# ChalmersPhotonicsLab/QAMpy

Measured on AMD Instinct MI355X. Metric: equalised MSym/s (2-pol, 2 SPS), higher is better.
Workload: dtype f32

## Files before the change

qampy_amd/csrc/api.hip:

```cpp
#include "common.h"
#include <stdlib.h>
#include <atomic>
#include <mutex>
#include <vector>
#include <unordered_map>
#include <string.h>

namespace qh {

thread_local hipStream_t g_stream = nullptr;
static thread_local hipStream_t g_streams[4] = {nullptr, nullptr, nullptr, nullptr};
int g_device = -1;
static thread_local std::string g_err;
static std::mutex g_mu;

void set_error(const std::string &s) { g_err = s; }

int hip_fail(hipError_t e, const char *what, const char *file, int line)
{
    g_err = std::string(hipGetErrorString(e)) + " in " + what + " (" + file + ":" + std::to_string(line) + ")";
    (void)hipGetLastError();
    return QH_ERR_HIP;
}

static std::atomic<int> g_reserved_cus{-1};
static std::atomic<double> g_gram_budget_gb{-1.0};
static std::atomic<int> g_default_tier{0};
static std::atomic<double> g_default_tol{1e-3};
static int reserved_cus()
{
    int v = g_reserved_cus.load();
    if (v < 0) { const char *e = getenv("QAMPY_HIP_RESERVED_CUS"); v = e ? atoi(e) : 32; if (v < 0) v = 0; g_reserved_cus.store(v); }
    return v;
}
double gram_budget_gb()
{
    double v = g_gram_budget_gb.load();
    if (v < 0) { const char *e = getenv("QAMPY_HIP_GRAM_BUDGET_GB"); v = e ? atof(e) : 160.0; if (!(v > 0)) v = 160.0; g_gram_budget_gb.store(v); }
    return v;
}
static std::atomic<int> g_pit_timing{-1};
int pit_timing_mode()
{
    int v = g_pit_timing.load();
    if (v < 0) { const char *e = getenv("QAMPY_HIP_PIT_TIMING"); v = !e ? 1 : (e[0] == 'a' ? 2 : (e[0] == 'n' ? 0 : 1)); g_pit_timing.store(v); }
    return v;
}
int default_tier() { return g_default_tier.load(); }
double default_tier_tol() { return g_default_tol.load(); }

static int init_device(int device)
{
    std::lock_guard<std::mutex> lk(g_mu);
    if (g_stream && device == g_device) return QH_OK;
    if (g_device >= 0 && device != g_device) {
        set_error("libqampy_hip is already initialised on device " + std::to_string(g_device) + ": one device per process");
        return QH_ERR_ARG;
    }
    int n = 0;
    if (hipGetDeviceCount(&n) != hipSuccess || n <= 0) {
        (void)hipGetLastError();
        set_error("no HIP device visible: libqampy_hip needs a gfx950 (MI355X) GPU, there is no CPU fallback");
        return QH_ERR_NODEVICE;
    }
    if (device < 0 || device >= n) { set_error("device index out of range"); return QH_ERR_ARG; }
    hipDeviceProp_t prop;
    QH_HIP(hipGetDeviceProperties(&prop, device));
    if (strncmp(prop.gcnArchName, "gfx950", 6) != 0) {
        set_error(std::string("device is ") + prop.gcnArchName + ", libqampy_hip is built for gfx950 only");
        return QH_ERR_NODEVICE;
    }
    QH_HIP(hipSetDevice(device));
    int prio_least = 0, prio_greatest = 0;
    QH_HIP(hipDeviceGetStreamPriorityRange(&prio_least, &prio_greatest));
    for (int i = 0; i < 4; i++) {
        if (g_streams[i]) { (void)hipStreamDestroy(g_streams[i]); g_streams[i] = nullptr; }
        if (i == 2) {
            const int reserved = reserved_cus();
            const int ncu = prop.multiProcessorCount;
            if (reserved > 0 && reserved < ncu) {
                std::vector<uint32_t> mask((ncu + 31) / 32, 0u);
                for (int c = reserved; c < ncu; c++) mask[c / 32] |= 1u << (c % 32);
                if (hipExtStreamCreateWithCUMask(&g_streams[i], (uint32_t)mask.size(), mask.data()) == hipSuccess) continue;
                (void)hipGetLastError();
                g_streams[i] = nullptr;
            }
        }
        QH_HIP(hipStreamCreateWithPriority(&g_streams[i], hipStreamNonBlocking, i == 2 ? prio_least : prio_greatest));
    }
    g_stream = g_streams[0];
    g_device = device;
    return QH_OK;
}

hipStream_t side_stream() { return g_stream == g_streams[0] ? g_streams[1] : g_streams[0]; }
hipStream_t helper_stream() { return g_streams[3]; }

int ensure_init()
{
    if (g_stream) return QH_OK;
    return init_device(g_device >= 0 ? g_device : 0);
}

thread_local void *g_scratch[16] = {nullptr};
thread_local size_t g_scratch_n[16] = {0};
thread_local unsigned g_scratch_epoch = 0;
static std::atomic<int> g_form[FORM_COUNT];
struct FormName { const char *key, *env; };
static const FormName FORM_NAMES[FORM_COUNT] = {
    {"trainer", "QAMPY_HIP_TRAINER"}, {"pit_form", "QAMPY_HIP_PIT_FORM"}, {"seg_lanes", "QAMPY_HIP_SEG_LANES"}, {"pit_probe", "QAMPY_HIP_PIT_PROBE"},
    {"bps", "QAMPY_HIP_BPS"}};
static int form_parse(int k, const char *v, int *out)
{
    if (!v || !v[0]) { *out = 0; return 0; }
    switch (k) {
    case FORM_TRAINER: *out = v[0] == 'd' ? 1 : (v[0] == 'l' ? 2 : (v[0] == 'i' ? 3 : (v[0] == 'a' || v[0] == '0' ? 0 : -1))); break;
    case FORM_PIT: *out = v[0] == 's' ? 1 : (v[0] == 'b' ? 2 : (v[0] == 'a' || v[0] == '0' ? 0 : -1)); break;
    case FORM_SEG_LANES: { const int n = atoi(v); *out = (n == 8 || n == 16 || n == 0) ? n : -1; break; }
    case FORM_BPS: *out = v[0] == 't' ? 1 : (v[0] == 'l' ? 2 : (v[0] == 'a' || v[0] == '0' ? 0 : -1)); break;
    default: *out = atoi(v) != 0 ? 1 : 0; break;
    }
    return *out < 0 ? -1 : 0;
}
static const int g_form_env_read = [] {
    for (int k = 0; k < FORM_COUNT; k++) {
        int v = 0;
        if (form_parse(k, getenv(FORM_NAMES[k].env), &v) == 0) g_form[k].store(v);
    }
    return 0;
}();
int form(FormKey k) { return g_form[k].load(std::memory_order_relaxed); }
const char *trainer_force()
{
    switch (form(FORM_TRAINER)) {
    case 1: return "direct";
    case 2: return "lookahead";
    case 3: return "iterative";
    default: return "";
    }
}
static constexpr int POOL_CLASSES = 48, POOL_KEEP = 8;
static constexpr size_t POOL_BYTES = (size_t)24 << 30;
static std::vector<void *> g_pool[POOL_CLASSES];
static size_t g_pool_bytes = 0;
static void pool_release();
static int pool_class(size_t bytes) { int k = 8; while (((size_t)1 << k) < bytes && k < POOL_CLASSES - 1) k++; return k; }
int pool_alloc(size_t bytes, void **p, size_t *cap)
{
    const int k = pool_class(bytes);
    *cap = (size_t)1 << k;
    {
        std::lock_guard<std::mutex> lk(g_mu);
        if (!g_pool[k].empty()) { *p = g_pool[k].back(); g_pool[k].pop_back(); g_pool_bytes -= *cap; return QH_OK; }
    }
    hipError_t e = hipMalloc(p, *cap);
    if (e == hipErrorOutOfMemory) {
        (void)hipGetLastError();
        (void)hipDeviceSynchronize();
        pool_release();
        e = hipMalloc(p, *cap);
    }
    QH_HIP(e);
    return QH_OK;
}
void pool_free(void *p, size_t cap)
{
    const int k = pool_class(cap);
    {
        std::lock_guard<std::mutex> lk(g_mu);
        if ((int)g_pool[k].size() < POOL_KEEP && g_pool_bytes + cap <= POOL_BYTES) { g_pool[k].push_back(p); g_pool_bytes += cap; return; }
    }
    (void)hipFree(p);
}
static std::unordered_map<void *, size_t> g_dlive;
static void pool_release()
{
    std::lock_guard<std::mutex> lk(g_mu);
    for (auto &v : g_pool) { for (void *p : v) (void)hipFree(p); v.clear(); }
    g_pool_bytes = 0;
}

static std::vector<void *> g_hpool[POOL_CLASSES];
static size_t g_hpool_bytes = 0;
static constexpr size_t HPOOL_BYTES = (size_t)8 << 30;
static std::vector<std::pair<void *, size_t>> g_hlive;
int pinned_alloc(size_t bytes, void **p)
{
    const int k = pool_class(bytes ? bytes : 1);
    const size_t cap = (size_t)1 << k;
    {
        std::lock_guard<std::mutex> lk(g_mu);
        if (!g_hpool[k].empty()) { *p = g_hpool[k].back(); g_hpool[k].pop_back(); g_hpool_bytes -= cap; g_hlive.emplace_back(*p, cap); return QH_OK; }
    }
    QH_HIP(hipHostMalloc(p, cap, hipHostMallocDefault));
    std::lock_guard<std::mutex> lk(g_mu);
    g_hlive.emplace_back(*p, cap);
    return QH_OK;
}
int pinned_free(void *p)
{
    size_t cap = 0;
    {
        std::lock_guard<std::mutex> lk(g_mu);
        for (size_t i = 0; i < g_hlive.size(); i++)
            if (g_hlive[i].first == p) { cap = g_hlive[i].second; g_hlive[i] = g_hlive.back(); g_hlive.pop_back(); break; }
        if (!cap) { set_error("qh_pinned_free: not a live buffer of qh_pinned_alloc"); return QH_ERR_ARG; }
        const int k = pool_class(cap);
        if ((int)g_hpool[k].size() < POOL_KEEP && g_hpool_bytes + cap <= HPOOL_BYTES) { g_hpool[k].push_back(p); g_hpool_bytes += cap; return QH_OK; }
    }
    (void)hipHostFree(p);
    return QH_OK;
}
static void hpool_release()
{
    std::lock_guard<std::mutex> lk(g_mu);
    for (auto &v : g_hpool) { for (void *p : v) (void)hipHostFree(p); v.clear(); }
    g_hpool_bytes = 0;
}

int scratch(int slot, size_t bytes, void **p)
{
    if (bytes > g_scratch_n[slot]) {
        if (g_scratch[slot]) QH_HIP(hipFree(g_scratch[slot]));
        g_scratch[slot] = nullptr; g_scratch_n[slot] = 0;
        QH_HIP(hipMalloc(&g_scratch[slot], bytes));
        g_scratch_n[slot] = bytes;
    }
    *p = g_scratch[slot];
    return QH_OK;
}
unsigned scratch_epoch() { return g_scratch_epoch; }

}

extern "C" {
int qh_set_trainer(int form)
{
    if (form < 0 || form > 3) { qh::set_error("qh_set_trainer: 0 automatic, 1 direct, 2 lookahead, 3 iterative"); return QH_ERR_ARG; }
    qh::g_form[qh::FORM_TRAINER].store(form);
    return QH_OK;
}
int qh_set_form(const char *key, const char *value)
{
    if (!key) { qh::set_error("qh_set_form: key"); return QH_ERR_ARG; }
    for (int k = 0; k < qh::FORM_COUNT; k++) {
        if (strcmp(key, qh::FORM_NAMES[k].key) != 0) continue;
        int v = 0;
        if (qh::form_parse(k, value, &v) != 0) { qh::set_error(std::string("qh_set_form: value '") + (value ? value : "") + "' is not one of key '" + key + "'"); return QH_ERR_ARG; }
        qh::g_form[k].store(v);
        return QH_OK;
    }
    qh::set_error(std::string("qh_set_form: unknown key '") + key + "'");
    return QH_ERR_ARG;
}
int qh_get_form(const char *key, int *value)
{
    if (!value) { qh::set_error("qh_get_form: value"); return QH_ERR_ARG; }
    for (int k = 0; key && k < qh::FORM_COUNT; k++)
        if (strcmp(key, qh::FORM_NAMES[k].key) == 0) { *value = qh::g_form[k].load(); return QH_OK; }
    qh::set_error("qh_get_form: unknown key");
    return QH_ERR_ARG;
}

int qh_set_reserved_cus(int n)
{
    if (n < 0) { qh::set_error("qh_set_reserved_cus: n >= 0"); return QH_ERR_ARG; }
    qh::g_reserved_cus.store(n);
    return QH_OK;
}
int qh_set_gram_budget_gb(double gb)
{
// ... 224 lines not shown
```

qampy_amd/csrc/common.h:

```cpp
#pragma once
#include <hip/hip_runtime.h>
#include <stdint.h>
#include <string>
#include "../../include/qampy_hip.h"

namespace qh {

extern thread_local hipStream_t g_stream;
extern int g_device;
void set_error(const std::string &s);
int hip_fail(hipError_t e, const char *what, const char *file, int line);

#define QH_HIP(call)                                                        \
    do {                                                                    \
        hipError_t _e = (call);                                             \
        if (_e != hipSuccess) return qh::hip_fail(_e, #call, __FILE__, __LINE__); \
    } while (0)

#define QH_REQUIRE(cond, msg)                                   \
    do {                                                        \
        if (!(cond)) { qh::set_error(msg); return QH_ERR_ARG; } \
    } while (0)

#define QH_WAVE_FIRST() __builtin_amdgcn_s_setprio(3)

int ensure_init();
hipStream_t side_stream();
hipStream_t helper_stream();
enum FormKey { FORM_TRAINER = 0, FORM_PIT, FORM_SEG_LANES, FORM_PIT_PROBE, FORM_BPS, FORM_COUNT };
int form(FormKey k);
const char *trainer_force();
double gram_budget_gb();
int pit_timing_mode();
int default_tier();
double default_tier_tol();
int scratch(int slot, size_t bytes, void **p);
unsigned scratch_epoch();

int pool_alloc(size_t bytes, void **p, size_t *cap);
void pool_free(void *p, size_t cap);

struct DevBuf {
    void *p = nullptr;
    size_t n = 0, cap = 0;
    ~DevBuf() { if (p) pool_free(p, cap); }
    int alloc(size_t bytes) {
        n = bytes;
        return pool_alloc(bytes ? bytes : 1, &p, &cap);
    }
    int from_host(const void *h, size_t bytes) {
        int rc = alloc(bytes);
        if (rc) return rc;
        if (bytes) QH_HIP(hipMemcpyAsync(p, h, bytes, hipMemcpyHostToDevice, g_stream));
        return QH_OK;
    }
    int to_host(void *h, size_t bytes) const {
        if (bytes) QH_HIP(hipMemcpyAsync(h, p, bytes, hipMemcpyDeviceToHost, g_stream));
        return QH_OK;
    }
};

template <typename R> struct Cx { R re, im; };

template <typename R> struct Cx2T;
template <> struct Cx2T<float> { using type = float2; };
template <> struct Cx2T<double> { using type = double2; };

template <typename R> __device__ __forceinline__ Cx<R> ldg(const Cx<R> *p)
{
    using V = typename Cx2T<R>::type;
    V v = *reinterpret_cast<const V *>(p);
    return Cx<R>{v.x, v.y};
}
template <typename R> __device__ __forceinline__ void stg(Cx<R> *p, Cx<R> v)
{
    using V = typename Cx2T<R>::type;
    V o; o.x = v.re; o.y = v.im;
    *reinterpret_cast<V *>(p) = o;
}

__device__ __forceinline__ float fma_(float a, float b, float c) { return __builtin_fmaf(a, b, c); }
__device__ __forceinline__ double fma_(double a, double b, double c) { return __builtin_fma(a, b, c); }
__device__ __forceinline__ float abs_(float a) { return __builtin_fabsf(a); }
__device__ __forceinline__ double abs_(double a) { return __builtin_fabs(a); }
__device__ __forceinline__ float min_(float a, float b) { return __builtin_fminf(a, b); }
__device__ __forceinline__ double min_(double a, double b) { return __builtin_fmin(a, b); }

constexpr int DPP_QUAD_1032 = 0xB1;
constexpr int DPP_QUAD_2301 = 0x4E;
constexpr int DPP_ROW_HALF_MIRROR = 0x141;
constexpr int DPP_ROW_MIRROR = 0x140;
constexpr int DPP_ROW_BCAST15 = 0x142;
constexpr int DPP_ROW_BCAST31 = 0x143;

template <int CTRL, int ROW_MASK = 0xF> __device__ __forceinline__ float dpp_mov(float v)
{
    return __builtin_bit_cast(float, __builtin_amdgcn_update_dpp(0, __builtin_bit_cast(int, v), CTRL, ROW_MASK, 0xF, false));
}
template <int CTRL, int ROW_MASK = 0xF> __device__ __forceinline__ double dpp_mov(double v)
{
    long long b = __builtin_bit_cast(long long, v);
    int lo = (int)b, hi = (int)(b >> 32);
    lo = __builtin_amdgcn_update_dpp(0, lo, CTRL, ROW_MASK, 0xF, false);
    hi = __builtin_amdgcn_update_dpp(0, hi, CTRL, ROW_MASK, 0xF, false);
    return __builtin_bit_cast(double, ((long long)hi << 32) | (unsigned)lo);
}

__device__ __forceinline__ float readlane(float v, int lane)
{
    return __builtin_bit_cast(float, __builtin_amdgcn_readlane(__builtin_bit_cast(int, v), lane));
}
__device__ __forceinline__ double readlane(double v, int lane)
{
    long long b = __builtin_bit_cast(long long, v);
    int lo = __builtin_amdgcn_readlane((int)b, lane), hi = __builtin_amdgcn_readlane((int)(b >> 32), lane);
    return __builtin_bit_cast(double, ((long long)hi << 32) | (unsigned)lo);
}
__device__ __forceinline__ int readlane(int v, int lane) { return __builtin_amdgcn_readlane(v, lane); }

template <typename R> __device__ __forceinline__ R wave_sum(R v)
{
    v += dpp_mov<DPP_QUAD_1032>(v);
    v += dpp_mov<DPP_QUAD_2301>(v);
    v += dpp_mov<DPP_ROW_HALF_MIRROR>(v);
    v += dpp_mov<DPP_ROW_MIRROR>(v);
    v += dpp_mov<DPP_ROW_BCAST15, 0xA>(v);
    v += dpp_mov<DPP_ROW_BCAST31, 0xC>(v);
    return readlane(v, 63);
}
template <typename R> __device__ __forceinline__ void wave_sum2(R &a, R &b)
{
    a += dpp_mov<DPP_QUAD_1032>(a);            b += dpp_mov<DPP_QUAD_1032>(b);
    a += dpp_mov<DPP_QUAD_2301>(a);            b += dpp_mov<DPP_QUAD_2301>(b);
    a += dpp_mov<DPP_ROW_HALF_MIRROR>(a);      b += dpp_mov<DPP_ROW_HALF_MIRROR>(b);
    a += dpp_mov<DPP_ROW_MIRROR>(a);           b += dpp_mov<DPP_ROW_MIRROR>(b);
    a += dpp_mov<DPP_ROW_BCAST15, 0xA>(a);     b += dpp_mov<DPP_ROW_BCAST15, 0xA>(b);
    a += dpp_mov<DPP_ROW_BCAST31, 0xC>(a);     b += dpp_mov<DPP_ROW_BCAST31, 0xC>(b);
    a = readlane(a, 63);
    b = readlane(b, 63);
}
template <typename R> __device__ __forceinline__ R wave_min(R v)
{
    v = min_(v, dpp_mov<DPP_QUAD_1032>(v));
    v = min_(v, dpp_mov<DPP_QUAD_2301>(v));
    v = min_(v, dpp_mov<DPP_ROW_HALF_MIRROR>(v));
    v = min_(v, dpp_mov<DPP_ROW_MIRROR>(v));
    R r0 = readlane(v, 0), r1 = readlane(v, 16), r2 = readlane(v, 32), r3 = readlane(v, 48);
    return min_(min_(r0, r1), min_(r2, r3));
}

}
```

qampy_amd/csrc/train_pit.h:

```cpp
#pragma once
#include <atomic>
#include <chrono>
#include <vector>
#include "train_impl.h"
#include "train_seg.h"

namespace qh {

typedef qh_pit_report PitCtrl;

constexpr double PIT_CONTRACT = 0.2;
constexpr int PIT_PROBE = 128;
constexpr int PIT_SEEDWIN = 512;
constexpr int PIT_MAXSEG = 65536;

__host__ __device__ inline int pit_symmetry(int method)
{
    switch (method) {
    case QH_M_CMA: case QH_M_SGNCMA: case QH_M_RDE: return 0;
    case QH_M_CMA2: return 2;
    default: return 4;
    }
}

// ... 56 lines not shown
    for (int k = 0; k < nmodes; k++)
        for (int64_t i = threadIdx.x; i < npow; i += 256) {
            const Cx<R> v = E[(size_t)k * L + i];
            acc += (double)v.re * v.re + (double)v.im * v.im;
        }
    red[threadIdx.x] = acc;
    __syncthreads();
    for (int s = 128; s > 0; s >>= 1) {
        if (threadIdx.x < s) red[threadIdx.x] += red[threadIdx.x + s];
        __syncthreads();
    }
    if (threadIdx.x == 0) {
        const double p = red[0] / ((double)nmodes * (double)npow);
        const double m = (double)*mu;
        double ma = gear * m;
        const double cap = bound / ((double)ntot * (p > 1e-30 ? p : 1e-30));
        if (ma > cap) ma = cap;
        if (!(ma > m)) ma = m;
        c->segments = sg.S; c->seg_len = sg.len; c->mu = m; c->mu_acq = ma; c->power = p; c->tol = tol;
        for (int q = 0; q < QH_PIT_MAXPASS; q++) { c->result_change[q] = -1; c->deviation[q] = -1; c->deviation_rms[q] = -1; c->deviation_taps[q] = -1; c->deviation_taps_worst[q] = -1; } c->passes = 0; c->converged = 0; c->acq_chunks = 0; c->acq_steps = 0; c->acq_done = 0; c->done = 0; c->diverged = 0; c->corr_on = 0; c->gain = 0; c->out_power = 0;
        for (int i = 0; i < QH_PIT_MAXPASS; i++) c->defect[i] = -1;
        for (int i = 0; i < QH_PIT_MAXCHUNK; i++) c->acq_err[i] = -1;
        *mu_acq = (R)ma;
    }
}

template <typename R>
__global__ void __launch_bounds__(256) pit_acq_monitor_kernel(const Cx<R> *err, int64_t err_pitch, int64_t step0, int64_t n, int nsel,
                                                              const int64_t *modes_dev, double plateau, PitCtrl *c, R *mu_acq, const R *mu, double floor_gear)
{
    QH_WAVE_FIRST();
    if (threadIdx.x == 0 && floor_gear >= 0) {
        const R lo = (R)((double)*mu * floor_gear), h = *mu_acq * (R)0.5;
        *mu_acq = h > lo ? h : (*mu_acq > lo ? lo : *mu_acq);
    }
    if (c->acq_done) return;
    __shared__ double red[256];
    double acc = 0;
    for (int j = 0; j < nsel; j++) {
        const Cx<R> *row = err + (size_t)modes_dev[j] * err_pitch + step0;
        for (int64_t i = threadIdx.x; i < n; i += 256) {
            const Cx<R> v = row[i];
            acc += (double)v.re * v.re + (double)v.im * v.im;
        }
    }
    red[threadIdx.x] = acc;
    __syncthreads();
    for (int s = 128; s > 0; s >>= 1) {
        if (threadIdx.x < s) red[threadIdx.x] += red[threadIdx.x + s];
        __syncthreads();
    }
    if (threadIdx.x == 0) {
        const double v = red[0] / ((double)n * nsel);
        const int k = c->acq_chunks;
        if (k < QH_PIT_MAXCHUNK) c->acq_err[k] = v;
        c->acq_chunks = k + 1;
        c->acq_steps = step0 + n;
        if (!(v == v) || v > 1e30) { c->diverged = 1; c->acq_done = 1; return; }
        if (k >= 1) {
            const double prev = c->acq_err[k - 1 < QH_PIT_MAXCHUNK ? k - 1 : QH_PIT_MAXCHUNK - 1];
            if (v > 100 * c->acq_err[0]) { c->diverged = 1; c->acq_done = 1; return; }
            if (v > plateau * prev) c->acq_done = 1;
        }
    }
}

template <typename R> __global__ void pit_acq_finish_kernel(Cx<R> *wx, const Cx<R> *w_start, int n, PitCtrl *c)
{
    QH_WAVE_FIRST();
    const int i = blockIdx.x * blockDim.x + threadIdx.x;
    if (c->diverged && i < n) wx[i] = w_start[i];
}

inline size_t pit_phase_pitch(int ntaps, int os, int nwin) { return (size_t)nwin + (size_t)(ntaps + os - 1) / os + 1; }
template <typename R>
__global__ void __launch_bounds__(256) pit_phase_kernel(const Cx<R> *E, int nmodes, int64_t L, int os, const Cx<R> *wx, int ntaps, PitSeg sg,
                                                        const int64_t *modes_dev, int nwin, double *z)
{
    QH_WAVE_FIRST();
    extern __shared__ __attribute__((aligned(16))) char pit_smem[];
    Cx<R> *w = reinterpret_cast<Cx<R> *>(pit_smem);
    const int ntot = nmodes * ntaps;
    const int pitch = nwin + (ntaps + os - 1) / os + 1;
    Cx<R> *xs = w + ntot;
    __shared__ double rr[256], ri[256];
    const int s = blockIdx.x, j = blockIdx.y;
    const int mode = (int)modes_dev[j];
    for (int f = threadIdx.x; f < ntot; f += 256) w[f] = wx[(size_t)mode * ntot + f];
    const int64_t st = sg.start(s);
    int64_t n = sg.steps(s);
    if (n > nwin) n = nwin;
    const int ns = n > 0 ? (int)(n - 1) * os + ntaps : 0;
    for (int k = 0; k < nmodes; k++) {
        const Cx<R> *x = E + (size_t)k * L + st * os;
        for (int g = threadIdx.x; g < ns; g += 256) xs[((size_t)k * os + g % os) * pitch + g / os] = x[g];
    }
    __syncthreads();
    double zr = 0, zi = 0;
    for (int i = threadIdx.x; i < n; i += 256) {
        R yr = 0, yi = 0;
        for (int k = 0; k < nmodes; k++) {
            const Cx<R> *wk = w + k * ntaps;
            for (int r = 0; r < os; r++) {
                const Cx<R> *xp = xs + ((size_t)k * os + r) * pitch + i;
                int u = 0;
                for (int t = r; t < ntaps; t += os, u++) {
                    const Cx<R> a = xp[u], b = wk[t];
                    yr = fma_(a.re, b.re, fma_(-a.im, b.im, yr));
                    yi = fma_(a.re, b.im, fma_(a.im, b.re, yi));
                }
            }
        }
        const double y2r = (double)yr * yr - (double)yi * yi, y2i = 2.0 * yr * yi;
        zr += y2r * y2r - y2i * y2i;
        zi += 2.0 * y2r * y2i;
    }
    rr[threadIdx.x] = zr; ri[threadIdx.x] = zi;
    __syncthreads();
    for (int q = 128; q > 0; q >>= 1) {
        if (threadIdx.x < q) { rr[threadIdx.x] += rr[threadIdx.x + q]; ri[threadIdx.x] += ri[threadIdx.x + q]; }
        __syncthreads();
    }
    if (threadIdx.x == 0) { z[2 * ((size_t)s * gridDim.y + j)] = rr[0]; z[2 * ((size_t)s * gridDim.y + j) + 1] = ri[0]; }
}

static __global__ void __launch_bounds__(256) pit_unwrap_kernel(const double *z, int S, int nsel, double *rot, double *phi, int *jump)
{
    QH_WAVE_FIRST();
    __shared__ int ptot[512];
    const double q = 1.5707963267948966;
    phi += (size_t)blockIdx.x * S; jump += (size_t)blockIdx.x * S;
    for (int j = blockIdx.x; j <= (int)blockIdx.x; j++) {
        for (int s = threadIdx.x; s < S; s += 256) {
            const double zr = z[2 * ((size_t)s * nsel + j)], zi = z[2 * ((size_t)s * nsel + j) + 1];
            phi[s] = (zr == 0 && zi == 0) ? 0.0 : (double)atan2f((float)-zi, (float)-zr) / 4;
        }
        __syncthreads();
        for (int s = threadIdx.x; s < S; s += 256) jump[s] = s == 0 ? 0 : (int)rint((phi[s - 1] - phi[s]) / q);
        __syncthreads();
        block_prefix_sum<int>(jump, S, ptot);
        for (int s = threadIdx.x; s < S; s += 256) {
            const double p = phi[s] + q * (jump[s] & 3);
            float sn, cs;
            sincosf((float)p, &sn, &cs);
            rot[2 * ((size_t)s * nsel + j)] = cs;
            rot[2 * ((size_t)s * nsel + j) + 1] = -sn;
        }
        __syncthreads();
    }
}

template <typename R>
__global__ void __launch_bounds__(256) pit_seed_kernel(const Cx<R> *wx, int nmodes, int ntot, const int64_t *modes_dev, int nsel, const double *rot, Cx<R> *X,
                                                       const Cx<R> *w0, Cx<R> *Y, PitCtrl *c)
{
    QH_WAVE_FIRST();
    const int s = blockIdx.x;
    const int n = nmodes * ntot;
    if (s == 0 && c) {
        if (threadIdx.x == 0) { c->done = 0; c->converged = 0; c->passes = 0; }
        for (int q = threadIdx.x; q < QH_PIT_MAXPASS; q += 256) {
            c->result_change[q] = -1; c->deviation[q] = -1; c->deviation_rms[q] = -1; c->deviation_taps[q] = -1; c->deviation_taps_worst[q] = -1; c->defect[q] = -1;
        }
    }
    const bool exact0 = s == 0 && w0 != nullptr;
    for (int e = threadIdx.x; e < n; e += 256) {
        const int row = e / ntot;
        Cx<R> v = exact0 ? w0[e] : wx[e];
        if (rot && !exact0) {
            for (int j = 0; j < nsel; j++)
                if ((int)modes_dev[j] == row) {
                    const double c = rot[2 * ((size_t)s * nsel + j)], d = rot[2 * ((size_t)s * nsel + j) + 1];
                    const double vr = (double)v.re * c - (double)v.im * d, vi = (double)v.re * d + (double)v.im * c;
                    v = Cx<R>{(R)vr, (R)vi};
                    break;
                }
        }
        X[(size_t)s * n + e] = v;
        Y[(size_t)s * n + e] = v;
    }
}

template <typename R>
__global__ void __launch_bounds__(PIT_PROBE) pit_defect_kernel(const Cx<R> *E, int nmodes, int64_t L, int os, int ntaps, PitSeg sg, int64_t TrSyms,
                                                                const int64_t *modes_dev, const Cx<R> *X, const Cx<R> *Y, int sym, const PitCtrl *c, double *dfc, double *pw, double *gph,
                                                                const Cx<R> *wx_prev)
{
    QH_WAVE_FIRST();
    if (c->done) return;
    extern __shared__ __attribute__((aligned(16))) char pit_smem[];
    Cx<R> *wa = reinterpret_cast<Cx<R> *>(pit_smem);
    const int ntot = nmodes * ntaps;
    Cx<R> *wb = wa + ntot;
    const int pitch = PIT_PROBE + (ntaps + os - 1) / os + 1;
    Cx<R> *xs = wb + ntot;
    __shared__ double red[4][PIT_PROBE];
    const int b = blockIdx.x + 1, j = blockIdx.y;
    const int mode = (int)modes_dev[j];
    const size_t wset = (size_t)nmodes * ntot;
    const bool result_probe = b == sg.S;
    for (int f = threadIdx.x; f < ntot; f += PIT_PROBE) {
        wa[f] = result_probe ? wx_prev[(size_t)mode * ntot + f] : X[(size_t)b * wset + (size_t)mode * ntot + f];
        wb[f] = Y[(size_t)(b - 1) * wset + (size_t)mode * ntot + f];
    }
    const int64_t st0 = result_probe ? (TrSyms > PIT_PROBE ? TrSyms - PIT_PROBE : 0) : sg.start(b);
    int64_t nout = TrSyms - st0;
    if (nout > PIT_PROBE) nout = PIT_PROBE;
    const int ns = nout > 0 ? (int)(nout - 1) * os + ntaps : 0;
    for (int k = 0; k < nmodes; k++) {
        const Cx<R> *x = E + (size_t)k * L + st0 * os;
        for (int g = threadIdx.x; g < ns; g += PIT_PROBE) xs[((size_t)k * os + g % os) * pitch + g / os] = x[g];
    }
    __syncthreads();
    double aa = 0, bb = 0, cr = 0, ci = 0;
    if (threadIdx.x < nout) {
        R ar = 0, ai = 0, br = 0, bi = 0;
        for (int k = 0; k < nmodes; k++)
            for (int r = 0; r < os; r++) {
                const Cx<R> *xp = xs + ((size_t)k * os + r) * pitch + threadIdx.x;
                int u = 0;
                for (int t = r; t < ntaps; t += os, u++) {
                    const Cx<R> v = xp[u], p = wa[k * ntaps + t], q = wb[k * ntaps + t];
                    ar = fma_(v.re, p.re, fma_(-v.im, p.im, ar)); ai = fma_(v.re, p.im, fma_(v.im, p.re, ai));
                    br = fma_(v.re, q.re, fma_(-v.im, q.im, br)); bi = fma_(v.re, q.im, fma_(v.im, q.re, bi));
                }
            }
        aa = (double)ar * ar + (double)ai * ai;
        bb = (double)br * br + (double)bi * bi;
        cr = (double)br * ar + (double)bi * ai;
        ci = (double)bi * ar - (double)br * ai;
    }
    red[0][threadIdx.x] = aa; red[1][threadIdx.x] = bb; red[2][threadIdx.x] = cr; red[3][threadIdx.x] = ci;
    __syncthreads();
    for (int q = PIT_PROBE / 2; q > 0; q >>= 1) {
        if (threadIdx.x < q)
            for (int u = 0; u < 4; u++) red[u][threadIdx.x] += red[u][threadIdx.x + q];
        __syncthreads();
    }
    if (threadIdx.x == 0) {
        const double A = red[0][0], B = red[1][0], Cr = red[2][0], Ci = red[3][0];
        double proj, gr = 1, gi = 0;
        if (sym == 0) {
            proj = sqrt(Cr * Cr + Ci * Ci);
            if (proj > 0) { gr = Cr / proj; gi = Ci / proj; }
        } else if (sym == 4 || sym == 2 || sym == 1) {
            if (sym == 4 && fabs(Ci) > fabs(Cr)) { gr = 0; gi = Ci >= 0 ? 1 : -1; proj = fabs(Ci); }
            else if (sym == 1) { gr = 1; proj = Cr; }
            else { gr = Cr >= 0 ? 1 : -1; proj = fabs(Cr); }
        } else {
            const double step = 6.283185307179586 / sym;
            const double k = rint(atan2(Ci, Cr) / step) * step;
            gr = cos(k); gi = sin(k);
            proj = Cr * gr + Ci * gi;
        }
        if (!result_probe) { gph[2 * ((size_t)blockIdx.x * gridDim.y + j)] = gr; gph[2 * ((size_t)blockIdx.x * gridDim.y + j) + 1] = gi; }
        double d2 = (A + B - 2 * proj) / (B > 1e-300 ? B : 1e-300);
        if (d2 < 0) d2 = 0;
        dfc[(size_t)blockIdx.x * gridDim.y + j] = (A == A && B == B) ? sqrt(d2) : 1e30;
        if (!result_probe) pw[(size_t)blockIdx.x * gridDim.y + j] = B / PIT_PROBE;
    }
}

template <typename R> __device__ inline double pit_gain(int method, double Py, Cx<R> c0)
{
    switch (method) {
    case QH_M_CMA: case QH_M_SGNCMA: return 2 * Py - (double)c0.re;
    case QH_M_MCMA: return 1.5 * Py - 0.5 * ((double)c0.re + (double)c0.im);
    case QH_M_RDE: case QH_M_MRDE: case QH_M_MDDMA: return Py;
    case QH_M_DD: return 1.0;
    case QH_M_SBD: return 0.866 * sqrt(Py / 2);
    default: return 0.0;
    }
}

constexpr double PIT_DEV_SAFETY = 1.0, PIT_DEV_WORST = 3.0, PIT_DEV_TAPS = 2.0, PIT_DEV_TAPS_WORST = 3.0;
template <typename R> struct PitDecideArgs {
    const double *dfc, *pw;
    int nb;
    const Cx<R> *Ylast;
    int n;
    Cx<R> *wx;
    PitCtrl *c;
    float *host_view;
    int nrow;
    const float *devmax;
    int ndev;
    double safety;
    const float2 *Ye;
    float2 *Yprev;
    int ne, ncol_e;
    const double *theta;
    const int64_t *modes_dev;
    int ntot_w, S, sym, corr_wanted;
    const float2 *Dfin;
    const float2 *Vfin;
    const double *lam_fin;
    int stall_from;
    const float *extra;
};
constexpr int PIT_FIN_MAX = 128;
template <typename R> __device__ __forceinline__ void pit_decide_body(const PitDecideArgs<R> &a)
{
    const double *dfc = a.dfc; const int nb = a.nb; const Cx<R> *Ylast = a.Ylast; const int n = a.n; Cx<R> *wx = a.wx; PitCtrl *c = a.c; float *host_view = a.host_view;
    const int nrow = a.nrow; const float *devmax = a.devmax; const int ndev = a.ndev; const double safety = a.safety; const float2 *Ye = a.Ye; float2 *Yprev = a.Yprev;
    const int ne = a.ne, ncol_e = a.ncol_e; const double *theta = a.theta; const int64_t *modes_dev = a.modes_dev; const int ntot_w = a.ntot_w, S = a.S, sym = a.sym, corr_wanted = a.corr_wanted;
    const int p = c->passes, corr_on0 = c->corr_on;
    const double c_out_power = c->out_power, c_gain = c->gain, c_power = c->power, c_mu = c->mu, c_tol = c->tol;
    const double c_seg_len = (double)c->seg_len;
    const int pl = p - 1 < QH_PIT_MAXPASS ? p - 1 : QH_PIT_MAXPASS - 1, pl2 = p - 2 < QH_PIT_MAXPASS ? p - 2 : QH_PIT_MAXPASS - 1;
    const double drms1 = p >= 1 ? c->deviation_rms[pl] : 0.0, drms2 = p >= 2 ? c->deviation_rms[pl2] : 0.0, dfc2 = p >= 2 ? c->defect[pl2] : 0.0;
    if (Yprev)
        for (int e = threadIdx.x; e < ne * nrow; e += 256) { const int k = e / nrow, j = e - k * nrow; Yprev[e] = Ye[(size_t)k * ncol_e + (ncol_e - nrow) + j]; }
    __shared__ double red[4], redd[4], reds[4], redt[4], redw[4], redm[4];
    __shared__ int s_flag[2];
    __shared__ float s_crit;
    double m = 0, dv = 0, ds = 0, dt = 0, wn = 0, dm = 0;
    for (int i0 = threadIdx.x; i0 < nb; i0 += 8 * 256) {
        double v[8];
#pragma unroll
        for (int q = 0; q < 8; q++) v[q] = i0 + 256 * q < nb ? dfc[i0 + 256 * q] : 0.0;
#pragma unroll
        for (int q = 0; q < 8; q++) m = (v[q] > m || !(v[q] == v[q])) ? (v[q] == v[q] ? v[q] : 1e30) : m;
    }
    if (devmax)
        for (int i = threadIdx.x; i < ndev; i += 256) {
            const double v = (double)devmax[4 * i];
            dv = (v > dv || !(v == v)) ? (v == v ? v : 1e30) : dv;
            ds += (double)devmax[4 * i + 1];
            dt += (double)devmax[4 * i + 2];
            const double vm = (double)devmax[4 * i + 3];
            dm = (vm > dm || !(vm == vm)) ? (vm == vm ? vm : 1e30) : dm;
        }
    double chg = 0;
    for (int r = 0; r < nrow; r++) { const double v = dfc[nb + r]; chg = (v > chg || !(v == v)) ? v : chg; }
    const bool extrap = a.Dfin != nullptr && p >= 1 && corr_on0 && c_gain > 0;
    for (int e = threadIdx.x; e < n; e += 256) {
        Cx<R> v = Ylast[e];
        wn += (double)v.re * v.re + (double)v.im * v.im;
        const int row = e / ntot_w;
        int jj = -1;
        for (int j = 0; j < nrow; j++) if ((int)modes_dev[j] == row) { jj = j; break; }
        if (jj >= 0 && theta) {
            const double tr = theta[2 * ((size_t)(S - 1) * nrow + jj)], ti = theta[2 * ((size_t)(S - 1) * nrow + jj) + 1];
            if (sym == 0) v = Cx<R>{(R)(tr * v.re - ti * v.im), (R)(tr * v.im + ti * v.re)};
        }
        wx[e] = v;
    }
    for (int o = 32; o > 0; o >>= 1) {
        const double m2 = __shfl_xor(m, o), dv2 = __shfl_xor(dv, o), dm2 = __shfl_xor(dm, o);
        m = m > m2 ? m : m2; dv = dv > dv2 ? dv : dv2; dm = dm > dm2 ? dm : dm2;
        ds += __shfl_xor(ds, o); dt += __shfl_xor(dt, o); wn += __shfl_xor(wn, o);
    }
    if ((threadIdx.x & 63) == 0) {
        const int w = threadIdx.x >> 6;
        red[w] = m; redd[w] = dv; reds[w] = ds; redt[w] = dt; redw[w] = wn; redm[w] = dm;
    }
    __syncthreads();
    if (threadIdx.x == 0)
        for (int w = 1; w < 4; w++) {
            red[0] = red[0] > red[w] ? red[0] : red[w]; redd[0] = redd[0] > redd[w] ? redd[0] : redd[w]; redm[0] = redm[0] > redm[w] ? redm[0] : redm[w];
            reds[0] += reds[w]; redt[0] += redt[w]; redw[0] += redw[w];
        }
    if (threadIdx.x == 0) {
        const bool have_dev = devmax != nullptr && corr_on0 && c_out_power > 0;
        const double dev = have_dev ? sqrt(redd[0] / c_out_power) : -1.0;
        const double dev_rms = have_dev ? sqrt(reds[0] / ((double)(nb + nrow) * c_out_power)) : -1.0;
        const double wnorm2 = redw[0] / (double)(nrow > 0 ? nrow : 1);
        const double dev_tap = (have_dev && wnorm2 > 0) ? sqrt(redt[0] / ((double)(nb + nrow) * wnorm2)) : -1.0;
        const double dev_tap_worst = (have_dev && wnorm2 > 0) ? sqrt(redm[0] / wnorm2) : -1.0;
        if (p < QH_PIT_MAXPASS) { c->defect[p] = red[0]; c->result_change[p] = chg; c->deviation[p] = dev; c->deviation_rms[p] = dev_rms; c->deviation_taps[p] = dev_tap; c->deviation_taps_worst[p] = dev_tap_worst; }
        c->passes = p + 1;
        double crit;
        if (have_dev) {
            crit = safety * dev_rms;
            if (safety * dev / PIT_DEV_WORST > crit) crit = safety * dev / PIT_DEV_WORST;
            double rho = 1.0;
            if (extrap && drms1 > 0) { rho = dev_rms / drms1; rho = rho < 0.25 ? 0.25 : (rho > 1.0 ? 1.0 : rho); }
            if (dev_tap >= 0 && safety * rho * dev_tap / PIT_DEV_TAPS > crit) crit = safety * rho * dev_tap / PIT_DEV_TAPS;
            if (dev_tap_worst >= 0 && safety * rho * dev_tap_worst / PIT_DEV_TAPS_WORST > crit) crit = safety * rho * dev_tap_worst / PIT_DEV_TAPS_WORST;
        }
        else {
            double amp = 1.0;
            if (c_gain > 0 && c_power > 0 && c_mu > 0) {
                const double gl = c_gain * 2.0 * c_power, a = c_mu * c_seg_len * gl;
                if (a > 0) amp = (1.0 - exp(-0.2 * gl)) / (1.0 - exp(-a));
                if (!(amp > 1.0)) amp = 1.0;
            }
            crit = red[0] * amp;
        }
        if (have_dev && p >= 2 && p < QH_PIT_MAXPASS && drms1 > 0 && drms2 > 0 && dev_rms > 1.5 * drms1 && drms1 > 1.5 * drms2) c->corr_on = 0;
        if (a.extra) { const double ex = (double)a.extra[0]; if (p < QH_PIT_MAXPASS) c->result_change[p] = ex; if (ex > crit || !(ex == ex)) crit = ex == ex ? ex : 1e30; }
        int done = 0, conv = 0;
        if (crit < c_tol && (have_dev || !corr_wanted)) { c->converged = 1; done = 1; conv = 1; }
        else if (p >= a.stall_from && p < QH_PIT_MAXPASS) {
            const bool use_dev = have_dev && drms2 > 0;
            const double prev2 = use_dev ? drms2 : dfc2, now = use_dev ? dev_rms : red[0];
            if (!(now < prev2)) done = 1;
        }
        if (done) c->done = 1;
        s_flag[0] = done; s_flag[1] = conv; s_crit = (float)crit;
    }
    __syncthreads();
    if (s_flag[1] && extrap) {
        __shared__ float2 s_cd[PIT_FIN_MAX];
        const float2 *VT = a.Vfin + (size_t)ntot_w * ntot_w;
        for (int jj = 0; jj < nrow; jj++) {
            const size_t col = (size_t)(S - 1) * nrow + jj;
            for (int k = threadIdx.x; k < ntot_w; k += 256) {
                const double ak = c_mu * c_gain * c_seg_len * a.lam_fin[k];
                const float ck = ak > 0 ? __expf(-(float)ak) : 1.f;
                const float2 dk = a.Dfin[(size_t)k * ncol_e + col];
                s_cd[k] = float2{ck * dk.x, ck * dk.y};
            }
            __syncthreads();
            const int row = (int)modes_dev[jj];
            const double tr = theta[2 * ((size_t)(S - 1) * nrow + jj)], ti = theta[2 * ((size_t)(S - 1) * nrow + jj) + 1];
            for (int f = threadIdx.x; f < ntot_w; f += 256) {
                float dr = 0.f, di = 0.f;
#pragma unroll 8
                for (int k = 0; k < ntot_w; k++) {
                    const float2 vk = VT[(size_t)k * ntot_w + f], cd = s_cd[k];
                    dr += vk.x * cd.x - vk.y * cd.y; di += vk.x * cd.y + vk.y * cd.x;
                }
                const int e = row * ntot_w + f;
                const Cx<R> v = wx[e];
                if (sym == 0) wx[e] = Cx<R>{(R)(v.re + dr), (R)(v.im + di)};
                else wx[e] = Cx<R>{(R)(v.re + tr * dr + ti * di), (R)(v.im + tr * di - ti * dr)};
            }
            __syncthreads();
        }
        __threadfence();
    }
    __syncthreads();
    if (threadIdx.x == 0) {
        host_view[1] = s_crit;
        __threadfence_system();
        __hip_atomic_store(&host_view[0], s_flag[0] ? (s_flag[1] ? 1.f : 2.f) : 0.f, __ATOMIC_RELEASE, __HIP_MEMORY_SCOPE_SYSTEM);
    }
}

template <typename R> __global__ void __launch_bounds__(256) pit_decide_kernel(PitDecideArgs<R> a)
{
    QH_WAVE_FIRST();
    if (a.c->done) return;
    pit_decide_body<R>(a);
}

template <typename R>
__global__ void __launch_bounds__(256) pit_rotate_err_kernel(Cx<R> *err, int64_t err_pitch, int64_t err_off, PitSeg sg, const int64_t *modes_dev, int nsel,
                                                             const double *theta, const PitCtrl *c, int p)
{
    QH_WAVE_FIRST();
    if (p >= 0 && (!c->done || c->passes != p + 1)) return;
    const int s = blockIdx.x, j = blockIdx.y;
    if (s == 0) return;
    const double tr = theta[2 * ((size_t)s * nsel + j)], ti = theta[2 * ((size_t)s * nsel + j) + 1];
    Cx<R> *row = err + (size_t)modes_dev[j] * err_pitch + err_off + sg.start(s);
    const int64_t n = sg.steps(s);
    for (int64_t i = threadIdx.x; i < n; i += 256) {
        const Cx<R> v = row[i];
        row[i] = Cx<R>{(R)(tr * v.re - ti * v.im), (R)(tr * v.im + ti * v.re)};
    }
}

typedef double2 Z;
__device__ __forceinline__ Z zmul(Z a, Z b) { return Z{a.x * b.x - a.y * b.y, a.x * b.y + a.y * b.x}; }

constexpr int PIT_COVW = 32, PIT_COVB = 256;
template <typename R, int EPT>
__global__ void __launch_bounds__(256) pit_cov_kernel(const Cx<R> *E, int nmodes, int64_t L, int os, int ntaps, int64_t TrSyms, int nwin, Z *part)
{
    QH_WAVE_FIRST();
    extern __shared__ __attribute__((aligned(16))) char pit_smem[];
    Cx<R> *x = reinterpret_cast<Cx<R> *>(pit_smem);
    const int ntot = nmodes * ntaps;
    const int nent = ntot * ntot;
    const int64_t stride = TrSyms / nwin > 0 ? TrSyms / nwin : 1;
    for (int e = threadIdx.x; e < PIT_COVW * ntot; e += 256) {
        const int w = e / ntot, f = e - w * ntot;
        const int k = f / ntaps, t = f - k * ntaps;
        const int64_t i = ((int64_t)blockIdx.x * PIT_COVW + w) * stride;
        x[e] = (i < TrSyms && (int64_t)blockIdx.x * PIT_COVW + w < nwin) ? E[(size_t)k * L + i * os + t] : Cx<R>{0, 0};
    }
    __syncthreads();
#pragma unroll 1
    for (int q = 0; q < EPT; q++) {
        const int e = threadIdx.x + 256 * q;
        if (e >= nent) break;
        const int fa = e / ntot, fb = e - fa * ntot;
        float ar = 0, ai = 0;
#pragma unroll 8
        for (int w = 0; w < PIT_COVW; w++) {
            const Cx<R> u = x[w * ntot + fa], v = x[w * ntot + fb];
            ar += (float)(u.re * v.re + u.im * v.im);
            ai += (float)(u.re * v.im - u.im * v.re);
        }
        part[(size_t)blockIdx.x * nent + e] = Z{(double)ar, (double)ai};
    }
}
static __global__ void __launch_bounds__(256) pit_cov_reduce_kernel(const Z *part, int nent, int nblk, Z *Rc)
{
    QH_WAVE_FIRST();
    __shared__ double sr[256], si[256];
    const int e = blockIdx.x * 64 + (threadIdx.x & 63), grp = threadIdx.x >> 6;
    double ar = 0, ai = 0;
    if (e < nent) {
#pragma unroll 16
        for (int b = grp; b < nblk; b += 4) { const Z v = part[(size_t)b * nent + e]; ar += v.x; ai += v.y; }
    }
    sr[threadIdx.x] = ar; si[threadIdx.x] = ai;
    __syncthreads();
    if (grp == 0 && e < nent) {
        const int t = threadIdx.x;
        Rc[e] = Z{(sr[t] + sr[t + 64]) + (sr[t + 128] + sr[t + 192]), (si[t] + si[t + 64]) + (si[t + 128] + si[t + 192])};
    }
}

typedef float2 Zf;
constexpr int PIT_EIGMAX = 128, PIT_EIGSWEEPS = 5;
static_assert(PIT_FIN_MAX >= PIT_EIGMAX, "final extrapolation stages one eigen-space column");
__device__ __forceinline__ Zf cmulf(Zf a, Zf b) { return Zf{a.x * b.x - a.y * b.y, a.x * b.y + a.y * b.x}; }
static __global__ void __launch_bounds__(1024) pit_jacobi_kernel(const Z *Rc, int n, double norm, double *lam, Zf *Vout, int nsweep, float4 *glog)
{
    QH_WAVE_FIRST();
    extern __shared__ __attribute__((aligned(16))) char pit_smem[];
    const int ld = n + 1;
    Zf *A = reinterpret_cast<Zf *>(pit_smem);
    Zf *V = A + (size_t)n * ld;
    const int tid = threadIdx.x;
    const int wave = tid >> 6, lane = tid & 63;
    for (int i = wave; i < n; i += 16)
        for (int j = lane; j < n; j += 64) {
            const Z v = Rc[(size_t)i * n + j];
            A[i * ld + j] = Zf{(float)(v.x * norm), (float)(v.y * norm)};
            if (!glog) V[i * ld + j] = Zf{i == j ? 1.f : 0.f, 0.f};
        }
    __syncthreads();
    const int m = (n + 1) & ~1;
    const int npair = m / 2;
    constexpr int NP = (PIT_EIGMAX / 2 + 15) / 16, NR = (PIT_EIGMAX + 63) / 64;
    for (int sweep = 0; sweep < nsweep; sweep++) {
        for (int r = 0; r < m - 1; r++) {
            int2 ixs[NP];
            float4 gs[NP];
            auto pair_of = [&](int i) -> int2 {
                int pa, pb;
                if (i == 0) { pa = m - 1; pb = r; }
                else {
                    pa = r + i; if (pa >= m - 1) pa -= m - 1;
                    pb = r - i; if (pb < 0) pb += m - 1;
                }
                const int p = pa < pb ? pa : pb, q = pa < pb ? pb : pa;
                return (i < npair && q < n) ? int2{p, q} : int2{0, n};
            };
            float4 gl = {1.f, 0.f, 1.f, 0.f};
            {
                const int2 ix = pair_of(wave + 16 * (lane < NP ? lane : 0));
                if (lane < NP && ix.y < n) {
                    const Zf apq = A[ix.x * ld + ix.y];
                    const float app = A[ix.x * ld + ix.x].x, aqq = A[ix.y * ld + ix.y].x;
                    const float m2 = apq.x * apq.x + apq.y * apq.y;
                    if (m2 > 1e-36f) {
                        const float rmag = __builtin_amdgcn_rsqf(m2);
                        const float tau = (aqq - app) * 0.5f * rmag;
                        const float t = (tau >= 0 ? 1.f : -1.f) * __builtin_amdgcn_rcpf(fabsf(tau) + __builtin_amdgcn_sqrtf(1.f + tau * tau));
                        const float c = __builtin_amdgcn_rsqf(1.f + t * t);
                        gl = float4{c, t * c, apq.x * rmag, apq.y * rmag};
                    }
                }
            }
#pragma unroll
            for (int a = 0; a < NP; a++) {
                ixs[a] = pair_of(wave + 16 * a);
                gs[a] = float4{__builtin_bit_cast(float, __builtin_amdgcn_readlane(__builtin_bit_cast(int, gl.x), a)),
                               __builtin_bit_cast(float, __builtin_amdgcn_readlane(__builtin_bit_cast(int, gl.y), a)),
                               __builtin_bit_cast(float, __builtin_amdgcn_readlane(__builtin_bit_cast(int, gl.z), a)),
                               __builtin_bit_cast(float, __builtin_amdgcn_readlane(__builtin_bit_cast(int, gl.w), a))};
            }
            if (glog && lane < NP) {
                const int pi = wave + 16 * lane;
                if (pi < npair) glog[((size_t)sweep * (m - 1) + r) * npair + pi] = gl;
            }
            {
                Zf xp[NP][NR][2], xq[NP][NR][2];
#pragma unroll
                for (int a = 0; a < NP; a++) {
                    const int2 ix = ixs[a];
                    if (ix.y >= n) continue;
#pragma unroll
                    for (int b = 0; b < NR; b++) {
                        if (64 * b >= n) continue;
                        const int row = lane + 64 * b < n ? lane + 64 * b : n - 1;
                        xp[a][b][0] = A[row * ld + ix.x]; xq[a][b][0] = A[row * ld + ix.y];
                        if (!glog) { xp[a][b][1] = V[row * ld + ix.x]; xq[a][b][1] = V[row * ld + ix.y]; }
                    }
                }
#pragma unroll
                for (int a = 0; a < NP; a++) {
// ... 327 lines not shown
    }
}
template <typename R, int PHASE>
__global__ void __launch_bounds__(256) pit_model_kernel(PitModelArgs<R> a)
{
    QH_WAVE_FIRST();
    const int lane = threadIdx.x & 63, wave = threadIdx.x >> 6, grp = lane >> 4, l16 = lane & 15;
    const int gg = (blockIdx.x * 4 + wave) * 4 + grp, ng = gridDim.x * 16;
    const int ntot = a.nmodes * a.ntaps;
    constexpr int TP = PIT_EIGMAX / 16;
    const int pw = 2 * PIT_EIGMAX + 8;
    const int tpl = (ntot + 15) / 16;
    for (int j = 0; j < a.nsel; j++) {
        const int mode = (int)a.modes[j];
        __shared__ Zf tab[PIT_MODTAB];
        const int nsy_l = a.nsy <= PIT_MODTAB ? (int)a.nsy : 1;
        const int tables_l = a.nsy <= PIT_MODTAB ? a.tables : 0;
        __syncthreads();
        for (int e = threadIdx.x; e < nsy_l; e += 256) { const Cx<R> v = a.symbols[(size_t)mode * a.sy_pitch + e]; tab[e] = Zf{(float)v.re, (float)v.im}; }
        __syncthreads();
        Zf wv[TP], uv[TP], pacc[TP];
        int64_t xoff[TP];
        float gacc = 0.f, k11 = 0.f, k12 = 0.f, k22 = 0.f, zz = 0.f, cnt = 0.f;
#pragma unroll
        for (int q = 0; q < TP; q++) {
            const int f = l16 * tpl + q;
            const bool ok = q < tpl && f < ntot;
            const int k = ok ? f / a.ntaps : 0;
            xoff[q] = ok ? (int64_t)k * a.L + (f - k * a.ntaps) : -1;
            wv[q] = Zf{0.f, 0.f}; uv[q] = Zf{0.f, 0.f}; pacc[q] = Zf{0.f, 0.f};
            if (ok) { const Cx<R> t = a.wx[(size_t)mode * ntot + f]; wv[q] = Zf{(float)t.re, (float)t.im}; if (PHASE == 1) { const Cx<R> v = a.u[(size_t)j * ntot + f]; uv[q] = Zf{(float)v.re, (float)v.im}; } }
        }
        int64_t st = ((int64_t)PIT_SEEDWIN * a.sg.S) / PIT_MODW;
        st = st < 1 ? 1 : (st > 37 ? 37 : st);
        for (int wi0 = gg - grp; wi0 < PIT_MODW; wi0 += ng) {
            const int wi = wi0 + grp;
            const int sgi = wi % a.sg.S;
            const int64_t off = (int64_t)(wi / a.sg.S) * st;
            const int64_t i = a.sg.start(sgi) + off;
            const bool valid = wi < PIT_MODW && off < PIT_SEEDWIN && off < a.sg.steps(sgi) && i < a.TrSyms;
            float rc = 1.f, rs = 0.f;
            if (a.rot && valid) { rc = (float)a.rot[2 * ((size_t)sgi * a.nsel + j)]; rs = (float)a.rot[2 * ((size_t)sgi * a.nsel + j) + 1]; }
            Zf xv[TP];
            float yr = 0.f, yi = 0.f, zr = 0.f, zi = 0.f;
#pragma unroll
            for (int q = 0; q < TP; q++) {
                xv[q] = Zf{0.f, 0.f};
                if (valid && xoff[q] >= 0) { const Cx<R> v = a.E[xoff[q] + i * a.os]; xv[q] = Zf{(float)v.re, (float)v.im}; }
            }
#pragma unroll
            for (int q = 0; q < TP; q++) {
                yr += xv[q].x * wv[q].x - xv[q].y * wv[q].y; yi += xv[q].x * wv[q].y + xv[q].y * wv[q].x;
                if (PHASE == 1) { zr += xv[q].x * uv[q].x - xv[q].y * uv[q].y; zi += xv[q].x * uv[q].y + xv[q].y * uv[q].x; }
            }
            for (int o = 8; o > 0; o >>= 1) { yr += __shfl_xor(yr, o); yi += __shfl_xor(yi, o); if (PHASE == 1) { zr += __shfl_xor(zr, o); zi += __shfl_xor(zi, o); } }
            const float yr0 = yr, yi0 = yi;
            { const float t = yr * rc - yi * rs; yi = yr * rs + yi * rc; yr = t; }
            if (PHASE == 1) { const float t = zr * rc - zi * rs; zi = zr * rs + zi * rc; zr = t; }
            float g11, g12, g22;
            pit_gain_matrix(a.method, yr, yi, tab, nsy_l, tables_l, g11, g12, g22);
            if (valid) {
                if (PHASE == 0) {
#pragma unroll
                    for (int q = 0; q < TP; q++) { pacc[q].x += xv[q].x * yr0 + xv[q].y * yi0; pacc[q].y += xv[q].x * yi0 - xv[q].y * yr0; }
                    gacc += 0.5f * (g11 + g22);
                } else {
                    k11 += zr * zr * g11 + 2 * zr * zi * g12 + zi * zi * g22;
                    k22 += zi * zi * g11 - 2 * zr * zi * g12 + zr * zr * g22;
                    k12 += -zr * zi * g11 + (zr * zr - zi * zi) * g12 + zr * zi * g22;
                    zz += zr * zr + zi * zi;
                }
                cnt += 1.f;
            }
        }
        __shared__ float blk[4][2 * PIT_EIGMAX + 8];
        for (int e = lane; e < 2 * PIT_EIGMAX + 8; e += 64) blk[wave][e] = 0.f;
        if (PHASE == 0) {
#pragma unroll
            for (int q = 0; q < TP; q++) {
                float pr = pacc[q].x, pi = pacc[q].y;
                pr += __shfl_xor(pr, 16); pi += __shfl_xor(pi, 16); pr += __shfl_xor(pr, 32); pi += __shfl_xor(pi, 32);
                const int f = l16 * tpl + q;
                if (grp == 0 && q < tpl && f < ntot) { blk[wave][2 * f] = pr; blk[wave][2 * f + 1] = pi; }
            }
            gacc += __shfl_xor(gacc, 16); gacc += __shfl_xor(gacc, 32); cnt += __shfl_xor(cnt, 16); cnt += __shfl_xor(cnt, 32);
            if (lane == 0) { blk[wave][2 * PIT_EIGMAX] = gacc; blk[wave][2 * PIT_EIGMAX + 1] = cnt; }
        } else {
            for (int o = 16; o <= 32; o <<= 1) { k11 += __shfl_xor(k11, o); k12 += __shfl_xor(k12, o); k22 += __shfl_xor(k22, o); zz += __shfl_xor(zz, o); cnt += __shfl_xor(cnt, o); }
            if (lane == 0) { blk[wave][0] = k11; blk[wave][1] = k12; blk[wave][2] = k22; blk[wave][3] = zz; blk[wave][4] = cnt; }
        }
        __syncthreads();
        float *dst = a.part + ((size_t)blockIdx.x * a.nsel + j) * pw;
        const int nval = PHASE == 0 ? 2 * PIT_EIGMAX + 2 : 5;
        for (int e = threadIdx.x; e < nval; e += 256) dst[e] = (blk[0][e] + blk[1][e]) + (blk[2][e] + blk[3][e]);
        __syncthreads();
    }
    __shared__ int last;
    __syncthreads();
    if (threadIdx.x == 0) { __threadfence(); const unsigned t = atomicAdd(a.ticket, 1u); last = t == gridDim.x - 1; if (last) { *a.ticket = 0; __threadfence(); } }
    __syncthreads();
    if (!last) return;
    __shared__ float red[256];
    const int nblk = gridDim.x;
    auto psum = [&](int j, int e) -> float {
        float acc = 0.f;
        for (int b0 = 0; b0 < nblk; b0 += 16) {
            float v[16];
#pragma unroll
            for (int q = 0; q < 16; q++) v[q] = b0 + q < nblk ? a.part[((size_t)(b0 + q) * a.nsel + j) * pw + e] : 0.f;
#pragma unroll
            for (int q = 0; q < 16; q++) acc += v[q];
        }
        return acc;
    };
    __shared__ float vals[2 * PIT_EIGMAX + 8];
    const int nval = PHASE == 0 ? 2 * PIT_EIGMAX + 2 : 5;
    for (int j = 0; j < a.nsel; j++) {
        for (int e = threadIdx.x; e < nval; e += 256) vals[e] = (PHASE == 1 || e >= 2 * PIT_EIGMAX || e < 2 * ntot) ? psum(j, e) : 0.f;
        __syncthreads();
        if (PHASE == 0) {
            float nrm = 0.f;
            for (int f = threadIdx.x; f < ntot; f += 256) nrm += vals[2 * f] * vals[2 * f] + vals[2 * f + 1] * vals[2 * f + 1];
            red[threadIdx.x] = nrm; __syncthreads();
            for (int o = 128; o > 0; o >>= 1) { if (threadIdx.x < o) red[threadIdx.x] += red[threadIdx.x + o]; __syncthreads(); }
            const float inv = red[0] > 0.f ? rsqrtf(red[0]) : 0.f;
            for (int f = threadIdx.x; f < ntot; f += 256) a.u[(size_t)j * ntot + f] = Cx<R>{(R)(vals[2 * f] * inv), (R)(vals[2 * f + 1] * inv)};
            if (threadIdx.x == 0) {
                const float gs = vals[2 * PIT_EIGMAX], cs = vals[2 * PIT_EIGMAX + 1];
                a.model[j].g = cs > 0.f ? gs / cs : 0.f;
                a.model[j].ok = 0;
            }
        } else if (threadIdx.x == 0) {
            float k11 = vals[0], k12 = vals[1], k22 = vals[2], zz = vals[3];
            const float cs = vals[4];
            const float n = cs > 0.f ? 1.f / cs : 0.f;
            k11 *= n; k12 *= n; k22 *= n; zz *= n;
            const float tr = 0.5f * (k11 + k22), df = 0.5f * (k11 - k22), rad = sqrtf(df * df + k12 * k12);
            float c = 1.f, sn = 0.f;
            if (rad > 1e-12f * (fabsf(tr) + 1e-30f)) { const float ang = 0.5f * atan2f(k12, df); c = cosf(ang); sn = sinf(ang); }
            PitModel m = a.model[j];
            m.k1 = tr + rad; m.k2 = tr - rad; m.q11 = c; m.q21 = sn; m.q12 = -sn; m.q22 = c; m.lam_u = zz;
            m.ok = (m.g > 0.f && m.g == m.g && m.k1 == m.k1 && m.k2 == m.k2) ? 1 : 0;
            a.model[j] = m;
        }
        __syncthreads();
    }
}

typedef float pit_f4 __attribute__((ext_vector_type(4)));
constexpr int PIT_MC = 16, PIT_MBP = PIT_MC + 1;
inline int pit_mfma_threads(int n) { return 64 * ((n + 15) / 16); }
inline size_t pit_mfma_lds(int n) { return ((size_t)(n + 4) * PIT_MBP + (size_t)PIT_MC * (PIT_EIGMAX + 1)) * sizeof(Zf); }
template <typename R, int MODE>
__global__ void __launch_bounds__(64 * (PIT_EIGMAX / 16)) pit_basis_mfma_kernel(const Zf *__restrict__ A2, const Cx<R> *__restrict__ T, const Zf *__restrict__ D, Zf *__restrict__ Out,
                                                                               int n, int ncol, const PitCtrl *c, PitFuse<R> fz)
{
    QH_WAVE_FIRST();
    if (c->done) return;
    extern __shared__ __attribute__((aligned(16))) char pit_smem[];
    const int np = (n + 3) & ~3;
    Zf *Bs = reinterpret_cast<Zf *>(pit_smem);
    Zf *Ct = Bs + (size_t)(n + 4) * PIT_MBP;
    const int tid = threadIdx.x, lane = tid & 63, wave = tid >> 6, nw = blockDim.x >> 6, nt = blockDim.x;
    const int nb1 = (ncol + PIT_MC - 1) / PIT_MC;
    const bool second = MODE == 0 && (int)blockIdx.x >= nb1;
    if (second) { T = fz.T2; Out = reinterpret_cast<Zf *>(fz.Out2); }
    const int col0 = ((int)blockIdx.x - (second ? nb1 : 0)) * PIT_MC;
    const size_t wset = (size_t)fz.nmodes * n;
    const int am = 16 * wave + (lane & 15), ak = lane >> 4;
    const Zf *ag = A2 + (size_t)ak * n + am;
    auto lda = [&](int k) -> Zf { return (am < n && k + ak < n) ? ag[(size_t)k * n] : Zf{0.f, 0.f}; };
    constexpr int PF = 8;
    Zf abuf[PF];
#pragma unroll
    for (int i = 0; i < PF; i++) abuf[i] = lda(4 * i);
    constexpr int NCW = 3;
    if (MODE == 0) {
        for (int cb = 0; cb < PIT_MC; cb += NCW * nw) {
            Zf tmp[NCW][2];
#pragma unroll
            for (int q = 0; q < NCW; q++) {
                const int cc = cb + wave + nw * q, col = col0 + cc;
                tmp[q][0] = Zf{0.f, 0.f}; tmp[q][1] = Zf{0.f, 0.f};
                if (cc < PIT_MC && col < ncol) {
                    const int s = col / fz.nsel, j = col - s * fz.nsel;
                    const Cx<R> *src = T + (size_t)s * wset + (size_t)fz.modes_dev[j] * n;
                    if (lane < n) { const Cx<R> t = src[lane]; tmp[q][0] = Zf{(float)t.re, (float)t.im}; }
                    if (lane + 64 < n) { const Cx<R> t = src[lane + 64]; tmp[q][1] = Zf{(float)t.re, (float)t.im}; }
                }
            }
#pragma unroll
            for (int q = 0; q < NCW; q++) {
                const int cc = cb + wave + nw * q;
                if (cc < PIT_MC) {
                    if (lane < np) Bs[lane * PIT_MBP + cc] = tmp[q][0];
                    if (lane + 64 < np) Bs[(lane + 64) * PIT_MBP + cc] = tmp[q][1];
                }
            }
        }
    } else {
        const int cc = tid & 15, k0 = tid >> 4, kstep = nt >> 4;
        const bool okc = col0 + cc < ncol;
        for (int kb = 0; kb < np; kb += 8 * kstep) {
            Zf tmp[8];
#pragma unroll
            for (int q = 0; q < 8; q++) {
                const int k = kb + k0 + kstep * q;
                tmp[q] = (okc && k < n) ? D[(size_t)k * ncol + col0 + cc] : Zf{0.f, 0.f};
            }
#pragma unroll
            for (int q = 0; q < 8; q++) {
                const int k = kb + k0 + kstep * q;
                if (k < np) Bs[k * PIT_MBP + cc] = tmp[q];
            }
        }
    }
    const bool pre = MODE == 1 && NCW * nw >= PIT_MC;
    Cx<R> xv[MODE == 1 ? NCW : 1][2];
    double th[MODE == 1 ? NCW : 1][2];
    if (pre) {
#pragma unroll
        for (int q = 0; q < NCW; q++) {
            const int cc = wave + nw * q, col = col0 + cc;
            xv[q][0] = Cx<R>{0, 0}; xv[q][1] = Cx<R>{0, 0}; th[q][0] = 1; th[q][1] = 0;
            if (cc < PIT_MC && col < ncol) {
                const int s = col / fz.nsel, j = col - s * fz.nsel;
                const size_t base = (size_t)s * wset + (size_t)fz.modes_dev[j] * n;
                th[q][0] = fz.theta[2 * (size_t)col]; th[q][1] = fz.theta[2 * (size_t)col + 1];
                if (lane < n) xv[q][0] = fz.X[base + lane];
                if (lane + 64 < n) xv[q][1] = fz.X[base + lane + 64];
            }
        }
    }
    __syncthreads();
    pit_f4 rr = {0.f, 0.f, 0.f, 0.f}, ii = rr, im = rr;
    const Zf *bp = Bs + (lane >> 4) * PIT_MBP + (lane & 15);
    for (int k0 = 0; k0 < np; k0 += 4 * PF) {
#pragma unroll
        for (int i = 0; i < PF; i++) {
            const int k = k0 + 4 * i;
            if (k < np) {
                Zf a = abuf[i];
                abuf[i] = lda(k + 4 * PF);
                if (MODE == 0) a.y = -a.y;
                const Zf b = bp[(size_t)k * PIT_MBP];
                rr = __builtin_amdgcn_mfma_f32_16x16x4f32(a.x, b.x, rr, 0, 0, 0);
                ii = __builtin_amdgcn_mfma_f32_16x16x4f32(a.y, b.y, ii, 0, 0, 0);
                im = __builtin_amdgcn_mfma_f32_16x16x4f32(a.x, b.y, im, 0, 0, 0);
                im = __builtin_amdgcn_mfma_f32_16x16x4f32(a.y, b.x, im, 0, 0, 0);
            }
        }
    }
    const int cl = lane & 15;
    if (MODE == 0) {
        const int col = col0 + cl;
#pragma unroll
        for (int q = 0; q < 4; q++) {
            const int m = 16 * wave + 4 * (lane >> 4) + q;
            if (m < n && col < ncol) Out[(size_t)m * ncol + col] = Zf{rr[q] - ii[q], im[q]};
        }
    } else {
#pragma unroll
        for (int q = 0; q < 4; q++) {
            const int m = 16 * wave + 4 * (lane >> 4) + q;
            Ct[cl * (PIT_EIGMAX + 1) + m] = Zf{rr[q] - ii[q], im[q]};
        }
        __syncthreads();
        for (int cb = 0; cb < PIT_MC; cb += NCW * nw) {
#pragma unroll
            for (int q = 0; q < NCW; q++) {
                const int cc = cb + wave + nw * q, col = col0 + cc;
                if (cc < PIT_MC && col < ncol) {
                    const int s = col / fz.nsel, j = col - s * fz.nsel;
                    const size_t base = (size_t)s * wset + (size_t)fz.modes_dev[j] * n;
                    const double qr = pre ? th[q][0] : fz.theta[2 * (size_t)col], qi = pre ? th[q][1] : fz.theta[2 * (size_t)col + 1];
#pragma unroll
                    for (int h = 0; h < 2; h++) {
                        const int m = lane + 64 * h;
                        if (m < n) {
                            const Cx<R> x = pre ? xv[q][h] : fz.X[base + m];
                            const Zf d = Ct[cc * (PIT_EIGMAX + 1) + m];
                            const Cx<R> w{(R)(qr * x.re - qi * x.im + fz.damp * d.x), (R)(qr * x.im + qi * x.re + fz.damp * d.y)};
                            fz.X[base + m] = w;
                            fz.Y[base + m] = w;
                        }
                    }
                }
            }
        }
    }
}

static __global__ void __launch_bounds__(256) pit_bound_kernel(const Zf *Xe, const Zf *Ye, const Zf *Yprev, const double *lam, int n, int S, int nsel, int sym,
                                                              const PitCtrl *c, double *dfc, double *pw, double *gph, float4 *ualpha = nullptr)
{
    QH_WAVE_FIRST();
    if (c->done) return;
    const int lane = threadIdx.x & 63, bi = blockIdx.x * 4 + (threadIdx.x >> 6);
    const int nb = (S - 1) * nsel, ncol = S * nsel;
    if (bi >= nb + nsel) return;
    const bool result_probe = bi >= nb;
    const int j = result_probe ? bi - nb : bi % nsel;
    const int sb = result_probe ? S - 1 : bi / nsel;
    const Zf *pa = result_probe ? (c->passes == 0 ? Xe + (size_t)(S - 1) * nsel + j : Yprev + j) : Xe + (size_t)(sb + 1) * nsel + j;
    const size_t sa = (result_probe && c->passes != 0) ? (size_t)nsel : (size_t)ncol;
    const Zf *pb = Ye + (size_t)sb * nsel + j;
    Zf av[(PIT_EIGMAX + 63) / 64], bv[(PIT_EIGMAX + 63) / 64];
    float lv[(PIT_EIGMAX + 63) / 64];
    double A = 0, B = 0, Cr = 0, Ci = 0;
#pragma unroll
    for (int q = 0; q < (PIT_EIGMAX + 63) / 64; q++) {
        const int k = lane + 64 * q;
        av[q] = Zf{0.f, 0.f}; bv[q] = Zf{0.f, 0.f}; lv[q] = 0.f;
        if (k < n) {
            av[q] = pa[(size_t)k * sa]; bv[q] = pb[(size_t)k * ncol];
            const float l = (float)lam[k];
            lv[q] = l > 0.f ? l : 0.f;
        }
        A += (double)lv[q] * ((double)av[q].x * av[q].x + (double)av[q].y * av[q].y);
        B += (double)lv[q] * ((double)bv[q].x * bv[q].x + (double)bv[q].y * bv[q].y);
        Cr += (double)lv[q] * ((double)bv[q].x * av[q].x + (double)bv[q].y * av[q].y);
        Ci += (double)lv[q] * ((double)bv[q].y * av[q].x - (double)bv[q].x * av[q].y);
    }
    for (int o = 32; o > 0; o >>= 1) { A += __shfl_xor(A, o); B += __shfl_xor(B, o); Cr += __shfl_xor(Cr, o); Ci += __shfl_xor(Ci, o); }
    double gr = 1, gi = 0;
    if (sym == 0) {
        const double pr = sqrt(Cr * Cr + Ci * Ci);
        if (pr > 0) { gr = Cr / pr; gi = Ci / pr; }
    } else if (sym == 4 || sym == 2 || sym == 1) {
        if (sym == 4 && fabs(Ci) > fabs(Cr)) { gr = 0; gi = Ci >= 0 ? 1 : -1; }
        else if (sym == 1) gr = 1;
        else gr = Cr >= 0 ? 1 : -1;
    } else {
        const double step = 6.283185307179586 / sym;
        const double kk = rint(atan2(Ci, Cr) / step) * step;
        gr = cos(kk); gi = sin(kk);
    }
    double d2 = 0;
    const float grf = (float)gr, gif = (float)gi;
#pragma unroll
    for (int q = 0; q < (PIT_EIGMAX + 63) / 64; q++) {
        const float dr = bv[q].x - (grf * av[q].x - gif * av[q].y), di = bv[q].y - (grf * av[q].y + gif * av[q].x);
        d2 += (double)lv[q] * ((double)dr * dr + (double)di * di);
    }
    for (int o = 32; o > 0; o >>= 1) d2 += __shfl_xor(d2, o);
    if (ualpha && !result_probe) {
        float nn = 0.f, ar = 0.f, ai = 0.f;
#pragma unroll
        for (int q = 0; q < (PIT_EIGMAX + 63) / 64; q++) {
            const float dr = bv[q].x - (grf * av[q].x - gif * av[q].y), di = bv[q].y - (grf * av[q].y + gif * av[q].x);
            const float ur = lv[q] * bv[q].x, ui = lv[q] * bv[q].y;
            nn += ur * ur + ui * ui;
            ar += ur * dr + ui * di;
            ai += ur * di - ui * dr;
        }
        for (int o = 32; o > 0; o >>= 1) { nn += __shfl_xor(nn, o); ar += __shfl_xor(ar, o); ai += __shfl_xor(ai, o); }
        const float inv = nn > 0.f ? rsqrtf(nn) : 0.f;
        if (lane == 0) ualpha[bi] = float4{ar * inv, ai * inv, inv, 0.f};
    }
    if (lane == 0) {
        if (!result_probe) { gph[2 * (size_t)bi] = gr; gph[2 * (size_t)bi + 1] = gi; pw[bi] = B; }
        dfc[bi] = (A == A && B == B) ? sqrt(d2 / (B > 1e-300 ? B : 1e-300)) : 1e30;
    }
}

constexpr int PIT_RT = 1024;
template <typename R>
__global__ void __launch_bounds__(PIT_RT) pit_recur_eig_kernel(Zf *Xe, const Zf *Ye, Zf *D, const double *theta, const double *lam, int nsel, int S, int64_t T, const R *mu,
                                                               double beta, const PitCtrl *c, const float *Msum = nullptr, float damp = 1.f,
                                                               const float4 *ualpha = nullptr, const float2 *uq = nullptr)
{
    QH_WAVE_FIRST();
    if (c->done) return;
    __shared__ float4 aff[2 * PIT_RT];
    const int k = blockIdx.x, j = blockIdx.y;
    const int ncol = S * nsel;
    Zf *row = D + (size_t)k * ncol + j, *xr = Xe + (size_t)k * ncol + j;
    const Zf *yr = Ye + (size_t)k * ncol + j;
    double a = (double)*mu * c->gain * (double)T * lam[k];
    if (a < 0) a = 0;
    const float coef = c->corr_on ? (float)exp(-a * (1 + beta * a)) : 0.f;
    const float gl = (float)(c->gain * lam[k] > 0 ? c->gain * lam[k] : 0.0), betaf = (float)beta;
    const bool corr = c->corr_on != 0;
    auto cf = [&](int s) -> float {
        if (!Msum) return coef;
        const float as = gl * Msum[(size_t)s * nsel + j];
        return corr ? __expf(-as * (1.f + betaf * as)) : 0.f;
    };
    const int len = (S + PIT_RT - 1) / PIT_RT;
    const int s0 = threadIdx.x * len, s1 = s0 + len < S ? s0 + len : S;
    auto th = [&](int s) { return Zf{(float)theta[2 * ((size_t)s * nsel + j)], (float)theta[2 * ((size_t)s * nsel + j) + 1]}; };
    auto scan_op = [](float4 e, float4 l) { return float4{l.x * e.x, l.x * e.y + l.y, l.x * e.z + l.z, 0.f}; };
    if (len <= 4) {
        Zf y[4], x[4], t[5], r[4];
        t[0] = s0 > 0 && s0 < S ? th(s0 - 1) : Zf{1.f, 0.f};
#pragma unroll
        for (int q = 0; q < 4; q++) {
            const int s = s0 + q;
            const bool ok = s < s1;
            y[q] = (ok && s > 0) ? yr[(size_t)(s - 1) * nsel] : Zf{0.f, 0.f};
            x[q] = ok ? xr[(size_t)s * nsel] : Zf{0.f, 0.f};
            t[q + 1] = ok ? th(s) : Zf{1.f, 0.f};
        }
        Zf run{0.f, 0.f};
        float cq[4], clen = 1.f;
        float4 ua[4];
        float2 qq[4];
        const float lk = (float)(lam[k] > 0 ? lam[k] : 0.0);
#pragma unroll
        for (int q = 0; q < 4; q++) {
            const int s = s0 + q;
            cq[q] = (s < s1 && s > 0) ? cf(s - 1) : (s < s1 ? 0.f : 1.f);
            ua[q] = (ualpha && s < s1 && s > 0) ? ualpha[(size_t)(s - 1) * nsel + j] : float4{0.f, 0.f, 0.f, 0.f};
            qq[q] = (uq && s < s1 && s > 0) ? uq[(size_t)s * nsel + j] : float2{0.f, 0.f};
        }
        Zf uk[4];
#pragma unroll
        for (int q = 0; q < 4; q++) {
            const int s = s0 + q;
            uk[q] = Zf{0.f, 0.f};
            if (s < s1) {
                x[q] = cmulf(t[q + 1], x[q]);
                Zf d{0.f, 0.f};
                if (s > 0) {
                    const Zf aa = cmulf(t[q], y[q]);
                    d = Zf{aa.x - x[q].x, aa.y - x[q].y};
                    uk[q] = Zf{aa.x * lk * ua[q].z, aa.y * lk * ua[q].z};
                    const Zf ual = cmulf(uk[q], Zf{ua[q].x, ua[q].y});
                    d = Zf{d.x - ual.x, d.y - ual.y};
                }
                run = Zf{d.x + cq[q] * run.x, d.y + cq[q] * run.y};
                r[q] = run;
                clen *= cq[q];
            }
        }
        const float4 comp = block_scan_excl<float4, decltype(scan_op), PIT_RT>(float4{clen, run.x, run.y, 0.f}, scan_op, float4{1.f, 0.f, 0.f, 0.f}, aff);
        float pw = 1.f;
#pragma unroll
        for (int q = 0; q < 4; q++) {
            const int s = s0 + q;
            if (s < s1) {
                pw *= cq[q];
                const Zf uqv = cmulf(uk[q], Zf{qq[q].x, qq[q].y});
                const Zf v{r[q].x + pw * comp.y + uqv.x, r[q].y + pw * comp.z + uqv.y};
                row[(size_t)s * nsel] = v;
                xr[(size_t)s * nsel] = Zf{x[q].x + damp * v.x, x[q].y + damp * v.y};
            }
        }
        return;
    }
    Zf run{0.f, 0.f};
    float clen = 1.f;
    for (int sb = s0; sb < s1; sb += 4) {
        Zf y[4], x[4], t[5];
        t[0] = sb > 0 ? th(sb - 1) : Zf{1.f, 0.f};
#pragma unroll
        for (int q = 0; q < 4; q++) {
            const int s = sb + q;
            const bool ok = s < s1;
            y[q] = (ok && s > 0) ? yr[(size_t)(s - 1) * nsel] : Zf{0.f, 0.f};
            x[q] = ok ? xr[(size_t)s * nsel] : Zf{0.f, 0.f};
            t[q + 1] = ok ? th(s) : Zf{1.f, 0.f};
        }
#pragma unroll
        for (int q = 0; q < 4; q++) {
            const int s = sb + q;
            if (s < s1) {
                Zf d{0.f, 0.f};
                if (s > 0) {
                    const Zf aa = cmulf(t[q], y[q]), bb = cmulf(t[q + 1], x[q]);
                    d = Zf{aa.x - bb.x, aa.y - bb.y};
                    if (ualpha) {
                        const float4 al = ualpha[(size_t)(s - 1) * nsel + j];
                        const float lk2 = (float)(lam[k] > 0 ? lam[k] : 0.0);
                        const Zf ual = cmulf(Zf{aa.x * lk2 * al.z, aa.y * lk2 * al.z}, Zf{al.x, al.y});
                        d = Zf{d.x - ual.x, d.y - ual.y};
                    }
                }
                const float cs = s > 0 ? cf(s - 1) : 0.f;
                run = Zf{d.x + cs * run.x, d.y + cs * run.y};
                clen *= cs;
                row[(size_t)s * nsel] = run;
            }
        }
    }
    const float4 comp = block_scan_excl<float4, decltype(scan_op), PIT_RT>(float4{clen, run.x, run.y, 0.f}, scan_op, float4{1.f, 0.f, 0.f, 0.f}, aff);
    const Zf cin{comp.y, comp.z};
    float pw = 1.f;
    for (int sb = s0; sb < s1; sb += 4) {
        Zf v[4], x[4], t[4];
#pragma unroll
        for (int q = 0; q < 4; q++) {
            const int s = sb + q;
            const bool ok = s < s1;
            v[q] = ok ? row[(size_t)s * nsel] : Zf{0.f, 0.f};
            x[q] = ok ? xr[(size_t)s * nsel] : Zf{0.f, 0.f};
            t[q] = ok ? th(s) : Zf{1.f, 0.f};
        }
#pragma unroll
        for (int q = 0; q < 4; q++) {
            const int s = sb + q;
            if (s < s1) {
                pw *= s > 0 ? cf(s - 1) : 0.f;
                v[q].x += pw * cin.x; v[q].y += pw * cin.y;
                if (uq && s > 0) {
                    const float4 al = ualpha[(size_t)(s - 1) * nsel + j];
                    const float2 qv = uq[(size_t)s * nsel + j];
                    const float lk2 = (float)(lam[k] > 0 ? lam[k] : 0.0);
                    const Zf ts = s > 0 ? th(s - 1) : Zf{1.f, 0.f};
                    const Zf aa = cmulf(ts, yr[(size_t)(s - 1) * nsel]);
                    const Zf uqv = cmulf(Zf{aa.x * lk2 * al.z, aa.y * lk2 * al.z}, Zf{qv.x, qv.y});
                    v[q].x += uqv.x; v[q].y += uqv.y;
                }
                row[(size_t)s * nsel] = v[q];
                const Zf xx = cmulf(t[q], x[q]);
                xr[(size_t)s * nsel] = Zf{xx.x + damp * v[q].x, xx.y + damp * v[q].y};
            }
        }
    }
}

template <typename R>
__global__ void __launch_bounds__(256) pit_recur_kernel(Zf *D, const double *lam, int nsel, int S, int64_t T, const R *mu, double beta, const PitCtrl *c)
{
    QH_WAVE_FIRST();
    if (c->done) return;
    __shared__ float4 aff[512];
    const int k = blockIdx.x, j = blockIdx.y;
    const int ncol = S * nsel;
    Zf *row = D + (size_t)k * ncol + j;
    double a = (double)*mu * c->gain * (double)T * lam[k];
    if (a < 0) a = 0;
    const float coef = c->corr_on ? (float)exp(-a * (1 + beta * a)) : 0.f;
    const int len = (S + 255) / 256;
    const int s0 = threadIdx.x * len, s1 = s0 + len < S ? s0 + len : S;
    Zf run{0.f, 0.f};
    for (int s = s0; s < s1; s++) {
        const Zf d = row[(size_t)s * nsel];
        run = Zf{d.x + coef * run.x, d.y + coef * run.y};
        row[(size_t)s * nsel] = run;
    }
    const float clen = powf(coef, (float)len);
    const float4 comp = block_scan_excl<float4>(float4{clen, run.x, run.y, 0.f},
                                                [](float4 e, float4 l) { return float4{l.x * e.x, l.x * e.y + l.y, l.x * e.z + l.z, 0.f}; },
                                                float4{1.f, 0.f, 0.f, 0.f}, aff);
    const Zf cin{comp.y, comp.z};
    float pw = coef;
    for (int s = s0; s < s1; s++) {
        Zf v = row[(size_t)s * nsel];
        v.x += pw * cin.x; v.y += pw * cin.y;
        row[(size_t)s * nsel] = v;
        pw *= coef;
    }
}

template <typename R>
__global__ void __launch_bounds__(256) pit_adapt_init_kernel(const R *mu, const Cx<R> *e_last, int n, R *rS, Cx<R> *eS)
{
    QH_WAVE_FIRST();
    const R r0 = (R)1 / *mu;
    for (int s = blockIdx.x * 256 + threadIdx.x; s < n; s += gridDim.x * 256) { rS[s] = r0; eS[s] = s == 0 ? *e_last : Cx<R>{0, 0}; }
}
template <typename R>
__global__ void __launch_bounds__(1024) pit_adapt_scan_kernel(R *rS, const R *rE, Cx<R> *eS, const Cx<R> *eE, int n, float *chg, const PitCtrl *c, float relax,
                                                              float *rPrev, float *dPrev, int newton)
{
    QH_WAVE_FIRST();
    if (c->done) return;
    __shared__ double2 buf[16];
    __shared__ float red[16];
    const int pass = c->passes;
    const int len = (n + 1023) / 1024;
    const int s0 = threadIdx.x * len, s1 = s0 + len < n ? s0 + len : n;
    auto seg_map = [&](int s, double &A, double &B) {
        const double rho = (double)rS[s], d = (double)rE[s] - rho;
        double kappa = 0;
        if (newton && pass >= 2) {
            const double rp = (double)rPrev[s], dp = (double)dPrev[s];
            if (fabs(rho - rp) > 1e-6 * rho && fabs(d) > 1e-30) kappa = -((d - dp) / d) / ((rho - rp) / rho);
            kappa = kappa == kappa ? (kappa < 0 ? 0 : (kappa > 4 ? 4 : kappa)) : 0;
        }
        A = 1.0 - kappa * d / rho;
        B = d * (1.0 + kappa);
    };
    double Ac = 1, Bc = 0;
    for (int s = s0; s < s1; s++) { double A, B; seg_map(s, A, B); Bc = A * Bc + B; Ac = A * Ac; }
    auto comp = [](double2 e, double2 l) { return double2{l.x * e.x, l.x * e.y + l.y}; };
    const double2 pre = block_scan_excl<double2, decltype(comp), 1024>(double2{Ac, Bc}, comp, double2{1.0, 0.0}, buf);
    double run = pre.x * (double)rS[0] + pre.y;
    float worst = 0.f;
    for (int s = s0; s < s1; s++) {
        double A, B;
        seg_map(s, A, B);
        const float old = (float)rS[s];
        rPrev[s] = old; dPrev[s] = (float)((double)rE[s] - (double)old);
        if (s > 0) {
            const float nw = pass == 0 ? (float)run : old + relax * ((float)run - old);
            const float rel = fabsf(nw - old) / (fabsf(old) > 1e-30f ? fabsf(old) : 1e-30f);
            worst = (rel > worst || !(rel == rel)) ? (rel == rel ? rel : 3.0e38f) : worst;
            rS[s] = (R)nw;
            eS[s] = eE[s - 1];
        }
        run = A * run + B;
    }
    for (int o = 32; o > 0; o >>= 1) { const float w2 = __shfl_xor(worst, o); worst = worst > w2 ? worst : w2; }
    if ((threadIdx.x & 63) == 0) red[threadIdx.x >> 6] = worst;
    __syncthreads();
    if (threadIdx.x == 0) { float m = 0.f; for (int w = 0; w < 16; w++) m = m > red[w] ? m : red[w]; chg[0] = m; }
}
template <typename R> __global__ void pit_adapt_finish_kernel(R *mu, const R *rE, int n) { *mu = (R)1 / rE[n - 1]; }

struct PitInit { void *z[3]; unsigned zn[3]; void *cd[2]; const void *cs[2]; unsigned cn[2]; int64_t *modes_dev; int64_t modes[16]; int nsel; };
static __global__ void __launch_bounds__(256) pit_init_kernel(PitInit a)
{
    QH_WAVE_FIRST();
    const unsigned t = blockIdx.x * 256 + threadIdx.x, nt = gridDim.x * 256;
#pragma unroll
    for (int r = 0; r < 3; r++)
        if (a.z[r]) for (unsigned i = t; i < a.zn[r] / 4; i += nt) reinterpret_cast<uint32_t *>(a.z[r])[i] = 0u;
#pragma unroll
    for (int r = 0; r < 2; r++)
        if (a.cd[r]) for (unsigned i = t; i < a.cn[r] / 8; i += nt) reinterpret_cast<uint64_t *>(a.cd[r])[i] = reinterpret_cast<const uint64_t *>(a.cs[r])[i];
    if ((int)t < a.nsel) a.modes_dev[t] = a.modes[t];
}
constexpr int PIT_GT_THREADS = 1024;
template <typename R>
__global__ void __launch_bounds__(PIT_GT_THREADS) pit_gauge_kernel(const double *gph, int S, int nsel, PitCtrl *c, double *theta, const double *pw, int nb, int method, const Cx<R> *sy0,
                                                                   int want_corr, const PitModel *model = nullptr, const float4 *ualpha = nullptr, float2 *uq = nullptr,
                                                                   const R *mu = nullptr, int64_t T = 0, const float *Msum = nullptr)
{
    QH_WAVE_FIRST();
    if (c->done) return;
    constexpr int NT = PIT_GT_THREADS;
    __shared__ double redp[NT / 64];
    __shared__ double2 gbuf[NT / 64];
    __shared__ float4 abuf[NT / 64];
    if (gridDim.x > 1 && blockIdx.x == 1 && !(model && uq)) return;
    if (model && uq && (gridDim.x == 1 || blockIdx.x == 1)) {
        const bool corr = c->passes == 0 ? true : c->corr_on != 0;
        const int len = (S + NT - 1) / NT;
        const int s0 = threadIdx.x * len, s1 = s0 + len < S ? s0 + len : S;
        const float muT = mu ? (float)((double)*mu * (double)T) : 0.f;
        auto op = [](float4 e, float4 l) { return float4{l.x * e.x, l.x * e.y + l.y, l.z * e.z, l.z * e.w + l.w}; };
        for (int j = 0; j < nsel; j++) {
            const PitModel m = model[j];
            const bool on = corr && m.ok;
            auto cf = [&](int s, float &c1, float &c2) {
                const float t = Msum ? Msum[(size_t)s * nsel + j] : muT;
                c1 = on ? __expf(-fmaxf(m.k1, 0.f) * t) : 0.f; c2 = on ? __expf(-fmaxf(m.k2, 0.f) * t) : 0.f;
            };
            float4 loc{1.f, 0.f, 1.f, 0.f};
            for (int s = s0; s < s1; s++) {
                float b1 = 0.f, b2 = 0.f, c1 = 0.f, c2 = 0.f;
                if (s > 0) { const float4 al = ualpha[(size_t)(s - 1) * nsel + j]; b1 = m.q11 * al.x + m.q21 * al.y; b2 = m.q12 * al.x + m.q22 * al.y; cf(s - 1, c1, c2); }
                loc = op(loc, float4{c1, b1, c2, b2});
            }
            const float4 pre = block_scan_excl<float4, decltype(op), NT>(loc, op, float4{1.f, 0.f, 1.f, 0.f}, abuf);
            float r1 = pre.y, r2 = pre.w;
            for (int s = s0; s < s1; s++) {
                float b1 = 0.f, b2 = 0.f, c1 = 0.f, c2 = 0.f;
                if (s > 0) { const float4 al = ualpha[(size_t)(s - 1) * nsel + j]; b1 = m.q11 * al.x + m.q21 * al.y; b2 = m.q12 * al.x + m.q22 * al.y; cf(s - 1, c1, c2); }
                r1 = c1 * r1 + b1; r2 = c2 * r2 + b2;
                uq[(size_t)s * nsel + j] = float2{m.q11 * r1 + m.q12 * r2, m.q21 * r1 + m.q22 * r2};
            }
        }
        if (gridDim.x > 1) return;
    }
    if (c->passes == 0) {
        double ps = 0;
        for (int i = threadIdx.x; i < nb; i += NT) ps += pw[i];
        for (int o = 32; o > 0; o >>= 1) ps += __shfl_xor(ps, o);
        if ((threadIdx.x & 63) == 0) redp[threadIdx.x >> 6] = ps;
        __syncthreads();
        if (threadIdx.x == 0) {
            double tot = 0;
            for (int w = 0; w < NT / 64; w++) tot += redp[w];
            const double Py = tot / (nb > 0 ? nb : 1);
            double g = pit_gain<R>(method, Py, sy0[0]);
            if (model) {
                double gs = 0; int ng = 0;
                for (int j = 0; j < nsel; j++) if (model[j].ok) { gs += (double)model[j].g; ng++; }
                if (ng == nsel && gs > 0) g = gs / ng;
            }
            c->out_power = Py; c->gain = g;
            c->corr_on = (want_corr && g > 0 && g == g) ? 1 : 0;
        }
        __syncthreads();
    }
    const int len = (S + NT - 1) / NT;
    const int s0 = threadIdx.x * len, s1 = s0 + len < S ? s0 + len : S;
    auto cm = [](double2 x, double2 y) { return double2{x.x * y.x - x.y * y.y, x.x * y.y + x.y * y.x}; };
    const double2 *g2 = reinterpret_cast<const double2 *>(gph);
    double2 *th2 = reinterpret_cast<double2 *>(theta);
    if (len <= 4 && nsel <= 2) {
        double2 g[2][4];
#pragma unroll
        for (int j = 0; j < 2; j++)
#pragma unroll
            for (int q = 0; q < 4; q++) {
                const int s = s0 + q;
                g[j][q] = (j < nsel && s < s1 && s > 0) ? g2[(size_t)(s - 1) * nsel + j] : double2{1.0, 0.0};
            }
#pragma unroll
        for (int j = 0; j < 2; j++) {
            if (j >= nsel) break;
            const double2 prod = cm(cm(g[j][0], g[j][1]), cm(g[j][2], g[j][3]));
            double2 run = block_scan_excl<double2, decltype(cm), NT>(prod, cm, double2{1.0, 0.0}, gbuf);
#pragma unroll
            for (int q = 0; q < 4; q++) {
                const int s = s0 + q;
                run = cm(run, g[j][q]);
                if (s < s1) {
                    const double r = rsqrt(run.x * run.x + run.y * run.y);
                    th2[(size_t)s * nsel + j] = double2{run.x * r, run.y * r};
                }
            }
        }
        return;
    }
    for (int j = 0; j < nsel; j++) {
        double2 prod{1.0, 0.0};
        for (int s = s0; s < s1; s++)
            if (s > 0) prod = cm(prod, g2[(size_t)(s - 1) * nsel + j]);
        double2 run = block_scan_excl<double2, decltype(cm), NT>(prod, cm, double2{1.0, 0.0}, gbuf);
        for (int s = s0; s < s1; s++) {
            if (s > 0) run = cm(run, g2[(size_t)(s - 1) * nsel + j]);
            const double r = rsqrt(run.x * run.x + run.y * run.y);
            th2[(size_t)s * nsel + j] = double2{run.x * r, run.y * r};
        }
    }
}
template <typename R>
__global__ void __launch_bounds__(256) pit_devest_kernel(const Zf *D, const double *lam, int n, int ncol, const PitCtrl *c, float *devmax, unsigned *ticket, PitDecideArgs<R> da)
{
    QH_WAVE_FIRST();
    if (c->done) return;
    __shared__ float part[2][4][64], red[64], reds[64], redt[64], redm[64];
    const int cl = threadIdx.x & 63, kg = threadIdx.x >> 6;
    const int col = blockIdx.x * 64 + cl;
    float acc = 0.f, tap = 0.f;
    if (col < ncol) {
#pragma unroll 8
        for (int k = kg; k < n; k += 4) {
            const Zf v = D[(size_t)k * ncol + col];
            const float l = (float)lam[k], m2 = v.x * v.x + v.y * v.y;
            acc += (l > 0.f ? l : 0.f) * m2;
            tap += m2;
        }
    }
    part[0][kg][cl] = acc; part[1][kg][cl] = tap;
    __syncthreads();
    if (kg == 0) {
        acc = (part[0][0][cl] + part[0][1][cl]) + (part[0][2][cl] + part[0][3][cl]);
        tap = (part[1][0][cl] + part[1][1][cl]) + (part[1][2][cl] + part[1][3][cl]);
        red[cl] = (acc == acc) ? acc : 3.0e38f;
        reds[cl] = (acc == acc) ? acc : 3.0e38f;
        redt[cl] = (tap == tap) ? tap : 3.0e38f;
        redm[cl] = (tap == tap) ? tap : 3.0e38f;
    }
    __syncthreads();
    for (int s = 32; s > 0; s >>= 1) {
        if (threadIdx.x < s) {
            red[threadIdx.x] = red[threadIdx.x] > red[threadIdx.x + s] ? red[threadIdx.x] : red[threadIdx.x + s];
            reds[threadIdx.x] += reds[threadIdx.x + s];
            redt[threadIdx.x] += redt[threadIdx.x + s];
            redm[threadIdx.x] = redm[threadIdx.x] > redm[threadIdx.x + s] ? redm[threadIdx.x] : redm[threadIdx.x + s];
        }
        __syncthreads();
    }
    if (threadIdx.x == 0) {
        devmax[4 * blockIdx.x] = red[0]; devmax[4 * blockIdx.x + 1] = reds[0]; devmax[4 * blockIdx.x + 2] = redt[0]; devmax[4 * blockIdx.x + 3] = redm[0];
    }
    __shared__ int last;
    if (threadIdx.x == 0) {
        __threadfence();
        const unsigned t = atomicAdd(ticket, 1u);
        last = t == gridDim.x - 1;
        if (last) { *ticket = 0; __threadfence(); }
    }
    __syncthreads();
    if (!last) return;
    pit_decide_body<R>(da);
}
static __global__ void __launch_bounds__(256) pit_front_kernel(const Zf *D, const double *lam, int n, int ncol, double thr, int *front, int *bad)
{
    QH_WAVE_FIRST();
    const int col = blockIdx.x * 256 + threadIdx.x;
    if (col >= ncol) return;
    float acc = 0.f;
    for (int k = 0; k < n; k++) { const Zf v = D[(size_t)k * ncol + col]; const float l = (float)lam[k]; acc += (l > 0.f ? l : 0.f) * (v.x * v.x + v.y * v.y); }
    if (!(acc == acc) || acc > 1e30f) { atomicMax(bad, 1); return; }
    if ((double)acc > thr) atomicMax(front, col);
}
struct PitTiming { int npass; float pass_ms[QH_PIT_MAXPASS]; float acq_ms; };
inline PitTiming &pit_timing() { static thread_local PitTiming t; return t; }
constexpr int PIT_NEV = (QH_PIT_MAXPASS > QH_PIT_MAXCHUNK ? QH_PIT_MAXPASS : QH_PIT_MAXCHUNK) + 1;
struct PitEvents { hipEvent_t t0[PIT_NEV], t1[PIT_NEV], flag[PIT_NEV]; int32_t *hflag; float *hview; bool ok; };
inline PitEvents &pit_events()
{
    static thread_local PitEvents e = {{nullptr}, {nullptr}, {nullptr}, nullptr, nullptr, false};
    if (!e.ok) {
        for (int i = 0; i < PIT_NEV; i++) { (void)hipEventCreate(&e.t0[i]); (void)hipEventCreate(&e.t1[i]); (void)hipEventCreateWithFlags(&e.flag[i], hipEventDisableTiming); }
        (void)hipHostMalloc((void **)&e.hflag, PIT_NEV * sizeof(int32_t), hipHostMallocDefault);
        (void)hipHostMalloc((void **)&e.hview, 2 * PIT_NEV * sizeof(float), hipHostMallocCoherent);
        e.ok = e.hflag != nullptr && e.hview != nullptr;
    }
    return e;
}

inline int pit_auto_segments(int64_t TrSyms, double mu, int nsel, int cold)
{
    double target = (cold ? 0.45 : 0.4) / (mu > 1e-12 ? mu : 1e-12);
    if (target < 256) target = 256;
    if (target > 1048576) target = 1048576;
    const int64_t seg = ((int64_t)target + 63) / 64 * 64;
    int64_t St = TrSyms / seg;
    if (St > PIT_MAXSEG) St = PIT_MAXSEG;
    if (St < 4) return 1;
    if (nsel < 1) nsel = 1;
    const int64_t cap = cold ? 896 : 1024;
    auto cost = [&](int64_t S) {
        const int64_t chains = S * nsel;
        const bool l16 = chains <= 4096;
        const int64_t waves = (chains + (l16 ? 3 : 7)) / (l16 ? 4 : 8);
        return (double)((waves + cap - 1) / cap) * (double)(TrSyms / S) * (l16 ? 303.0 : 428.0);
    };
    int64_t best = St;
    double cbest = cost(St);
    auto consider = [&](int64_t S) {
        if (S < 4 || S > PIT_MAXSEG || S > St) return;
        const double c = cost(S);
        if (c < cbest * 0.999 || (c < cbest * 1.001 && S > best)) { best = S; cbest = c; }
    };
    const int64_t S16 = cap * 4 / nsel, S8 = cap * 8 / nsel;
    if (S16 * nsel <= 4096) consider(S16 < St ? S16 : St);
    for (int64_t r = 1; r * S8 <= St && r <= 64; r++) consider(r * S8);
    return (int)best;
}

inline size_t pit_basis_bytes(int ntot) { return (size_t)ntot * sizeof(double) + 2 * (size_t)ntot * ntot * sizeof(Zf); }
inline bool pit_basis_ok(int ntot, size_t elem) { return ntot <= PIT_EIGMAX && (size_t)PIT_COVW * ntot * elem <= 64 * 1024; }
struct PitBasisSync { hipEvent_t in = nullptr, out = nullptr; bool pending = false; };
inline PitBasisSync &pit_basis_sync() { static thread_local PitBasisSync b; return b; }
template <typename R>
int pit_basis(const void *E, int nmodes, int64_t L, int os, int ntaps, int64_t TrSyms, void *basis, int overlap = 0)
{
    int rc = ensure_init();
    if (rc) return rc;
    hipStream_t st = g_stream;
    PitBasisSync &bs = pit_basis_sync();
    if (overlap) {
        if (!bs.in) { QH_HIP(hipEventCreateWithFlags(&bs.in, hipEventDisableTiming)); QH_HIP(hipEventCreateWithFlags(&bs.out, hipEventDisableTiming)); }
        st = side_stream();
        QH_HIP(hipEventRecord(bs.in, g_stream));
        QH_HIP(hipStreamWaitEvent(st, bs.in, 0));
    }
    const int ntot = nmodes * ntaps;
    QH_REQUIRE(pit_basis_ok(ntot, sizeof(Cx<R>)), "pit basis: nmodes*ntaps too large for the eigen-solver");
    QH_REQUIRE(TrSyms >= 1 && (TrSyms - 1) * os + ntaps <= L, "pit basis: field shorter than TrSyms*os + ntaps");
    const size_t msz = (size_t)ntot * ntot;
    void *cb = nullptr;
    if ((rc = scratch(9, (1 + (size_t)PIT_COVB) * msz * sizeof(Z), &cb))) return rc;
    Z *Rc = (Z *)cb, *part = Rc + msz;
    const int ncov = (int)(TrSyms < PIT_COVW * PIT_COVB ? TrSyms : PIT_COVW * PIT_COVB);
    const int ept = (int)((msz + 255) / 256);
    const size_t lds = (size_t)PIT_COVW * ntot * sizeof(Cx<R>);
    if (ept <= 8) hipLaunchKernelGGL((pit_cov_kernel<R, 8>), dim3(PIT_COVB), dim3(256), lds, st, (const Cx<R> *)E, nmodes, L, os, ntaps, TrSyms, ncov, part);
    else if (ept <= 32) hipLaunchKernelGGL((pit_cov_kernel<R, 32>), dim3(PIT_COVB), dim3(256), lds, st, (const Cx<R> *)E, nmodes, L, os, ntaps, TrSyms, ncov, part);
    else hipLaunchKernelGGL((pit_cov_kernel<R, 64>), dim3(PIT_COVB), dim3(256), lds, st, (const Cx<R> *)E, nmodes, L, os, ntaps, TrSyms, ncov, part);
    hipLaunchKernelGGL(pit_cov_reduce_kernel, dim3((unsigned)((msz + 63) / 64)), dim3(256), 0, st, (const Z *)part, (int)msz, PIT_COVB, Rc);
    static std::atomic<bool> attr_set{false};
    if (!attr_set.load(std::memory_order_acquire)) { QH_HIP(hipFuncSetAttribute((const void *)pit_jacobi_kernel, hipFuncAttributeMaxDynamicSharedMemorySize, 160 * 1024 - 256)); attr_set.store(true, std::memory_order_release); }
    const int nsweep = PIT_EIGSWEEPS;
    float4 *glog = nullptr;
    const bool logged = true;
    const size_t jlds = (size_t)ntot * (ntot + 1) * sizeof(Zf) + 256;
    {
        void *gl = nullptr;
        const int mm = (ntot + 1) & ~1;
        if ((rc = scratch(11, (size_t)nsweep * (mm - 1) * (mm / 2) * sizeof(float4) + 64, &gl))) return rc;
        glog = (float4 *)gl;
    }
    const size_t blds = 2 * (size_t)ntot * (ntot + 1) * sizeof(Zf) + 256;
    if (logged && blds <= 160 * 1024 - 2048) {
        static std::atomic<bool> battr{false};
        if (!battr.load(std::memory_order_acquire)) { QH_HIP(hipFuncSetAttribute((const void *)pit_jacobi_blk_kernel, hipFuncAttributeMaxDynamicSharedMemorySize, 160 * 1024 - 2048)); battr.store(true, std::memory_order_release); }
        hipLaunchKernelGGL(pit_jacobi_blk_kernel, dim3(1), dim3(1024), blds, st, (const Z *)Rc, ntot, 1.0 / (double)ncov, (double *)basis, nsweep, glog);
    } else
    hipLaunchKernelGGL(pit_jacobi_kernel, dim3(1), dim3(1024), jlds, st, (const Z *)Rc, ntot, 1.0 / (double)ncov, (double *)basis,
                       (Zf *)((char *)basis + (size_t)ntot * sizeof(double)), nsweep, glog);
    if (glog) hipLaunchKernelGGL(pit_jacobi_v_kernel, dim3(ntot), dim3(64), 0, st, (const float4 *)glog, ntot, nsweep, (Zf *)((char *)basis + (size_t)ntot * sizeof(double)));
    QH_HIP(hipGetLastError());
    if (overlap) { QH_HIP(hipEventRecord(bs.out, st)); bs.pending = true; }
    return QH_OK;
}

inline qh_pit_opts pit_opts_default()
{
    qh_pit_opts o;
    memset(&o, 0, sizeof(o));
    o.phase_seed = -1; o.corr_beta = -1;
    return o;
}

template <typename R> inline int64_t pit_acq_chunk(R mu_acq)
{
    const double m = (double)mu_acq > 1e-12 ? (double)mu_acq : 1e-12;
    const int64_t c = (int64_t)1 << (int)floor(log2(2.0 / m) + 0.5);
    return c < 256 ? 256 : (c > 4096 ? 4096 : c);
}

struct PitPlan {
    PitSeg sg;
    double gear, bound, plateau, anneal;
    int64_t acq_ch = 0, amax = 0;
    int64_t CH = 0, ngram = 0;
    int nchunks = 0;
    void acquisition(const qh_pit_opts &o, int64_t TrSyms, int64_t chunk)
    {
        acq_ch = (chunk + LA_B - 1) / LA_B * LA_B;
        amax = o.acq_max > 0 ? o.acq_max : 2 * acq_ch;
        if (amax > TrSyms / 2 && o.acq_max <= 0) amax = TrSyms / 2;
        if (amax > TrSyms) amax = TrSyms;
        ngram = (amax / LA_B + 1) * LA_B < TrSyms ? (amax / LA_B + 1) * LA_B : TrSyms;
        CH = acq_ch;
        if (CH * QH_PIT_MAXCHUNK < amax) CH = (amax + QH_PIT_MAXCHUNK - 1) / QH_PIT_MAXCHUNK;
        CH = (CH + LA_B - 1) / LA_B * LA_B;
        if (CH < 4 * LA_B) CH = 4 * LA_B;
        nchunks = (int)(amax / CH);
    }
};
inline PitPlan pit_plan(const qh_pit_opts &o, int64_t TrSyms, int64_t head, int S, bool adaptive, int64_t chunk)
{
    PitPlan p;
    const int64_t nblk_all = (TrSyms - head) / LA_B;
// ... 11 lines not shown
    if (chunk > 0) p.acquisition(o, TrSyms, chunk);
    return p;
}

template <typename R>
int pit_acq_enqueue(const PitPlan &pl, const LaArgs<R> *la, bool use_bi, const TrainArgs<R> *ta, Cx<R> *wx, Cx<R> *err, int64_t err_pitch,
                    PitCtrl *ctrl, R *mu_acq, const R *mu_dev, const int64_t *modes_dev, int nsel)
{
    for (int c = 0; c < pl.nchunks; c++) {
        const int64_t step0 = (int64_t)c * pl.CH;
        int rc;
        if (la) {
            LaArgs<R> lp = *la;
            lp.E = la->E + step0 * la->os; lp.L = la->L - step0 * la->os; lp.TrSyms = pl.CH; lp.nch = 1; lp.wx = wx; lp.wx_cs = 0;
            lp.G = la->G + step0 * (la->gpair ? LA_B : GRAM_TRI / 2 / LA_B); lp.err = err; lp.err_pitch = err_pitch; lp.err_off = step0;
            lp.mu = mu_acq; lp.skip = &ctrl->acq_done;
            rc = use_bi ? launch_bi<R>(lp) : launch_la<R>(lp);
        } else {
            TrainArgs<R> tp = *ta;
            tp.wx = wx; tp.err = err; tp.mu = mu_acq; tp.nseg = 1; tp.seg_begin = step0; tp.seg_len = pl.CH; tp.seg_iter = 0; tp.skip = &ctrl->acq_done;
            rc = launch_any<R>(tp);
        }
        if (rc) return rc;
        hipLaunchKernelGGL((pit_acq_monitor_kernel<R>), dim3(1), dim3(256), 0, g_stream, (const Cx<R> *)err, err_pitch, step0, pl.CH, nsel, modes_dev,
                           pl.plateau, ctrl, mu_acq, mu_dev, pl.anneal);
    }
    return QH_OK;
}

struct PitPrepLayout { size_t ctrl, mu_acq, modes, wx, w0, err, gram, total; int64_t err_pitch; };
template <typename R> inline PitPrepLayout pit_prep_layout(int nmodes, int ntaps, int64_t acq_steps)
{
    PitPrepLayout l;
    auto up = [](size_t x) { return (x + 255) / 256 * 256; };
    const size_t wset = (size_t)nmodes * nmodes * ntaps * sizeof(Cx<R>);
    l.err_pitch = (acq_steps + LA_B + 63) / 64 * 64;
    l.ctrl = 0; l.mu_acq = up(sizeof(PitCtrl)); l.modes = l.mu_acq + 64; l.wx = up(l.modes + 128); l.w0 = up(l.wx + wset);
    l.err = up(l.w0 + wset); l.gram = up(l.err + (size_t)nmodes * l.err_pitch * sizeof(Cx<R>));
    l.total = up(l.gram + gram_bytes<R>(l.err_pitch));
    return l;
}
template <typename R> __global__ void __launch_bounds__(256) pit_adopt_kernel(Cx<R> *wx, const Cx<R> *wx_prep, int n, const PitCtrl *p, PitCtrl *c, R *mu_acq, const R *mu_acq_prep)
{
    QH_WAVE_FIRST();
    const int i = blockIdx.x * blockDim.x + threadIdx.x;
    if (!p->diverged && i < n) wx[i] = wx_prep[i];
    if (i == 0) {
        c->acq_chunks = p->acq_chunks; c->acq_steps = p->acq_steps; c->acq_done = 1; c->diverged = p->diverged; c->mu_acq = p->mu_acq;
        for (int q = 0; q < QH_PIT_MAXCHUNK; q++) c->acq_err[q] = p->acq_err[q];
        *mu_acq = *mu_acq_prep;
    }
}
template <typename R>
int pit_prepare(const void *E, int nmodes, int64_t L, int64_t TrSyms, int os, const R *mu_dev, const void *wx0, int ntaps, const int64_t *modes, int nsel,
                const void *symbols, int64_t nsy, int method, const qh_pit_opts *opts, void *prep, size_t prep_bytes)
{
    int rc = ensure_init();
    if (rc) return rc;
    if ((rc = train_args_ok("pit prepare", method, nmodes, ntaps, os, TrSyms, 1, nsel, nsy, modes))) return rc;
    QH_REQUIRE(opts && prep, "pit prepare: options and a preparation buffer are needed");
    QH_REQUIRE(TrSyms >= 1, "pit prepare: bad sizes");
    QH_REQUIRE((TrSyms - 1) * os + ntaps <= L, "pit prepare: field shorter than TrSyms*os + ntaps");
    const qh_pit_opts &o = *opts;
    QH_REQUIRE(o.acquire != 0 && o.adaptive == 0 && o.segments > 1 && o.mu_hint > 0 && o.acq_chunk > 0 && o.head_steps == 0 && !o.exchange,
               "pit prepare: not preparable (a cold fixed-step sweep with segments, mu_hint and acq_chunk given)");
    const int ntot = nmodes * ntaps;
    const PitPlan pl = pit_plan(o, TrSyms, 0, o.segments, false, o.acq_chunk);
    const PitSeg &sg = pl.sg;
    QH_REQUIRE(sg.S >= 2, "pit prepare: not preparable (nothing to parallelise)");
    const char *not_prep = "pit prepare: not preparable (throughput-form passes, block-form acquisition, blind error function)";
    QH_REQUIRE(!(method == QH_M_SBD || method == QH_M_MDDMA || method == QH_M_DD || method == QH_M_SBD_DATA), not_prep);
    TrainerForm f;
    if ((rc = trainer_form<R>(f, FORM_PASSES, method, 0, nmodes, ntaps, os, sg.len, (int64_t)sg.S * nsel, symbols, nsy, modes, nsel))) return rc;
    QH_REQUIRE(f.seg && f.block && la_shape_ok(nmodes, ntaps, os), not_prep);
    const PitPrepLayout lay = pit_prep_layout<R>(nmodes, ntaps, pl.amax);
    QH_REQUIRE(prep_bytes >= lay.total, "pit prepare: preparation buffer too small (qh_pit_prepare_bytes)");
    char *pb = (char *)prep;
    PitCtrl *ctrl = (PitCtrl *)(pb + lay.ctrl);
    R *mu_acq = (R *)(pb + lay.mu_acq);
    int64_t *modes_dev = (int64_t *)(pb + lay.modes);
    Cx<R> *wxp = (Cx<R> *)(pb + lay.wx), *w0 = (Cx<R> *)(pb + lay.w0), *errp = (Cx<R> *)(pb + lay.err);
    const size_t wset = (size_t)nmodes * ntot, wbytes = wset * sizeof(Cx<R>);
    const int64_t npow = L < 4096 ? L : 4096;
    hipLaunchKernelGGL((pit_setup_kernel<R>), dim3(1), dim3(256), 0, g_stream, (const Cx<R> *)E, nmodes, L, npow, ntot, mu_dev, pl.gear, pl.bound, o.tol > 0 ? o.tol : 1e-3, sg, ctrl, mu_acq);
    PitInit init{};
    init.cd[0] = wxp; init.cs[0] = wx0; init.cn[0] = (unsigned)wbytes;
    init.cd[1] = w0; init.cs[1] = wx0; init.cn[1] = (unsigned)wbytes;
    init.modes_dev = modes_dev; init.nsel = nsel;
    for (int j = 0; j < 16; j++) init.modes[j] = j < nsel ? modes[j] : 0;
    hipLaunchKernelGGL(pit_init_kernel, dim3(32), dim3(256), 0, g_stream, init);
    QH_REQUIRE(pl.ngram <= lay.err_pitch, "pit prepare: acquisition range exceeds the preparation buffer");
    void *G = nullptr;
    rc = f.pair_tab ? gram_build<R>(E, nmodes, L, os, ntaps, pl.ngram, &G, 1, 0, 0, pb + lay.gram) : QH_ERR_ARG;
    if (rc) return rc;
    LaArgs<R> la = la_args<R>(E, L, nmodes, ntaps, os, modes, nsel, method, symbols, nsy, mu_acq, errp, lay.err_pitch);
    la.G = (const GramPair<R> *)G; la.gpair = 1;
    if ((rc = pit_acq_enqueue<R>(pl, &la, f.use_bi, nullptr, wxp, errp, lay.err_pitch, ctrl, mu_acq, mu_dev, modes_dev, nsel))) return rc;
    hipLaunchKernelGGL((pit_acq_finish_kernel<R>), dim3((unsigned)((wset + 255) / 256)), dim3(256), 0, g_stream, wxp, (const Cx<R> *)w0, (int)wset, ctrl);
    QH_HIP(hipGetLastError());
    return QH_OK;
}

template <typename R>
int train_pit_dev(const void *E, int nmodes, int64_t L, int64_t TrSyms, int Niter, int os, R *mu_dev, void *wx, int ntaps,
                  const int64_t *modes, int nsel, const void *symbols, int64_t nsy, int method, void *err, int zero_err,
                  const void *gram, const qh_pit_opts *opts, void *report_dev, int depth = 0)
{
    int rc = ensure_init();
    if (rc) return rc;
    if ((rc = train_args_ok("train_equaliser", method, nmodes, ntaps, os, TrSyms, Niter, nsel, nsy, modes))) return rc;
    QH_REQUIRE(TrSyms == 0 || (TrSyms - 1) * os + ntaps <= L, "train_equaliser: field shorter than TrSyms*os + ntaps");
    qh_pit_opts o = opts ? *opts : pit_opts_default();
    auto exact_form = [&](PitCtrl *c, int ad, int zero, const void *g, int passes) -> int {
        int r = train_dev<R>(E, nmodes, L, TrSyms, Niter, os, mu_dev, wx, ntaps, modes, nsel, ad, symbols, nsy, method, err, zero, g);
        if (r) return r;
        const int32_t hdr[3] = {1, passes, 2};
        if (passes < 0) QH_HIP(hipMemcpyAsync(&c->converged, &hdr[2], sizeof(int32_t), hipMemcpyHostToDevice, g_stream));
        else QH_HIP(hipMemcpyAsync(&c->segments, hdr, sizeof(hdr), hipMemcpyHostToDevice, g_stream));
        QH_HIP(hipStreamSynchronize(g_stream));
        return QH_OK;
    };
    QH_REQUIRE(o.segments >= 0 && o.segments <= PIT_MAXSEG && o.max_passes >= 0 && o.max_passes <= QH_PIT_MAXPASS, "train_equaliser: bad segment / pass count");
    QH_REQUIRE(o.adaptive >= 0 && o.adaptive <= 2, "train_equaliser: adaptive must be 0, 1 or 2");
    bool adaptive = o.adaptive != 0;
    {
        bool exact_only = method == QH_M_SBD_DATA;
        if (adaptive && (o.adaptive == 2 || sizeof(R) != 4 || nsel != 1 || Niter != 1 || !seg_adaptive_supported(method))) exact_only = true;
        QH_REQUIRE(!(adaptive && o.exchange), "train_equaliser: a capture split over processes is trained with a fixed step");
        if (exact_only) {
            QH_REQUIRE(!o.exchange, "train_equaliser: a capture split over processes needs the parallel-in-time solver (blind / decision-directed method, fixed step)");
            void *cb0 = nullptr;
            if ((rc = scratch(8, sizeof(PitCtrl) + 64, &cb0))) return rc;
            PitCtrl *c0 = report_dev ? (PitCtrl *)report_dev : (PitCtrl *)cb0;
            PitSeg s1; s1.S = 1; s1.len = TrSyms; s1.extra = 0; s1.tail = 0;
            hipLaunchKernelGGL((pit_setup_kernel<R>), dim3(1), dim3(256), 0, g_stream, (const Cx<R> *)E, nmodes, L, (int64_t)(L < 4096 ? L : 4096), nmodes * ntaps, (const R *)mu_dev, 1.0, 1.0,
                               o.tol > 0 ? o.tol : 1e-3, s1, c0, (R *)((char *)cb0 + sizeof(PitCtrl)));
            return exact_form(c0, o.adaptive, zero_err, adaptive ? nullptr : gram, 0);
        }
    }
    if (adaptive) o.acquire = 0;
    const int ntot = nmodes * ntaps;
    const int npass = o.max_passes > 0 ? o.max_passes : (adaptive ? QH_PIT_MAXPASS : 16);
    const double tol = (o.tol > 0 ? o.tol : 1e-3) * (adaptive ? 1.0 / 3.0 : 1.0);
    const double safety = o.dev_safety > 0 ? o.dev_safety : PIT_DEV_SAFETY;
    const int sym = pit_symmetry(method);
    const bool seed_phase = o.phase_seed < 0 ? sym == 4 : o.phase_seed != 0;
    const bool want_corr = o.correction != 0 && pit_basis_ok(ntot, sizeof(Cx<R>));
    double beta = o.corr_beta >= 0 ? o.corr_beta : (sym == 0 ? 1.5 : 0.0);

    void *cbuf = nullptr;
    if ((rc = scratch(8, sizeof(PitCtrl) + 64, &cbuf))) return rc;
    PitCtrl *ctrl = report_dev ? (PitCtrl *)report_dev : (PitCtrl *)cbuf;
    R *mu_acq = (R *)((char *)cbuf + sizeof(PitCtrl));

    int S = o.segments;
    const float ad_relax = 1.0f, ad_damp = 0.7f;
    const int ad_newton = 1;
    const int64_t head_want = 16384;
    int64_t head = adaptive ? ((TrSyms / 4 < head_want ? TrSyms / 4 : head_want) / LA_B * LA_B) : 0;
    if (!adaptive && o.head_steps > 0) {
        QH_REQUIRE(!o.exchange, "train_equaliser: a capture split over processes takes no exact head");
        head = (int64_t)o.head_steps / LA_B * LA_B;
        if (head > TrSyms) head = TrSyms / LA_B * LA_B;
        o.acquire = 0;
    }
    int64_t seg_want = 2048;
    if (adaptive && !(method == QH_M_SBD || method == QH_M_MDDMA || method == QH_M_DD)) {
        const int64_t t = ((TrSyms - head) / 512 + LA_B - 1) / LA_B * LA_B;
        if (t > seg_want) seg_want = t;
    }
    if (S == 0 && adaptive) S = (int)((TrSyms - head) / seg_want < PIT_MAXSEG ? (TrSyms - head) / seg_want : PIT_MAXSEG);
    if (S == 0) {
        R mu_h = (R)o.mu_hint;
        if (!(o.mu_hint > 0)) {
            QH_HIP(hipMemcpyAsync(&mu_h, mu_dev, sizeof(R), hipMemcpyDeviceToHost, g_stream));
            QH_HIP(hipStreamSynchronize(g_stream));
        }
        S = pit_auto_segments(TrSyms, (double)mu_h, nsel, o.acquire);
    }
    PitPlan pl = pit_plan(o, TrSyms, head, S, adaptive, o.acquire ? o.acq_chunk : 0);
    const PitSeg &sg = pl.sg;
    if (zero_err) QH_HIP(hipMemsetAsync(err, 0, (size_t)nmodes * TrSyms * Niter * sizeof(Cx<R>), g_stream));
    const int64_t npow = L < 4096 ? L : 4096;
    hipLaunchKernelGGL((pit_setup_kernel<R>), dim3(1), dim3(256), 0, g_stream, (const Cx<R> *)E, nmodes, L, npow, ntot, (const R *)mu_dev, pl.gear, pl.bound, tol, sg, ctrl, mu_acq);
    QH_HIP(hipGetLastError());
    if (TrSyms == 0 || Niter == 0) return QH_OK;
    if (sg.S < 2) {
        const double zero = 0;
        QH_HIP(hipMemcpyAsync(&ctrl->defect[0], &zero, sizeof(double), hipMemcpyHostToDevice, g_stream));
        return exact_form(ctrl, adaptive ? 1 : 0, 0, gram, 1);
    }

    TrainerForm f;
    if ((rc = trainer_form<R>(f, FORM_PASSES, method, adaptive, nmodes, ntaps, os, sg.len, (int64_t)sg.S * nsel, symbols, nsy, modes, nsel))) return rc;
    if (adaptive && !f.seg) return exact_form(ctrl, 1, 0, nullptr, 0);
    const bool decision = method == QH_M_SBD || method == QH_M_MDDMA || method == QH_M_DD;
    const bool seg_form = f.seg, use_bi = f.use_bi, block_form = f.block, pair_tab = f.pair_tab;
    const bool split = o.exchange != nullptr;
    const int own_first = split ? o.seg_first : 0, own_count = split ? o.seg_count : sg.S;
    const bool xchg_async = split && o.exchange_on_stream != 0;
    if (split) {
        QH_REQUIRE(seg_form, "train_equaliser: a capture split over processes needs the throughput form of the passes (>= 512 chains, supported tap layout)");
        QH_REQUIRE(own_first >= 0 && own_count >= 0 && own_first + own_count <= sg.S, "train_equaliser: owned segments outside the segment grid");
        QH_REQUIRE(Niter == 1, "train_equaliser: a capture split over processes is trained in one sweep");
    }

    const size_t wset = (size_t)nmodes * ntot;
    const size_t wbytes = wset * sizeof(Cx<R>);
    void *wbuf = nullptr;
    const size_t nsj = (size_t)sg.S * nsel;
    const size_t bytes_w = ((2 * (size_t)sg.S + 2) * wbytes + 63) / 64 * 64;
    if ((rc = scratch(2, bytes_w + 10 * nsj * sizeof(double) + (size_t)nsel * sizeof(int64_t) + 320 + nsj * 16 + 4 * ((nsj + 63) / 64) * sizeof(float) + 64, &wbuf))) return rc;
    Cx<R> *X = (Cx<R> *)wbuf, *Y = X + (size_t)sg.S * wset, *w_start = Y + (size_t)sg.S * wset, *w_call = w_start + wset;
    double *z = (double *)((char *)wbuf + bytes_w), *rot = z + 2 * nsj, *dfc = rot + 2 * nsj, *pw = dfc + nsj, *gph = pw + nsj, *theta = gph + 2 * nsj;
    int64_t *modes_dev = (int64_t *)(theta + 2 * nsj);
    double *uw_phi = (double *)(modes_dev + ((nsel + 7) / 8 * 8));
    int *uw_jump = (int *)(uw_phi + (size_t)sg.S * nsel);
    float *devmax = (float *)(uw_jump + (size_t)sg.S * nsel);
    const int ndev = (int)((nsj + 63) / 64);
    unsigned *ticket = (unsigned *)(devmax + 4 * (size_t)ndev);
    PitInit init{};
    init.z[0] = ticket; init.zn[0] = sizeof(unsigned);
    R *ad_rS = nullptr, *ad_rE = nullptr;
    Cx<R> *ad_eS = nullptr, *ad_eE = nullptr, *ad_errh = nullptr;
    float *ad_M = nullptr, *ad_chg = nullptr, *ad_rP = nullptr, *ad_dP = nullptr;
    if (!adaptive && head > 0) {
        void *ab = nullptr;
        if ((rc = scratch(13, (size_t)nmodes * head * sizeof(Cx<R>) + 64, &ab))) return rc;
        ad_errh = (Cx<R> *)ab;
    }
    if (adaptive) {
        void *ab = nullptr;
        const size_t nS = ((size_t)sg.S + 15) / 16 * 16;
        if ((rc = scratch(13, nS * (2 * sizeof(R) + 2 * sizeof(Cx<R>) + 3 * sizeof(float)) + 64 + (size_t)nmodes * head * sizeof(Cx<R>), &ab))) return rc;
        ad_eS = (Cx<R> *)ab; ad_eE = ad_eS + nS; ad_errh = ad_eE + nS;
        ad_rS = (R *)(ad_errh + (size_t)nmodes * head); ad_rE = ad_rS + nS;
        ad_M = (float *)(ad_rE + nS); ad_rP = ad_M + nS; ad_dP = ad_rP + nS; ad_chg = ad_dP + nS;
    }
    init.modes_dev = modes_dev; init.nsel = nsel;
    for (int j = 0; j < 16; j++) init.modes[j] = j < nsel ? modes[j] : 0;
    const bool prepared = o.prepared != nullptr && o.acquire && !adaptive && head == 0 && Niter >= 1;
    const bool need_mu = adaptive || !(o.mu_hint > 0), need_acq = o.acquire && !(o.acq_chunk > 0) && !prepared;
    R mu_acq_h = 0;
    if (need_acq) QH_HIP(hipMemcpyAsync(&mu_acq_h, mu_acq, sizeof(R), hipMemcpyDeviceToHost, g_stream));
    R mu_host = need_mu ? (R)1 : (R)o.mu_hint;
    if (need_mu) QH_HIP(hipMemcpyAsync(&mu_host, mu_dev, sizeof(R), hipMemcpyDeviceToHost, g_stream));
    if (need_mu || need_acq) QH_HIP(hipStreamSynchronize(g_stream));
    if (!adaptive && !(mu_host != 0))
        return exact_form(ctrl, 0, 0, gram, 0);
    if (o.acquire && !(o.acq_chunk > 0)) pl.acquisition(o, TrSyms, pit_acq_chunk(mu_acq_h));

    const int64_t amax = pl.amax;
    void *G = const_cast<void *>(gram);
    if (prepared) QH_REQUIRE(seg_form && o.acq_chunk > 0, "train_equaliser: a prepared acquisition belongs to throughput-form passes with acq_chunk given (qh_pit_prepare_*_dev said so)");
    if (block_form && !G && (!seg_form || amax > 0) && !prepared) {
        const int64_t n = seg_form ? pl.ngram : TrSyms;
        rc = pair_tab ? gram_build<R>(E, nmodes, L, os, ntaps, n, &G) : gram_cur_build<R>(E, nmodes, L, os, ntaps, n, &G);
        if (rc) return rc;
    }
    const int64_t g_per_step = pair_tab ? LA_B : GRAM_TRI / 2 / LA_B;

    const int ncol = sg.S * nsel;
    const double *lam = nullptr;
    const Zf *Vb = nullptr;
    Zf *Dz[2] = {nullptr, nullptr};
    Zf *Xe = nullptr, *Ye = nullptr, *Yprev = nullptr;
    if (want_corr) {
        void *cb = nullptr;
        if ((rc = scratch(10, pit_basis_bytes(ntot) + 4 * (size_t)ntot * ncol * sizeof(Zf) + (size_t)ntot * nsel * sizeof(Zf) + 256, &cb))) return rc;
        void *basis = o.basis ? o.basis : cb;
        if (!o.basis && (rc = pit_basis<R>(E, nmodes, L, os, ntaps, TrSyms, basis))) return rc;
        lam = (const double *)basis; Vb = (const Zf *)((const char *)basis + (size_t)ntot * sizeof(double));
        Dz[0] = (Zf *)((char *)cb + (pit_basis_bytes(ntot) + 63) / 64 * 64); Dz[1] = Dz[0] + (size_t)ntot * ncol;
        Xe = Dz[1] + (size_t)ntot * ncol; Ye = Xe + (size_t)ntot * ncol; Yprev = Ye + (size_t)ntot * ncol;
    }
    const bool eig = want_corr && sizeof(R) == 4 && form(FORM_PIT_PROBE) == 0;
    const bool tables_ok = method == QH_M_CMA || method == QH_M_SGNCMA || method == QH_M_MCMA || method == QH_M_RDE || method == QH_M_MRDE ||
                           (decision && (use_bi || seg_form));
    const bool ssb = eig && tables_ok && method != QH_M_CMA2;
    PitModel *model = nullptr;
    float4 *ualpha = nullptr;
    float2 *uqv = nullptr;
    PitModelArgs<R> ma;
    hipEvent_t model_event = nullptr;
    if (ssb) {
        void *mb = nullptr;
        const size_t pw_ = 2 * PIT_EIGMAX + 8;
        const size_t b_part = (size_t)PIT_MODB * 4 * nsel * pw_ * sizeof(float), b_u = ((size_t)nsel * ntot * sizeof(Cx<R>) + 63) / 64 * 64;
        const size_t b_ua = ((size_t)ncol * sizeof(float4) + 63) / 64 * 64, b_uq = ((size_t)ncol * sizeof(float2) + 63) / 64 * 64;
        if ((rc = scratch(14, b_part + b_u + b_ua + b_uq + 16 * sizeof(PitModel) + 128, &mb))) return rc;
        ma.part = (float *)mb; ma.u = (Cx<R> *)((char *)mb + b_part);
        ualpha = (float4 *)((char *)mb + b_part + b_u); uqv = (float2 *)((char *)ualpha + b_ua);
        model = (PitModel *)((char *)uqv + b_uq); ma.model = model; ma.ticket = (unsigned *)(model + 16);
        init.z[1] = ma.ticket; init.zn[1] = sizeof(unsigned);
        init.z[2] = ualpha; init.zn[2] = (unsigned)(b_ua + b_uq);
        ma.E = (const Cx<R> *)E; ma.wx = (const Cx<R> *)wx; ma.L = L; ma.TrSyms = TrSyms; ma.nmodes = nmodes; ma.ntaps = ntaps; ma.os = os; ma.nsel = nsel; ma.method = method;
        if (decision) { ma.symbols = (const Cx<R> *)f.dd_table; ma.nsy = 2 * f.dd_npart + 1; ma.sy_pitch = 2 * BI_DD_MAXLEV; ma.tables = 1; }
        else { ma.symbols = (const Cx<R> *)symbols; ma.nsy = nsy; ma.sy_pitch = nsy; ma.tables = (method == QH_M_RDE || method == QH_M_MRDE) ? 1 : 0; }
        for (int j = 0; j < 16; j++) ma.modes[j] = j < nsel ? modes[j] : 0;
        if (o.corr_beta < 0) beta = 0.0;
    }
    const size_t glds = ((size_t)PIT_EIGMAX * PIT_EIGMAX + (size_t)PIT_EIGMAX * PIT_GT) * sizeof(Zf);
    static std::atomic<bool> gemm_attr{false};
    if (want_corr && !gemm_attr.load(std::memory_order_acquire)) {
        QH_HIP(hipFuncSetAttribute((const void *)pit_cgemm_kernel<R, true>, hipFuncAttributeMaxDynamicSharedMemorySize, 160 * 1024 - 256));
        QH_HIP(hipFuncSetAttribute((const void *)pit_cgemm_kernel<R, false>, hipFuncAttributeMaxDynamicSharedMemorySize, 160 * 1024 - 256));
        QH_HIP(hipFuncSetAttribute((const void *)pit_basis_mfma_kernel<R, 0>, hipFuncAttributeMaxDynamicSharedMemorySize, 128 * 1024));
        QH_HIP(hipFuncSetAttribute((const void *)pit_basis_mfma_kernel<R, 1>, hipFuncAttributeMaxDynamicSharedMemorySize, 128 * 1024));
        gemm_attr.store(true, std::memory_order_release);
    }

    LaArgs<R> la = la_args<R>(E, L, nmodes, ntaps, os, modes, nsel, method, symbols, nsy, mu_dev, err, TrSyms * Niter);
    la.G = (const GramPair<R> *)G; la.gpair = pair_tab ? 1 : 0; la.wx_cs = (int64_t)wset;
    la.dd_general = f.dd_general;
    f.alphabet(la);
    const TrainArgs<R> ta = train_args<R>(E, L, nmodes, ntaps, os, TrSyms, Niter, modes, nsel, method, symbols, nsy, mu_dev, err);

    PitTiming &tm = pit_timing();
    tm.npass = 0; tm.acq_ms = 0;
    bool acq_timed = false;
    PitEvents &ev = pit_events();
    QH_REQUIRE(ev.ok, "train_equaliser: no pinned memory for the pass flags");
    const bool redo_ok = o.exact_redo_off == 0;
    bool fell_back = false;
    if (redo_ok && !adaptive) { init.cd[0] = w_call; init.cs[0] = wx; init.cn[0] = (unsigned)wbytes; }
    if (o.acquire && Niter > 0) { init.cd[1] = w_start; init.cs[1] = wx; init.cn[1] = (unsigned)wbytes; }
    hipLaunchKernelGGL(pit_init_kernel, dim3(32), dim3(256), 0, g_stream, init);
    QH_HIP(hipGetLastError());
    for (int it = 0; it < Niter; it++) {
        if (it == 0 && prepared) {
            const PitPrepLayout lay = pit_prep_layout<R>(nmodes, ntaps, amax);
            const char *pb = (const char *)o.prepared;
            hipLaunchKernelGGL((pit_adopt_kernel<R>), dim3((unsigned)((wset + 255) / 256)), dim3(256), 0, g_stream, (Cx<R> *)wx, (const Cx<R> *)(pb + lay.wx), (int)wset,
                               (const PitCtrl *)(pb + lay.ctrl), ctrl, mu_acq, (const R *)(pb + lay.mu_acq));
            QH_HIP(hipGetLastError());
        } else if (it == 0 && o.acquire) {
            if (pl.nchunks > 0) { QH_HIP(hipEventRecord(ev.t0[PIT_NEV - 1], g_stream)); acq_timed = true; }
            if ((rc = pit_acq_enqueue<R>(pl, block_form ? &la : nullptr, use_bi, &ta, (Cx<R> *)wx, (Cx<R> *)err, TrSyms * Niter, ctrl, mu_acq, mu_dev,
                                         modes_dev, nsel))) return rc;
            if (pl.nchunks > 0) QH_HIP(hipEventRecord(ev.t1[PIT_NEV - 1], g_stream));
            hipLaunchKernelGGL((pit_acq_finish_kernel<R>), dim3((unsigned)((wset + 255) / 256)), dim3(256), 0, g_stream, (Cx<R> *)wx, (const Cx<R> *)w_start, (int)wset, ctrl);
            QH_HIP(hipGetLastError());
        }
        if (adaptive) {
            QH_HIP(hipMemcpyAsync(w_start, wx, wbytes, hipMemcpyDeviceToDevice, g_stream));
            QH_HIP(hipMemcpyAsync(ad_chg + 1, mu_dev, sizeof(R), hipMemcpyDeviceToDevice, g_stream));
            if ((rc = train_dev<R>(E, nmodes, L, head, 1, os, mu_dev, wx, ntaps, modes, 1, 1, symbols, nsy, method, ad_errh, 0, nullptr))) return rc;
            QH_HIP(hipMemcpyAsync((Cx<R> *)err + (size_t)modes[0] * TrSyms, ad_errh + (size_t)modes[0] * head, (size_t)head * sizeof(Cx<R>), hipMemcpyDeviceToDevice, g_stream));
            hipLaunchKernelGGL((pit_adapt_init_kernel<R>), dim3((sg.S + 255) / 256), dim3(256), 0, g_stream, (const R *)mu_dev, (const Cx<R> *)(ad_errh + (size_t)modes[0] * head + head - 1),
                               sg.S, ad_rS, ad_eS);
            QH_HIP(hipGetLastError());
        }
        if (!adaptive && head > 0) {
            if ((rc = train_dev<R>(E, nmodes, L, head, 1, os, mu_dev, wx, ntaps, modes, nsel, 0, symbols, nsy, method, ad_errh, 0, nullptr))) return rc;
            for (int j = 0; j < nsel; j++)
                QH_HIP(hipMemcpyAsync((Cx<R> *)err + (size_t)modes[j] * TrSyms * Niter + (size_t)it * TrSyms, ad_errh + (size_t)modes[j] * head, (size_t)head * sizeof(Cx<R>),
                                      hipMemcpyDeviceToDevice, g_stream));
        }
        const double *rot_use = nullptr;
        if (seed_phase) {
            int nwin = PIT_SEEDWIN;
            auto phase_lds = [&](int nw) { return ((size_t)ntot + (size_t)nmodes * os * pit_phase_pitch(ntaps, os, nw)) * sizeof(Cx<R>); };
            while (nwin > 32 && phase_lds(nwin) > 60 * 1024) nwin /= 2;
            QH_REQUIRE(phase_lds(nwin) <= 60 * 1024, "train_equaliser: phase seeding does not fit the LDS for this filter shape (pass phase_seed = 0)");
            hipLaunchKernelGGL((pit_phase_kernel<R>), dim3(sg.S, nsel), dim3(256), phase_lds(nwin), g_stream, (const Cx<R> *)E, nmodes, L, os,
                               (const Cx<R> *)wx, ntaps, sg, (const int64_t *)modes_dev, nwin, z);
            hipLaunchKernelGGL(pit_unwrap_kernel, dim3(nsel), dim3(256), 0, g_stream, (const double *)z, sg.S, nsel, rot, uw_phi, uw_jump);
            rot_use = rot;
        }
        const Cx<R> *w_exact = o.start == 1 ? nullptr : ((it == 0 && o.acquire) ? (const Cx<R> *)w_start : (const Cx<R> *)wx);
        hipLaunchKernelGGL((pit_seed_kernel<R>), dim3(sg.S), dim3(256), 0, g_stream, (const Cx<R> *)wx, nmodes, ntot, (const int64_t *)modes_dev, nsel, rot_use, X, w_exact, Y, ctrl);
        if (ssb) {
            ma.sg = sg; ma.rot = rot_use;
            static thread_local hipEvent_t ev_seed = nullptr, ev_model = nullptr;
            if (!ev_seed) { QH_HIP(hipEventCreateWithFlags(&ev_seed, hipEventDisableTiming)); QH_HIP(hipEventCreateWithFlags(&ev_model, hipEventDisableTiming)); }
            hipStream_t ss = helper_stream();
            QH_HIP(hipEventRecord(ev_seed, g_stream));
            QH_HIP(hipStreamWaitEvent(ss, ev_seed, 0));
            hipLaunchKernelGGL((pit_model_kernel<R, 0>), dim3(PIT_MODB), dim3(256), 0, ss, ma);
            hipLaunchKernelGGL((pit_model_kernel<R, 1>), dim3(PIT_MODB), dim3(256), 0, ss, ma);
            QH_HIP(hipEventRecord(ev_model, ss));
            model_event = ev_model;
        }
        QH_HIP(hipGetLastError());
        const int timing_mode = pit_timing_mode();
        auto decide_args = [&](int p, const float *dm, const float2 *ye, float2 *yprev, int ne, int ncol_e, int corr_wanted) {
            PitDecideArgs<R> d;
            d.dfc = dfc; d.pw = pw; d.nb = (int)((sg.S - 1) * nsel); d.Ylast = (const Cx<R> *)(Y + (size_t)(sg.S - 1) * wset); d.n = (int)wset; d.wx = (Cx<R> *)wx; d.c = ctrl;
            d.host_view = &ev.hview[2 * p]; d.nrow = nsel; d.devmax = dm; d.ndev = ndev; d.safety = safety; d.Ye = ye; d.Yprev = yprev; d.ne = ne; d.ncol_e = ncol_e;
            d.theta = theta; d.modes_dev = (const int64_t *)modes_dev; d.ntot_w = ntot; d.S = (int)sg.S; d.sym = sym; d.corr_wanted = corr_wanted;
            d.extra = adaptive ? (const float *)ad_chg : nullptr;
            d.Dfin = (ye && !adaptive) ? (const float2 *)Dz[1] : nullptr; d.Vfin = (const float2 *)Vb; d.lam_fin = lam;
            d.stall_from = adaptive ? 5 : 2;
            return d;
        };
        auto timed = [&](int p) { return timing_mode == 2 || (timing_mode == 1 && p == 1); };
        auto enqueue_pass = [&](int p) -> int {
            ((volatile float *)ev.hview)[2 * p] = -1.f;
            PitFuse<R> fz;
            fz.X = X; fz.Y = Y; fz.theta = theta; fz.modes_dev = (const int64_t *)modes_dev; fz.nmodes = nmodes; fz.nsel = nsel;
            fz.damp = (adaptive && p > 1) ? ad_damp : 1.f;
            if (p > 0 && want_corr) {
                if (eig)
                    hipLaunchKernelGGL((pit_basis_mfma_kernel<R, 1>), dim3((ncol + PIT_MC - 1) / PIT_MC), dim3(pit_mfma_threads(ntot)), pit_mfma_lds(ntot), g_stream, Vb + (size_t)ntot * ntot,
                                       (const Cx<R> *)nullptr, (const Zf *)Dz[1], (Zf *)nullptr, ntot, ncol, (const PitCtrl *)ctrl, fz);
                else
                    hipLaunchKernelGGL((pit_cgemm_kernel<R, false>), dim3((ncol + PIT_GT - 1) / PIT_GT), dim3(256), glds, g_stream, Vb + (size_t)ntot * ntot, (const Zf *)Dz[1], (Zf *)nullptr, ntot, ncol, (const PitCtrl *)ctrl, fz);
                QH_HIP(hipGetLastError());
            } else if (p > 0) {
                QH_HIP(hipMemcpyAsync(X + wset, Y, (size_t)(sg.S - 1) * wbytes, hipMemcpyDeviceToDevice, g_stream));
                QH_HIP(hipMemcpyAsync(Y, X, (size_t)sg.S * wbytes, hipMemcpyDeviceToDevice, g_stream));
            }
            if (o.on_pass) {
                hipStream_t keep = g_stream;
                o.on_pass(o.on_pass_user, it, p);
                g_stream = keep;
            }
            if (timed(p)) QH_HIP(hipEventRecord(ev.t0[p], g_stream));
            if (seg_form) {
                SegArgs<R> sa{};
                sa.E = (const Cx<R> *)E; sa.wx = Y; sa.symbols = la.symbols; sa.err = (Cx<R> *)err; sa.mu = mu_dev;
                sa.L = L; sa.TrSyms = TrSyms; sa.nsy = la.nsy; sa.sy_pitch = la.sy_pitch; sa.err_pitch = TrSyms * Niter; sa.err_off = (int64_t)it * TrSyms;
                sa.nmodes = nmodes; sa.ntaps = ntaps; sa.os = os; sa.nsel = nsel; sa.S = sg.S;
                sa.seg_len = sg.len; sa.seg_extra = sg.extra; sa.seg_tail = sg.tail; sa.seg_begin = sg.begin;
                sa.r_in = ad_rS; sa.r_out = ad_rE; sa.e_in = ad_eS; sa.e_out = ad_eE; sa.mu_sum = (R *)ad_M; sa.adapt_first = sg.begin > 0 ? 1 : 0;
                for (int j = 0; j < 16; j++) sa.modes[j] = j < nsel ? modes[j] : 0;
                sa.skip = &ctrl->done;
                sa.q_first = own_first * nsel; sa.q_count = split ? own_count * nsel : 0;
                if (!split || own_count > 0) { int r = launch_seg<R>(sa, method, adaptive); if (r) return r; }
                if (adaptive) hipLaunchKernelGGL((pit_adapt_scan_kernel<R>), dim3(1), dim3(1024), 0, g_stream, ad_rS, (const R *)ad_rE, ad_eS, (const Cx<R> *)ad_eE, sg.S, ad_chg, (const PitCtrl *)ctrl, ad_relax, ad_rP, ad_dP, ad_newton);
            } else if (block_form) {
                LaArgs<R> ls = la;
                ls.TrSyms = sg.len; ls.nch = sg.S; ls.wx = Y; ls.err_off = (int64_t)it * TrSyms; ls.seg = 1; ls.seg_extra = sg.extra; ls.seg_tail = sg.tail;
                ls.skip = &ctrl->done;
                if (sg.begin > 0) {
                    ls.E = (const Cx<R> *)E + sg.begin * os; ls.L = L - sg.begin * os; ls.err_off += sg.begin;
                    ls.G = (const GramPair<R> *)G + sg.begin * g_per_step;
                }
                { int r = use_bi ? launch_bi<R>(ls) : launch_la<R>(ls); if (r) return r; }
            } else {
                TrainArgs<R> ts = ta;
                ts.wx = Y; ts.nseg = sg.S; ts.seg_begin = sg.begin; ts.seg_len = sg.len; ts.seg_extra = sg.extra; ts.seg_tail = sg.tail; ts.seg_iter = it; ts.skip = &ctrl->done;
                { int r = launch_any<R>(ts); if (r) return r; }
            }
            if (timed(p)) QH_HIP(hipEventRecord(ev.t1[p], g_stream));
            if (split) {
                if (own_first > 0) QH_HIP(hipMemsetAsync(Y, 0, (size_t)own_first * wbytes, g_stream));
                if (own_first + own_count < sg.S)
                    QH_HIP(hipMemsetAsync(Y + (size_t)(own_first + own_count) * wset, 0, (size_t)(sg.S - own_first - own_count) * wbytes, g_stream));
                if (!xchg_async) QH_HIP(hipStreamSynchronize(g_stream));
                if (o.exchange(o.exchange_user, Y, (size_t)sg.S * wbytes) != 0) { set_error("train_equaliser: the exchange callback failed"); return QH_ERR_ARG; }
            }
            const int nbnd = (int)((sg.S - 1) * nsel);
            if (eig) {
                if (o.basis && pit_basis_sync().pending) {
                    QH_HIP(hipStreamWaitEvent(g_stream, pit_basis_sync().out, 0));
                    pit_basis_sync().pending = false;
                }
                auto forward2 = [&](const Cx<R> *src, Zf *dst, const Cx<R> *src2, Zf *dst2) {
                    PitFuse<R> f2 = fz;
                    f2.T2 = src2; f2.Out2 = reinterpret_cast<float2 *>(dst2);
                    hipLaunchKernelGGL((pit_basis_mfma_kernel<R, 0>), dim3(2 * ((ncol + PIT_MC - 1) / PIT_MC)), dim3(pit_mfma_threads(ntot)), pit_mfma_lds(ntot), g_stream, Vb, src, (const Zf *)nullptr, dst, ntot, ncol, (const PitCtrl *)ctrl, f2);
                };
                if (p == 0 && model_event) QH_HIP(hipStreamWaitEvent(g_stream, model_event, 0));
                forward2((const Cx<R> *)X, Xe, (const Cx<R> *)Y, Ye);
                hipLaunchKernelGGL(pit_bound_kernel, dim3((nbnd + nsel + 3) / 4), dim3(256), 0, g_stream, (const Zf *)Xe, (const Zf *)Ye, (const Zf *)Yprev, lam, ntot, sg.S, nsel, sym,
                                   (const PitCtrl *)ctrl, dfc, pw, gph, ualpha);
                hipLaunchKernelGGL((pit_gauge_kernel<R>), dim3(ssb ? 2 : 1), dim3(PIT_GT_THREADS), 0, g_stream, (const double *)gph, sg.S, nsel, ctrl, theta, (const double *)pw,
                                   nbnd, method, (const Cx<R> *)symbols + (size_t)modes[0] * nsy, 1, (const PitModel *)model, (const float4 *)ualpha, uqv,
                                   (const R *)mu_dev, sg.len, (const float *)ad_M);
                hipLaunchKernelGGL((pit_recur_eig_kernel<R>), dim3(ntot, nsel), dim3(PIT_RT), 0, g_stream, Xe, (const Zf *)Ye, Dz[1], (const double *)theta, lam, nsel, sg.S, sg.len,
                                   (const R *)mu_dev, beta, (const PitCtrl *)ctrl, (const float *)ad_M, (adaptive && p >= 1) ? ad_damp : 1.f,
                                   (const float4 *)ualpha, (const float2 *)uqv);
                hipLaunchKernelGGL((pit_devest_kernel<R>), dim3(ndev), dim3(256), 0, g_stream, (const Zf *)Dz[1], lam, ntot, ncol, (const PitCtrl *)ctrl, devmax, ticket,
                                   decide_args(p, (const float *)devmax, (const float2 *)Ye, (float2 *)Yprev, ntot, ncol, 1));
            } else {
            const size_t dlds = (2 * (size_t)ntot + (size_t)nmodes * os * pit_phase_pitch(ntaps, os, PIT_PROBE)) * sizeof(Cx<R>);
            QH_REQUIRE(dlds <= 60 * 1024, "train_equaliser: boundary probe does not fit the LDS for this filter shape");
            hipLaunchKernelGGL((pit_defect_kernel<R>), dim3(sg.S, nsel), dim3(PIT_PROBE), dlds, g_stream, (const Cx<R> *)E, nmodes, L, os,
                               ntaps, sg, TrSyms, (const int64_t *)modes_dev, (const Cx<R> *)X, (const Cx<R> *)Y, sym, (const PitCtrl *)ctrl, dfc, pw, gph, (const Cx<R> *)wx);
            hipLaunchKernelGGL((pit_gauge_kernel<R>), dim3(1), dim3(PIT_GT_THREADS), 0, g_stream, (const double *)gph, sg.S, nsel, ctrl, theta, (const double *)pw,
                               nbnd, method, (const Cx<R> *)symbols + (size_t)modes[0] * nsy, want_corr ? 1 : 0);
            if (want_corr) {
                if (o.basis && pit_basis_sync().pending) {
                    QH_HIP(hipStreamWaitEvent(g_stream, pit_basis_sync().out, 0));
                    pit_basis_sync().pending = false;
                }
                hipLaunchKernelGGL((pit_cgemm_kernel<R, true>), dim3((ncol + PIT_GT - 1) / PIT_GT), dim3(256), glds, g_stream, Vb, (const Zf *)nullptr, Dz[1], ntot, ncol, (const PitCtrl *)ctrl, fz);
                hipLaunchKernelGGL((pit_recur_kernel<R>), dim3(ntot, nsel), dim3(256), 0, g_stream, Dz[1], lam, nsel, sg.S, sg.len, (const R *)mu_dev, beta, (const PitCtrl *)ctrl);
                hipLaunchKernelGGL((pit_devest_kernel<R>), dim3(ndev), dim3(256), 0, g_stream, (const Zf *)Dz[1], lam, ntot, ncol, (const PitCtrl *)ctrl, devmax, ticket,
                                   decide_args(p, (const float *)devmax, (const float2 *)nullptr, (float2 *)nullptr, 0, 0, 1));
            } else
                hipLaunchKernelGGL((pit_decide_kernel<R>), dim3(1), dim3(256), 0, g_stream, decide_args(p, (const float *)nullptr, (const float2 *)nullptr, (float2 *)nullptr, 0, 0, 0));
            }
            QH_HIP(hipGetLastError());
            return QH_OK;
        };
        if ((rc = enqueue_pass(0))) return rc;
        if (it == 0 && o.on_pass0) {
            hipStream_t keep = g_stream;
            o.on_pass0(o.on_pass0_user);
            g_stream = keep;
        }
        bool ahead = false;
        bool certified = false;
        for (int p = 0; p < npass; p++) {
            double contr = PIT_CONTRACT;
            if (p >= 2 && ev.hview[2 * (p - 2) + 1] > 0) {
                contr = (double)ev.hview[2 * (p - 1) + 1] / (double)ev.hview[2 * (p - 2) + 1];
                contr = contr < 0.1 ? 0.1 : (contr > 0.9 ? 0.9 : contr);
            }
            const bool expect_last = p > 0 && contr * (double)ev.hview[2 * (p - 1) + 1] < tol;
            ahead = false;
            if (p + 1 < npass && !expect_last && (!split || xchg_async)) { if ((rc = enqueue_pass(p + 1))) return rc; ahead = true; }
            {
                volatile float *hv = (volatile float *)ev.hview;
                unsigned spins = 0;
                auto t_last = std::chrono::steady_clock::now();
                while (hv[2 * p] < 0.f) {
                    if ((++spins & 255u) != 0) continue;
                    const auto now = std::chrono::steady_clock::now();
                    if (now - t_last < std::chrono::milliseconds(20)) continue;
                    t_last = now;
                    const hipError_t q = hipStreamQuery(g_stream);
                    if (q == hipSuccess) { if (hv[2 * p] < 0.f) hv[2 * p] = 2.f; break; }
                    if (q != hipErrorNotReady) QH_HIP(q);
                }
                std::atomic_thread_fence(std::memory_order_acquire);
            }
            if (timed(p) && tm.npass < QH_PIT_MAXPASS) {
                float ms = 0;
                QH_HIP(hipEventSynchronize(ev.t1[p]));
                QH_HIP(hipEventElapsedTime(&ms, ev.t0[p], ev.t1[p]));
                tm.pass_ms[tm.npass++] = ms;
            }
            if (ev.hview[2 * p] != 0.f) { certified = ev.hview[2 * p] == 1.f; break; }
            if (p + 1 < npass && !ahead && (rc = enqueue_pass(p + 1))) return rc;
        }
        if (acq_timed) {
            float ms = 0;
            QH_HIP(hipEventSynchronize(ev.t1[PIT_NEV - 1]));
            QH_HIP(hipEventElapsedTime(&ms, ev.t0[PIT_NEV - 1], ev.t1[PIT_NEV - 1]));
            tm.acq_ms = ms; acq_timed = false;
        }
        if (!adaptive && !certified && redo_ok && !split && depth < 3 && o.head_auto_off == 0) {
            double hp = 0;
            int hfront[2] = {-1, 0};
            bool finite = false;
            if (eig) {
                int *fr = (int *)(ticket + 4);
                QH_HIP(hipMemcpyAsync(&hp, &ctrl->out_power, sizeof(double), hipMemcpyDeviceToHost, g_stream));
                QH_HIP(hipStreamSynchronize(g_stream));
                QH_HIP(hipMemcpyAsync(fr, hfront, sizeof(hfront), hipMemcpyHostToDevice, g_stream));
                hipLaunchKernelGGL(pit_front_kernel, dim3((ncol + 255) / 256), dim3(256), 0, g_stream, (const Zf *)Dz[1], lam, ntot, ncol, tol * tol * (hp > 0 ? hp : 1.0), fr, fr + 1);
                QH_HIP(hipMemcpyAsync(hfront, fr, sizeof(hfront), hipMemcpyDeviceToHost, g_stream));
                QH_HIP(hipStreamSynchronize(g_stream));
                finite = hp > 0 && hfront[1] == 0;
            }
            const int front = hfront[0];
            const int64_t front_seg = front < 0 ? -1 : front / nsel + 1;
            if (eig && finite && front >= 0 && front_seg <= sg.S / 4) {
                int64_t hs = front_seg + 8 + (front_seg + 1) / 2;
                if (hs > sg.S - 4) hs = sg.S - 4;
                const int64_t new_head = sg.start(hs);
                if (new_head > head && new_head < TrSyms && new_head <= 0x7fffffff) {
                    QH_HIP(hipMemcpyAsync(wx, w_call, wbytes, hipMemcpyDeviceToDevice, g_stream));
                    qh_pit_opts o2 = opts ? *opts : pit_opts_default();
                    o2.head_steps = (int32_t)new_head; o2.acquire = 0; o2.segments = 0;
                    return train_pit_dev<R>(E, nmodes, L, TrSyms, Niter, os, mu_dev, wx, ntaps, modes, nsel, symbols, nsy, method, err, 0, gram, &o2, report_dev, depth + 1);
                }
            }
        }
        if (!adaptive && !certified && redo_ok) {
            QH_HIP(hipMemcpyAsync(wx, w_call, wbytes, hipMemcpyDeviceToDevice, g_stream));
            if ((rc = exact_form(ctrl, 0, 0, gram, -1))) return rc;
            fell_back = true;
            break;
        }
        if (adaptive) {
            hipLaunchKernelGGL((pit_adapt_finish_kernel<R>), dim3(1), dim3(1), 0, g_stream, mu_dev, (const R *)ad_rE, sg.S);
            int32_t conv = 0;
            QH_HIP(hipMemcpyAsync(&conv, &ctrl->converged, sizeof(conv), hipMemcpyDeviceToHost, g_stream));
            QH_HIP(hipStreamSynchronize(g_stream));
            if (!conv && redo_ok) {
                fell_back = true;
                QH_HIP(hipMemcpyAsync(wx, w_start, wbytes, hipMemcpyDeviceToDevice, g_stream));
                QH_HIP(hipMemcpyAsync(mu_dev, ad_chg + 1, sizeof(R), hipMemcpyDeviceToDevice, g_stream));
                if ((rc = exact_form(ctrl, 1, 0, nullptr, -1))) return rc;
            }
        }
        if (sym == 0 && !fell_back)
            hipLaunchKernelGGL((pit_rotate_err_kernel<R>), dim3(sg.S, nsel), dim3(256), 0, g_stream, (Cx<R> *)err, (int64_t)(TrSyms * Niter), (int64_t)it * TrSyms, sg,
                               (const int64_t *)modes_dev, nsel, (const double *)theta, (const PitCtrl *)ctrl, -1);
        QH_HIP(hipGetLastError());
    }
    return QH_OK;
}

inline qh_pit_report &last_host_report() { static thread_local qh_pit_report r; return r; }
template <typename R>
int train_host_tier_b(const void *E, int nmodes, int64_t L, int64_t TrSyms, int Niter, int os, R *mu, void *wx, int ntaps,
                      const int64_t *modes, int nsel, int adaptive, const void *symbols, int64_t nsy, int method, void *err, double tol)
{
    int rc = ensure_init();
    if (rc) return rc;
    if ((rc = train_args_ok("train_equaliser", method, nmodes, ntaps, os, TrSyms, Niter, nsel, nsy, modes))) return rc;
    QH_REQUIRE(L >= 1, "train_equaliser: bad sizes");
    const size_t cs = sizeof(Cx<R>);
    bool cold = true;
    {
        const Cx<R> *w = (const Cx<R> *)wx;
        const size_t ntot = (size_t)nmodes * ntaps;
        for (int j = 0; j < nsel && cold; j++) {
            int nz = 0;
            for (size_t f = 0; f < ntot; f++) {
                const Cx<R> v = w[(size_t)modes[j] * ntot + f];
                if (v.re != 0 || v.im != 0) { nz++; if (!(v.re == 1 && v.im == 0)) nz = 2; }
                if (nz > 1) break;
            }
            cold = nz == 1;
        }
    }
    DevBuf dE, dw, ds, de, dmu, drep;
    if ((rc = dE.from_host(E, (size_t)nmodes * L * cs))) return rc;
    if ((rc = dw.from_host(wx, (size_t)nmodes * nmodes * ntaps * cs))) return rc;
    if ((rc = ds.from_host(symbols, (size_t)nmodes * nsy * cs))) return rc;
    if ((rc = dmu.from_host(mu, sizeof(R)))) return rc;
    if ((rc = de.alloc((size_t)nmodes * TrSyms * Niter * cs))) return rc;
    if ((rc = drep.alloc(sizeof(qh_pit_report)))) return rc;
    QH_HIP(hipMemsetAsync(drep.p, 0, sizeof(qh_pit_report), g_stream));
    qh_pit_opts o = pit_opts_default();
    o.correction = -1;
    o.tol = tol;
    o.adaptive = adaptive;
    if (adaptive == 1) {
        for (int j = 0; j < nsel; j++)
            if ((rc = train_pit_dev<R>(dE.p, nmodes, L, TrSyms, Niter, os, (R *)dmu.p, dw.p, ntaps, modes + j, 1, ds.p, nsy, method, de.p, j == 0 ? 1 : 0, nullptr, &o, drep.p))) return rc;
    } else {
        o.acquire = cold ? 1 : 0;
        if (!adaptive && *mu > 0) o.mu_hint = (double)*mu;
        if (!adaptive && *mu > 0) o.segments = pit_auto_segments(TrSyms, (double)*mu, nsel, o.acquire);
        if ((rc = train_pit_dev<R>(dE.p, nmodes, L, TrSyms, Niter, os, (R *)dmu.p, dw.p, ntaps, modes, nsel, ds.p, nsy, method, de.p, 1, nullptr, &o, drep.p))) return rc;
    }
    if ((rc = dw.to_host(wx, dw.n))) return rc;
    if ((rc = de.to_host(err, de.n))) return rc;
    if ((rc = dmu.to_host(mu, sizeof(R)))) return rc;
    if ((rc = drep.to_host(&last_host_report(), sizeof(qh_pit_report)))) return rc;
    QH_HIP(hipStreamSynchronize(g_stream));
    return QH_OK;
}

}
```

Baseline: 1207.

## Fuse PIT analysis pass into a single persistent kernel with grid barriers

Refactors the bound, gauge, recurrence, deviation-estimate, decide and basis kernels into device bodies. They are then run inside one resident pit_analysis_kernel that steps through the stages using software grid barriers in a sync word. This targets the per-pass kernel launch overhead and inter-kernel gaps in the eigen-path PIT analysis. It adds an abandon flag and polling limits, and carries deadlock and occupancy risk if not all blocks are co-resident.

```diff
diff --git a/qampy_amd/csrc/api.hip b/qampy_amd/csrc/api.hip
--- a/qampy_amd/csrc/api.hip
+++ b/qampy_amd/csrc/api.hip
@@ -109,7 +109,7 @@
 struct FormName { const char *key, *env; };
 static const FormName FORM_NAMES[FORM_COUNT] = {
     {"trainer", "QAMPY_HIP_TRAINER"}, {"pit_form", "QAMPY_HIP_PIT_FORM"}, {"seg_lanes", "QAMPY_HIP_SEG_LANES"}, {"pit_probe", "QAMPY_HIP_PIT_PROBE"},
-    {"bps", "QAMPY_HIP_BPS"}};
+    {"bps", "QAMPY_HIP_BPS"}, {"pit_analysis", "QAMPY_HIP_PIT_ANALYSIS"}};
 static int form_parse(int k, const char *v, int *out)
 {
     if (!v || !v[0]) { *out = 0; return 0; }
@@ -117,6 +117,7 @@
     case FORM_TRAINER: *out = v[0] == 'd' ? 1 : (v[0] == 'l' ? 2 : (v[0] == 'i' ? 3 : (v[0] == 'a' || v[0] == '0' ? 0 : -1))); break;
     case FORM_PIT: *out = v[0] == 's' ? 1 : (v[0] == 'b' ? 2 : (v[0] == 'a' || v[0] == '0' ? 0 : -1)); break;
     case FORM_SEG_LANES: { const int n = atoi(v); *out = (n == 8 || n == 16 || n == 0) ? n : -1; break; }
+    case FORM_PIT_ANALYSIS: *out = v[0] == 'l' ? 1 : (v[0] == 'e' ? 2 : (v[0] == 'a' || v[0] == '0' ? 0 : -1)); break;
     case FORM_BPS: *out = v[0] == 't' ? 1 : (v[0] == 'l' ? 2 : (v[0] == 'a' || v[0] == '0' ? 0 : -1)); break;
     default: *out = atoi(v) != 0 ? 1 : 0; break;
     }
diff --git a/qampy_amd/csrc/common.h b/qampy_amd/csrc/common.h
--- a/qampy_amd/csrc/common.h
+++ b/qampy_amd/csrc/common.h
@@ -27,7 +27,7 @@
 int ensure_init();
 hipStream_t side_stream();
 hipStream_t helper_stream();
-enum FormKey { FORM_TRAINER = 0, FORM_PIT, FORM_SEG_LANES, FORM_PIT_PROBE, FORM_BPS, FORM_COUNT };
+enum FormKey { FORM_TRAINER = 0, FORM_PIT, FORM_SEG_LANES, FORM_PIT_PROBE, FORM_BPS, FORM_PIT_ANALYSIS, FORM_COUNT };
 int form(FormKey k);
 const char *trainer_force();
 double gram_budget_gb();
diff --git a/qampy_amd/csrc/train_pit.h b/qampy_amd/csrc/train_pit.h
--- a/qampy_amd/csrc/train_pit.h
+++ b/qampy_amd/csrc/train_pit.h
@@ -232,13 +232,14 @@
 
 template <typename R>
 __global__ void __launch_bounds__(256) pit_seed_kernel(const Cx<R> *wx, int nmodes, int ntot, const int64_t *modes_dev, int nsel, const double *rot, Cx<R> *X,
-                                                       const Cx<R> *w0, Cx<R> *Y, PitCtrl *c)
+                                                       const Cx<R> *w0, Cx<R> *Y, PitCtrl *c, unsigned *sync_words = nullptr)
 {
     QH_WAVE_FIRST();
     const int s = blockIdx.x;
     const int n = nmodes * ntot;
     if (s == 0 && c) {
         if (threadIdx.x == 0) { c->done = 0; c->converged = 0; c->passes = 0; }
+        if (threadIdx.x == 0 && sync_words) { sync_words[0] = 0u; sync_words[1] = 0u; }
         for (int q = threadIdx.x; q < QH_PIT_MAXPASS; q += 256) {
             c->result_change[q] = -1; c->deviation[q] = -1; c->deviation_rms[q] = -1; c->deviation_taps[q] = -1; c->deviation_taps_worst[q] = -1; c->defect[q] = -1;
         }
@@ -379,7 +380,7 @@
     const float *extra;
 };
 constexpr int PIT_FIN_MAX = 128;
-template <typename R> __device__ __forceinline__ void pit_decide_body(const PitDecideArgs<R> &a)
+template <typename R> __device__ __forceinline__ void pit_decide_body(const PitDecideArgs<R> &a, const int tid, const bool act)
 {
     const double *dfc = a.dfc; const int nb = a.nb; const Cx<R> *Ylast = a.Ylast; const int n = a.n; Cx<R> *wx = a.wx; PitCtrl *c = a.c; float *host_view = a.host_view;
     const int nrow = a.nrow; const float *devmax = a.devmax; const int ndev = a.ndev; const double safety = a.safety; const float2 *Ye = a.Ye; float2 *Yprev = a.Yprev;
@@ -389,21 +390,21 @@
     const double c_seg_len = (double)c->seg_len;
     const int pl = p - 1 < QH_PIT_MAXPASS ? p - 1 : QH_PIT_MAXPASS - 1, pl2 = p - 2 < QH_PIT_MAXPASS ? p - 2 : QH_PIT_MAXPASS - 1;
     const double drms1 = p >= 1 ? c->deviation_rms[pl] : 0.0, drms2 = p >= 2 ? c->deviation_rms[pl2] : 0.0, dfc2 = p >= 2 ? c->defect[pl2] : 0.0;
-    if (Yprev)
-        for (int e = threadIdx.x; e < ne * nrow; e += 256) { const int k = e / nrow, j = e - k * nrow; Yprev[e] = Ye[(size_t)k * ncol_e + (ncol_e - nrow) + j]; }
+    if (Yprev && act)
+        for (int e = tid; e < ne * nrow; e += 256) { const int k = e / nrow, j = e - k * nrow; Yprev[e] = Ye[(size_t)k * ncol_e + (ncol_e - nrow) + j]; }
     __shared__ double red[4], redd[4], reds[4], redt[4], redw[4], redm[4];
     __shared__ int s_flag[2];
     __shared__ float s_crit;
     double m = 0, dv = 0, ds = 0, dt = 0, wn = 0, dm = 0;
-    for (int i0 = threadIdx.x; i0 < nb; i0 += 8 * 256) {
+    for (int i0 = act ? tid : nb; i0 < nb; i0 += 8 * 256) {
         double v[8];
 #pragma unroll
         for (int q = 0; q < 8; q++) v[q] = i0 + 256 * q < nb ? dfc[i0 + 256 * q] : 0.0;
 #pragma unroll
         for (int q = 0; q < 8; q++) m = (v[q] > m || !(v[q] == v[q])) ? (v[q] == v[q] ? v[q] : 1e30) : m;
     }
-    if (devmax)
-        for (int i = threadIdx.x; i < ndev; i += 256) {
+    if (devmax && act)
+        for (int i = tid; i < ndev; i += 256) {
             const double v = (double)devmax[4 * i];
             dv = (v > dv || !(v == v)) ? (v == v ? v : 1e30) : dv;
             ds += (double)devmax[4 * i + 1];
@@ -414,7 +415,7 @@
     double chg = 0;
     for (int r = 0; r < nrow; r++) { const double v = dfc[nb + r]; chg = (v > chg || !(v == v)) ? v : chg; }
     const bool extrap = a.Dfin != nullptr && p >= 1 && corr_on0 && c_gain > 0;
-    for (int e = threadIdx.x; e < n; e += 256) {
+    for (int e = act ? tid : n; e < n; e += 256) {
         Cx<R> v = Ylast[e];
         wn += (double)v.re * v.re + (double)v.im * v.im;
         const int row = e / ntot_w;
@@ -431,17 +432,17 @@
         m = m > m2 ? m : m2; dv = dv > dv2 ? dv : dv2; dm = dm > dm2 ? dm : dm2;
         ds += __shfl_xor(ds, o); dt += __shfl_xor(dt, o); wn += __shfl_xor(wn, o);
     }
-    if ((threadIdx.x & 63) == 0) {
-        const int w = threadIdx.x >> 6;
+    if (act && (tid & 63) == 0) {
+        const int w = tid >> 6;
         red[w] = m; redd[w] = dv; reds[w] = ds; redt[w] = dt; redw[w] = wn; redm[w] = dm;
     }
     __syncthreads();
-    if (threadIdx.x == 0)
+    if (tid == 0)
         for (int w = 1; w < 4; w++) {
             red[0] = red[0] > red[w] ? red[0] : red[w]; redd[0] = redd[0] > redd[w] ? redd[0] : redd[w]; redm[0] = redm[0] > redm[w] ? redm[0] : redm[w];
             reds[0] += reds[w]; redt[0] += redt[w]; redw[0] += redw[w];
         }
-    if (threadIdx.x == 0) {
+    if (tid == 0) {
         const bool have_dev = devmax != nullptr && corr_on0 && c_out_power > 0;
         const double dev = have_dev ? sqrt(redd[0] / c_out_power) : -1.0;
         const double dev_rms = have_dev ? sqrt(reds[0] / ((double)(nb + nrow) * c_out_power)) : -1.0;
@@ -486,7 +487,7 @@
         const float2 *VT = a.Vfin + (size_t)ntot_w * ntot_w;
         for (int jj = 0; jj < nrow; jj++) {
             const size_t col = (size_t)(S - 1) * nrow + jj;
-            for (int k = threadIdx.x; k < ntot_w; k += 256) {
+            for (int k = act ? tid : ntot_w; k < ntot_w; k += 256) {
                 const double ak = c_mu * c_gain * c_seg_len * a.lam_fin[k];
                 const float ck = ak > 0 ? __expf(-(float)ak) : 1.f;
                 const float2 dk = a.Dfin[(size_t)k * ncol_e + col];
@@ -495,7 +496,7 @@
             __syncthreads();
             const int row = (int)modes_dev[jj];
             const double tr = theta[2 * ((size_t)(S - 1) * nrow + jj)], ti = theta[2 * ((size_t)(S - 1) * nrow + jj) + 1];
-            for (int f = threadIdx.x; f < ntot_w; f += 256) {
+            for (int f = act ? tid : ntot_w; f < ntot_w; f += 256) {
                 float dr = 0.f, di = 0.f;
 #pragma unroll 8
                 for (int k = 0; k < ntot_w; k++) {
@@ -512,7 +513,7 @@
         __threadfence();
     }
     __syncthreads();
-    if (threadIdx.x == 0) {
+    if (tid == 0) {
         host_view[1] = s_crit;
         __threadfence_system();
         __hip_atomic_store(&host_view[0], s_flag[0] ? (s_flag[1] ? 1.f : 2.f) : 0.f, __ATOMIC_RELEASE, __HIP_MEMORY_SCOPE_SYSTEM);
@@ -523,7 +524,7 @@
 {
     QH_WAVE_FIRST();
     if (a.c->done) return;
-    pit_decide_body<R>(a);
+    pit_decide_body<R>(a, (int)threadIdx.x, true);
 }
 
 template <typename R>
@@ -1157,24 +1158,21 @@
 inline int pit_mfma_threads(int n) { return 64 * ((n + 15) / 16); }
 inline size_t pit_mfma_lds(int n) { return ((size_t)(n + 4) * PIT_MBP + (size_t)PIT_MC * (PIT_EIGMAX + 1)) * sizeof(Zf); }
 template <typename R, int MODE>
-__global__ void __launch_bounds__(64 * (PIT_EIGMAX / 16)) pit_basis_mfma_kernel(const Zf *__restrict__ A2, const Cx<R> *__restrict__ T, const Zf *__restrict__ D, Zf *__restrict__ Out,
-                                                                               int n, int ncol, const PitCtrl *c, PitFuse<R> fz)
-{
-    QH_WAVE_FIRST();
-    if (c->done) return;
-    extern __shared__ __attribute__((aligned(16))) char pit_smem[];
+__device__ __forceinline__ void pit_basis_mfma_body(const int vb, const int tid, const int nt, const bool act, char *pit_smem, const Zf *A2, const Cx<R> *T, const Zf *D, Zf *Out,
+                                                    int n, int ncol, PitFuse<R> fz)
+{
     const int np = (n + 3) & ~3;
     Zf *Bs = reinterpret_cast<Zf *>(pit_smem);
     Zf *Ct = Bs + (size_t)(n + 4) * PIT_MBP;
-    const int tid = threadIdx.x, lane = tid & 63, wave = tid >> 6, nw = blockDim.x >> 6, nt = blockDim.x;
+    const int lane = tid & 63, wave = tid >> 6, nw = nt >> 6;
     const int nb1 = (ncol + PIT_MC - 1) / PIT_MC;
-    const bool second = MODE == 0 && (int)blockIdx.x >= nb1;
+    const bool second = MODE == 0 && vb >= nb1;
     if (second) { T = fz.T2; Out = reinterpret_cast<Zf *>(fz.Out2); }
-    const int col0 = ((int)blockIdx.x - (second ? nb1 : 0)) * PIT_MC;
+    const int col0 = (vb - (second ? nb1 : 0)) * PIT_MC;
     const size_t wset = (size_t)fz.nmodes * n;
     const int am = 16 * wave + (lane & 15), ak = lane >> 4;
     const Zf *ag = A2 + (size_t)ak * n + am;
-    auto lda = [&](int k) -> Zf { return (am < n && k + ak < n) ? ag[(size_t)k * n] : Zf{0.f, 0.f}; };
+    auto lda = [&](int k) -> Zf { return (act && am < n && k + ak < n) ? ag[(size_t)k * n] : Zf{0.f, 0.f}; };
     constexpr int PF = 8;
     Zf abuf[PF];
 #pragma unroll
@@ -1187,7 +1185,7 @@
             for (int q = 0; q < NCW; q++) {
                 const int cc = cb + wave + nw * q, col = col0 + cc;
                 tmp[q][0] = Zf{0.f, 0.f}; tmp[q][1] = Zf{0.f, 0.f};
-                if (cc < PIT_MC && col < ncol) {
+                if (act && cc < PIT_MC && col < ncol) {
                     const int s = col / fz.nsel, j = col - s * fz.nsel;
                     const Cx<R> *src = T + (size_t)s * wset + (size_t)fz.modes_dev[j] * n;
                     if (lane < n) { const Cx<R> t = src[lane]; tmp[q][0] = Zf{(float)t.re, (float)t.im}; }
@@ -1197,7 +1195,7 @@
 #pragma unroll
             for (int q = 0; q < NCW; q++) {
                 const int cc = cb + wave + nw * q;
-                if (cc < PIT_MC) {
+                if (act && cc < PIT_MC) {
                     if (lane < np) Bs[lane * PIT_MBP + cc] = tmp[q][0];
                     if (lane + 64 < np) Bs[(lane + 64) * PIT_MBP + cc] = tmp[q][1];
                 }
@@ -1205,7 +1203,7 @@
         }
     } else {
         const int cc = tid & 15, k0 = tid >> 4, kstep = nt >> 4;
-        const bool okc = col0 + cc < ncol;
+        const bool okc = act && col0 + cc < ncol;
         for (int kb = 0; kb < np; kb += 8 * kstep) {
             Zf tmp[8];
 #pragma unroll
@@ -1216,7 +1214,7 @@
 #pragma unroll
             for (int q = 0; q < 8; q++) {
                 const int k = kb + k0 + kstep * q;
-                if (k < np) Bs[k * PIT_MBP + cc] = tmp[q];
+                if (act && k < np) Bs[k * PIT_MBP + cc] = tmp[q];
             }
         }
     }
@@ -1228,7 +1226,7 @@
         for (int q = 0; q < NCW; q++) {
             const int cc = wave + nw * q, col = col0 + cc;
             xv[q][0] = Cx<R>{0, 0}; xv[q][1] = Cx<R>{0, 0}; th[q][0] = 1; th[q][1] = 0;
-            if (cc < PIT_MC && col < ncol) {
+            if (act && cc < PIT_MC && col < ncol) {
                 const int s = col / fz.nsel, j = col - s * fz.nsel;
                 const size_t base = (size_t)s * wset + (size_t)fz.modes_dev[j] * n;
                 th[q][0] = fz.theta[2 * (size_t)col]; th[q][1] = fz.theta[2 * (size_t)col + 1];
@@ -1240,7 +1238,7 @@
     __syncthreads();
     pit_f4 rr = {0.f, 0.f, 0.f, 0.f}, ii = rr, im = rr;
     const Zf *bp = Bs + (lane >> 4) * PIT_MBP + (lane & 15);
-    for (int k0 = 0; k0 < np; k0 += 4 * PF) {
+    for (int k0 = 0; act && k0 < np; k0 += 4 * PF) {
 #pragma unroll
         for (int i = 0; i < PF; i++) {
             const int k = k0 + 4 * i;
@@ -1262,20 +1260,20 @@
 #pragma unroll
         for (int q = 0; q < 4; q++) {
             const int m = 16 * wave + 4 * (lane >> 4) + q;
-            if (m < n && col < ncol) Out[(size_t)m * ncol + col] = Zf{rr[q] - ii[q], im[q]};
+            if (act && m < n && col < ncol) Out[(size_t)m * ncol + col] = Zf{rr[q] - ii[q], im[q]};
         }
     } else {
 #pragma unroll
         for (int q = 0; q < 4; q++) {
             const int m = 16 * wave + 4 * (lane >> 4) + q;
-            Ct[cl * (PIT_EIGMAX + 1) + m] = Zf{rr[q] - ii[q], im[q]};
+            if (act) Ct[cl * (PIT_EIGMAX + 1) + m] = Zf{rr[q] - ii[q], im[q]};
         }
         __syncthreads();
         for (int cb = 0; cb < PIT_MC; cb += NCW * nw) {
 #pragma unroll
             for (int q = 0; q < NCW; q++) {
                 const int cc = cb + wave + nw * q, col = col0 + cc;
-                if (cc < PIT_MC && col < ncol) {
+                if (act && cc < PIT_MC && col < ncol) {
                     const int s = col / fz.nsel, j = col - s * fz.nsel;
                     const size_t base = (size_t)s * wset + (size_t)fz.modes_dev[j] * n;
                     const double qr = pre ? th[q][0] : fz.theta[2 * (size_t)col], qi = pre ? th[q][1] : fz.theta[2 * (size_t)col + 1];
@@ -1295,13 +1293,19 @@
         }
     }
 }
-
-static __global__ void __launch_bounds__(256) pit_bound_kernel(const Zf *Xe, const Zf *Ye, const Zf *Yprev, const double *lam, int n, int S, int nsel, int sym,
-                                                              const PitCtrl *c, double *dfc, double *pw, double *gph, float4 *ualpha = nullptr)
+template <typename R, int MODE>
+__global__ void __launch_bounds__(64 * (PIT_EIGMAX / 16)) pit_basis_mfma_kernel(const Zf *__restrict__ A2, const Cx<R> *__restrict__ T, const Zf *__restrict__ D, Zf *__restrict__ Out,
+                                                                               int n, int ncol, const PitCtrl *c, PitFuse<R> fz)
 {
     QH_WAVE_FIRST();
     if (c->done) return;
-    const int lane = threadIdx.x & 63, bi = blockIdx.x * 4 + (threadIdx.x >> 6);
+    extern __shared__ __attribute__((aligned(16))) char pit_smem[];
+    pit_basis_mfma_body<R, MODE>((int)blockIdx.x, (int)threadIdx.x, (int)blockDim.x, true, pit_smem, A2, T, D, Out, n, ncol, fz);
+}
+
+static __device__ __forceinline__ void pit_bound_body(const int bi, const int lane, const Zf *Xe, const Zf *Ye, const Zf *Yprev, const double *lam, int n, int S, int nsel, int sym,
+                                                      const PitCtrl *c, double *dfc, double *pw, double *gph, float4 *ualpha)
+{
     const int nb = (S - 1) * nsel, ncol = S * nsel;
     if (bi >= nb + nsel) return;
     const bool result_probe = bi >= nb;
@@ -1368,17 +1372,20 @@
         dfc[bi] = (A == A && B == B) ? sqrt(d2 / (B > 1e-300 ? B : 1e-300)) : 1e30;
     }
 }
+static __global__ void __launch_bounds__(256) pit_bound_kernel(const Zf *Xe, const Zf *Ye, const Zf *Yprev, const double *lam, int n, int S, int nsel, int sym,
+                                                              const PitCtrl *c, double *dfc, double *pw, double *gph, float4 *ualpha = nullptr)
+{
+    QH_WAVE_FIRST();
+    if (c->done) return;
+    pit_bound_body((int)(blockIdx.x * 4 + (threadIdx.x >> 6)), (int)(threadIdx.x & 63), Xe, Ye, Yprev, lam, n, S, nsel, sym, c, dfc, pw, gph, ualpha);
+}
 
 constexpr int PIT_RT = 1024;
 template <typename R>
-__global__ void __launch_bounds__(PIT_RT) pit_recur_eig_kernel(Zf *Xe, const Zf *Ye, Zf *D, const double *theta, const double *lam, int nsel, int S, int64_t T, const R *mu,
-                                                               double beta, const PitCtrl *c, const float *Msum = nullptr, float damp = 1.f,
-                                                               const float4 *ualpha = nullptr, const float2 *uq = nullptr)
-{
-    QH_WAVE_FIRST();
-    if (c->done) return;
+__device__ __forceinline__ void pit_recur_eig_body(const int k, const int j, Zf *Xe, const Zf *Ye, Zf *D, const double *theta, const double *lam, int nsel, int S, int64_t T, const R *mu,
+                                                   double beta, const PitCtrl *c, const float *Msum, float damp, const float4 *ualpha, const float2 *uq)
+{
     __shared__ float4 aff[2 * PIT_RT];
-    const int k = blockIdx.x, j = blockIdx.y;
     const int ncol = S * nsel;
     Zf *row = D + (size_t)k * ncol + j, *xr = Xe + (size_t)k * ncol + j;
     const Zf *yr = Ye + (size_t)k * ncol + j;
@@ -1524,6 +1531,15 @@
         }
     }
 }
+template <typename R>
+__global__ void __launch_bounds__(PIT_RT) pit_recur_eig_kernel(Zf *Xe, const Zf *Ye, Zf *D, const double *theta, const double *lam, int nsel, int S, int64_t T, const R *mu,
+                                                               double beta, const PitCtrl *c, const float *Msum = nullptr, float damp = 1.f,
+                                                               const float4 *ualpha = nullptr, const float2 *uq = nullptr)
+{
+    QH_WAVE_FIRST();
+    if (c->done) return;
+    pit_recur_eig_body<R>((int)blockIdx.x, (int)blockIdx.y, Xe, Ye, D, theta, lam, nsel, S, T, mu, beta, c, Msum, damp, ualpha, uq);
+}
 
 template <typename R>
 __global__ void __launch_bounds__(256) pit_recur_kernel(Zf *D, const double *lam, int nsel, int S, int64_t T, const R *mu, double beta, const PitCtrl *c)
@@ -1630,18 +1646,15 @@
 }
 constexpr int PIT_GT_THREADS = 1024;
 template <typename R>
-__global__ void __launch_bounds__(PIT_GT_THREADS) pit_gauge_kernel(const double *gph, int S, int nsel, PitCtrl *c, double *theta, const double *pw, int nb, int method, const Cx<R> *sy0,
-                                                                   int want_corr, const PitModel *model = nullptr, const float4 *ualpha = nullptr, float2 *uq = nullptr,
-                                                                   const R *mu = nullptr, int64_t T = 0, const float *Msum = nullptr)
-{
-    QH_WAVE_FIRST();
-    if (c->done) return;
+__device__ __forceinline__ void pit_gauge_body(const int vb, const int nvb, const double *gph, int S, int nsel, PitCtrl *c, double *theta, const double *pw, int nb, int method, const Cx<R> *sy0,
+                                               int want_corr, const PitModel *model, const float4 *ualpha, float2 *uq, const R *mu, int64_t T, const float *Msum)
+{
     constexpr int NT = PIT_GT_THREADS;
     __shared__ double redp[NT / 64];
     __shared__ double2 gbuf[NT / 64];
     __shared__ float4 abuf[NT / 64];
-    if (gridDim.x > 1 && blockIdx.x == 1 && !(model && uq)) return;
-    if (model && uq && (gridDim.x == 1 || blockIdx.x == 1)) {
+    if (nvb > 1 && vb == 1 && !(model && uq)) return;
+    if (model && uq && (nvb == 1 || vb == 1)) {
         const bool corr = c->passes == 0 ? true : c->corr_on != 0;
         const int len = (S + NT - 1) / NT;
         const int s0 = threadIdx.x * len, s1 = s0 + len < S ? s0 + len : S;
@@ -1669,7 +1682,7 @@
                 uq[(size_t)s * nsel + j] = float2{m.q11 * r1 + m.q12 * r2, m.q21 * r1 + m.q22 * r2};
             }
         }
-        if (gridDim.x > 1) return;
+        if (nvb > 1) return;
     }
     if (c->passes == 0) {
         double ps = 0;
@@ -1736,15 +1749,23 @@
     }
 }
 template <typename R>
-__global__ void __launch_bounds__(256) pit_devest_kernel(const Zf *D, const double *lam, int n, int ncol, const PitCtrl *c, float *devmax, unsigned *ticket, PitDecideArgs<R> da)
+__global__ void __launch_bounds__(PIT_GT_THREADS) pit_gauge_kernel(const double *gph, int S, int nsel, PitCtrl *c, double *theta, const double *pw, int nb, int method, const Cx<R> *sy0,
+                                                                   int want_corr, const PitModel *model = nullptr, const float4 *ualpha = nullptr, float2 *uq = nullptr,
+                                                                   const R *mu = nullptr, int64_t T = 0, const float *Msum = nullptr)
 {
     QH_WAVE_FIRST();
     if (c->done) return;
+    pit_gauge_body<R>((int)blockIdx.x, (int)gridDim.x, gph, S, nsel, c, theta, pw, nb, method, sy0, want_corr, model, ualpha, uq, mu, T, Msum);
+}
+template <typename R>
+__device__ __forceinline__ void pit_devest_body(const int vb, const int nvb, const int tid, const bool act, const Zf *D, const double *lam, int n, int ncol, float *devmax, unsigned *ticket,
+                                                const PitDecideArgs<R> &da)
+{
     __shared__ float part[2][4][64], red[64], reds[64], redt[64], redm[64];
-    const int cl = threadIdx.x & 63, kg = threadIdx.x >> 6;
-    const int col = blockIdx.x * 64 + cl;
+    const int cl = tid & 63, kg = tid >> 6;
+    const int col = vb * 64 + cl;
     float acc = 0.f, tap = 0.f;
-    if (col < ncol) {
+    if (act && col < ncol) {
 #pragma unroll 8
         for (int k = kg; k < n; k += 4) {
             const Zf v = D[(size_t)k * ncol + col];
@@ -1753,7 +1774,7 @@
             tap += m2;
         }
     }
-    part[0][kg][cl] = acc; part[1][kg][cl] = tap;
+    if (act) { part[0][kg][cl] = acc; part[1][kg][cl] = tap; }
     __syncthreads();
     if (kg == 0) {
         acc = (part[0][0][cl] + part[0][1][cl]) + (part[0][2][cl] + part[0][3][cl]);
@@ -1765,27 +1786,149 @@
     }
     __syncthreads();
     for (int s = 32; s > 0; s >>= 1) {
-        if (threadIdx.x < s) {
-            red[threadIdx.x] = red[threadIdx.x] > red[threadIdx.x + s] ? red[threadIdx.x] : red[threadIdx.x + s];
-            reds[threadIdx.x] += reds[threadIdx.x + s];
-            redt[threadIdx.x] += redt[threadIdx.x + s];
-            redm[threadIdx.x] = redm[threadIdx.x] > redm[threadIdx.x + s] ? redm[threadIdx.x] : redm[threadIdx.x + s];
+        if (tid < s) {
+            red[tid] = red[tid] > red[tid + s] ? red[tid] : red[tid + s];
+            reds[tid] += reds[tid + s];
+            redt[tid] += redt[tid + s];
+            redm[tid] = redm[tid] > redm[tid + s] ? redm[tid] : redm[tid + s];
         }
         __syncthreads();
     }
-    if (threadIdx.x == 0) {
-        devmax[4 * blockIdx.x] = red[0]; devmax[4 * blockIdx.x + 1] = reds[0]; devmax[4 * blockIdx.x + 2] = redt[0]; devmax[4 * blockIdx.x + 3] = redm[0];
+    if (tid == 0) {
+        devmax[4 * vb] = red[0]; devmax[4 * vb + 1] = reds[0]; devmax[4 * vb + 2] = redt[0]; devmax[4 * vb + 3] = redm[0];
     }
     __shared__ int last;
-    if (threadIdx.x == 0) {
+    if (tid == 0) {
         __threadfence();
         const unsigned t = atomicAdd(ticket, 1u);
-        last = t == gridDim.x - 1;
+        last = t == (unsigned)nvb - 1;
         if (last) { *ticket = 0; __threadfence(); }
     }
     __syncthreads();
     if (!last) return;
-    pit_decide_body<R>(da);
+    pit_decide_body<R>(da, tid, act);
+}
+template <typename R>
+__global__ void __launch_bounds__(256) pit_devest_kernel(const Zf *D, const double *lam, int n, int ncol, const PitCtrl *c, float *devmax, unsigned *ticket, PitDecideArgs<R> da)
+{
+    QH_WAVE_FIRST();
+    if (c->done) return;
+    pit_devest_body<R>((int)blockIdx.x, (int)gridDim.x, (int)threadIdx.x, true, D, lam, n, ncol, devmax, ticket, da);
+}
+struct PitSync { unsigned count; int abandoned; };
+constexpr int PIT_RES_GRID = 80;
+constexpr int PIT_RES_THREADS = 1024;
+constexpr unsigned PIT_RES_POLLS = 1u << 16;
+constexpr int PIT_RES_BARRIERS = 5;
+constexpr size_t PIT_RES_LDS = 96 * 1024;
+template <typename R> struct PitAnalysisArgs {
+    const Zf *V, *VT;
+    const Cx<R> *X, *Y;
+    Zf *Xe, *Ye, *Yprev, *D;
+    const double *lam;
+    double *dfc, *pw, *gph, *theta;
+    float4 *ualpha; float2 *uq; const PitModel *model;
+    const Cx<R> *sy0; const R *mu;
+    float *devmax; unsigned *ticket;
+    PitCtrl *c; PitSync *sync;
+    double beta;
+    int64_t T;
+    int n, S, nsel, sym, method, ssb;
+    int nt, groups, lds_group;
+    int carried;
+    int back;
+    unsigned gen0, polls;
+    PitFuse<R> fz; PitDecideArgs<R> da;
+};
+static __device__ __forceinline__ bool pit_grid_barrier(PitSync *s, unsigned target, unsigned polls)
+{
+    __shared__ int passed;
+    __threadfence();
+    __syncthreads();
+    if (threadIdx.x == 0) {
+        __hip_atomic_fetch_add(&s->count, 1u, __ATOMIC_RELAXED, __HIP_MEMORY_SCOPE_AGENT);
+        int ok = 0;
+        for (unsigned i = 0; i < polls; i++) {
+            if (__hip_atomic_load(&s->abandoned, __ATOMIC_RELAXED, __HIP_MEMORY_SCOPE_AGENT)) break;
+            if (__hip_atomic_load(&s->count, __ATOMIC_RELAXED, __HIP_MEMORY_SCOPE_AGENT) >= target) { ok = 1; break; }
+            __builtin_amdgcn_s_sleep(8);
+        }
+        if (!ok) __hip_atomic_store(&s->abandoned, 1, __ATOMIC_RELAXED, __HIP_MEMORY_SCOPE_AGENT);
+        passed = ok;
+    }
+    __syncthreads();
+    __threadfence();
+    return passed != 0;
+}
+template <typename R>
+__global__ void __launch_bounds__(PIT_RES_THREADS) pit_analysis_kernel(PitAnalysisArgs<R> a)
+{
+    QH_WAVE_FIRST();
+    if (a.c->done) return;
+    extern __shared__ __attribute__((aligned(16))) char pit_smem[];
+    const int tid = threadIdx.x, G = gridDim.x;
+    const int ncol = a.S * a.nsel, nb1 = (ncol + PIT_MC - 1) / PIT_MC;
+    const int grp = tid / a.nt, gt = tid - grp * a.nt;
+    const bool in_grp = grp < a.groups;
+    char *gsm = pit_smem + (size_t)(in_grp ? grp : 0) * a.lds_group;
+    unsigned gen = a.gen0;
+    auto barrier = [&]() -> bool {
+        gen++;
+        if (pit_grid_barrier(a.sync, gen * (unsigned)G, a.polls)) return true;
+        if (tid == 0) {
+            a.c->done = 1;
+            __threadfence_system();
+            __hip_atomic_store(&a.da.host_view[0], 3.f, __ATOMIC_RELEASE, __HIP_MEMORY_SCOPE_SYSTEM);
+        }
+        return false;
+    };
+    {
+        PitFuse<R> f1 = a.fz;
+        f1.T2 = a.Y; f1.Out2 = reinterpret_cast<float2 *>(a.Ye);
+        const int nvb = a.carried ? nb1 : 2 * nb1;
+        for (int b0 = blockIdx.x * a.groups; b0 < nvb; b0 += G * a.groups) {
+            const int vb = b0 + grp;
+            const bool act = in_grp && vb < nvb;
+            pit_basis_mfma_body<R, 0>(act ? vb : 0, gt, a.nt, act, gsm, a.V, a.carried ? a.Y : a.X, (const Zf *)nullptr, a.carried ? a.Ye : a.Xe, a.n, ncol, f1);
+            __syncthreads();
+        }
+    }
+    if (!barrier()) return;
+    {
+        const int nent = (a.S - 1) * a.nsel + a.nsel;
+        for (int bi = blockIdx.x * (PIT_RES_THREADS / 64) + (tid >> 6); bi < nent; bi += G * (PIT_RES_THREADS / 64))
+            pit_bound_body(bi, tid & 63, a.Xe, a.Ye, a.Yprev, a.lam, a.n, a.S, a.nsel, a.sym, a.c, a.dfc, a.pw, a.gph, a.ualpha);
+    }
+    if (!barrier()) return;
+    {
+        const int nvb = a.ssb ? 2 : 1;
+        if ((int)blockIdx.x < nvb)
+            pit_gauge_body<R>((int)blockIdx.x, nvb, a.gph, a.S, a.nsel, a.c, a.theta, a.pw, (a.S - 1) * a.nsel, a.method, a.sy0, 1, a.model, a.ualpha, a.uq, a.mu, a.T, (const float *)nullptr);
+    }
+    if (!barrier()) return;
+    for (int vb = blockIdx.x; vb < a.n * a.nsel; vb += G) {
+        pit_recur_eig_body<R>(vb % a.n, vb / a.n, a.Xe, a.Ye, a.D, a.theta, a.lam, a.nsel, a.S, a.T, a.mu, a.beta, a.c, (const float *)nullptr, 1.f, a.ualpha, a.uq);
+        __syncthreads();
+    }
+    if (!barrier()) return;
+    {
+        const int ndev = (ncol + 63) / 64;
+        for (int vb = blockIdx.x; vb < ndev; vb += G) {
+            pit_devest_body<R>(vb, ndev, tid, tid < 256, a.D, a.lam, a.n, ncol, a.devmax, a.ticket, a.da);
+            __syncthreads();
+        }
+    }
+    if (!barrier()) return;
+    if (!a.back || __hip_atomic_load(&a.c->done, __ATOMIC_RELAXED, __HIP_MEMORY_SCOPE_AGENT)) return;
+    for (int b0 = blockIdx.x * a.groups; b0 < nb1; b0 += G * a.groups) {
+        const int vb = b0 + grp;
+        const bool act = in_grp && vb < nb1;
+        pit_basis_mfma_body<R, 1>(act ? vb : 0, gt, a.nt, act, gsm, a.VT, (const Cx<R> *)nullptr, (const Zf *)a.D, (Zf *)nullptr, a.n, ncol, a.fz);
+        __threadfence();
+        __syncthreads();
+        pit_basis_mfma_body<R, 0>(act ? vb : 0, gt, a.nt, act, gsm, a.V, (const Cx<R> *)a.fz.X, (const Zf *)nullptr, a.Xe, a.n, ncol, a.fz);
+        __syncthreads();
+    }
 }
 static __global__ void __launch_bounds__(256) pit_front_kernel(const Zf *D, const double *lam, int n, int ncol, double thr, int *front, int *bad)
 {
@@ -2103,6 +2246,7 @@
     if ((rc = scratch(8, sizeof(PitCtrl) + 64, &cbuf))) return rc;
     PitCtrl *ctrl = report_dev ? (PitCtrl *)report_dev : (PitCtrl *)cbuf;
     R *mu_acq = (R *)((char *)cbuf + sizeof(PitCtrl));
+    PitSync *psync = (PitSync *)((char *)cbuf + sizeof(PitCtrl) + 16);
 
     int S = o.segments;
     const float ad_relax = 1.0f, ad_damp = 0.7f;
@@ -2229,6 +2373,14 @@
     const bool tables_ok = method == QH_M_CMA || method == QH_M_SGNCMA || method == QH_M_MCMA || method == QH_M_RDE || method == QH_M_MRDE ||
                            (decision && (use_bi || seg_form));
     const bool ssb = eig && tables_ok && method != QH_M_CMA2;
+    const int res_nt = pit_mfma_threads(ntot);
+    const size_t res_lds1 = (pit_mfma_lds(ntot) + 15) / 16 * 16;
+    int res_groups = PIT_RES_THREADS / res_nt;
+    if ((size_t)res_groups * res_lds1 > PIT_RES_LDS) res_groups = (int)(PIT_RES_LDS / res_lds1);
+    const bool resident = eig && !adaptive && !split && sg.S <= 8192 && res_groups >= 1 && form(FORM_PIT_ANALYSIS) != 1;
+    const unsigned res_polls = form(FORM_PIT_ANALYSIS) == 2 ? 0u : PIT_RES_POLLS;
+    int res_grid = ntot * nsel < PIT_RES_GRID ? ntot * nsel : PIT_RES_GRID;
+    if (res_grid < 2) res_grid = 2;
     PitModel *model = nullptr;
     float4 *ualpha = nullptr;
     float2 *uqv = nullptr;
@@ -2258,6 +2410,7 @@
         QH_HIP(hipFuncSetAttribute((const void *)pit_cgemm_kernel<R, false>, hipFuncAttributeMaxDynamicSharedMemorySize, 160 * 1024 - 256));
         QH_HIP(hipFuncSetAttribute((const void *)pit_basis_mfma_kernel<R, 0>, hipFuncAttributeMaxDynamicSharedMemorySize, 128 * 1024));
         QH_HIP(hipFuncSetAttribute((const void *)pit_basis_mfma_kernel<R, 1>, hipFuncAttributeMaxDynamicSharedMemorySize, 128 * 1024));
+        QH_HIP(hipFuncSetAttribute((const void *)pit_analysis_kernel<R>, hipFuncAttributeMaxDynamicSharedMemorySize, (int)PIT_RES_LDS));
         gemm_attr.store(true, std::memory_order_release);
     }
 
@@ -2320,7 +2473,7 @@
             rot_use = rot;
         }
         const Cx<R> *w_exact = o.start == 1 ? nullptr : ((it == 0 && o.acquire) ? (const Cx<R> *)w_start : (const Cx<R> *)wx);
-        hipLaunchKernelGGL((pit_seed_kernel<R>), dim3(sg.S), dim3(256), 0, g_stream, (const Cx<R> *)wx, nmodes, ntot, (const int64_t *)modes_dev, nsel, rot_use, X, w_exact, Y, ctrl);
+        hipLaunchKernelGGL((pit_seed_kernel<R>), dim3(sg.S), dim3(256), 0, g_stream, (const Cx<R> *)wx, nmodes, ntot, (const int64_t *)modes_dev, nsel, rot_use, X, w_exact, Y, ctrl, (unsigned *)psync);
         if (ssb) {
             ma.sg = sg; ma.rot = rot_use;
             static thread_local hipEvent_t ev_seed = nullptr, ev_model = nullptr;
@@ -2351,7 +2504,8 @@
             PitFuse<R> fz;
             fz.X = X; fz.Y = Y; fz.theta = theta; fz.modes_dev = (const int64_t *)modes_dev; fz.nmodes = nmodes; fz.nsel = nsel;
             fz.damp = (adaptive && p > 1) ? ad_damp : 1.f;
-            if (p > 0 && want_corr) {
+            if (p > 0 && resident) {
+            } else if (p > 0 && want_corr) {
                 if (eig)
                     hipLaunchKernelGGL((pit_basis_mfma_kernel<R, 1>), dim3((ncol + PIT_MC - 1) / PIT_MC), dim3(pit_mfma_threads(ntot)), pit_mfma_lds(ntot), g_stream, Vb + (size_t)ntot * ntot,
                                        (const Cx<R> *)nullptr, (const Zf *)Dz[1], (Zf *)nullptr, ntot, ncol, (const PitCtrl *)ctrl, fz);
@@ -2414,6 +2568,22 @@
                     hipLaunchKernelGGL((pit_basis_mfma_kernel<R, 0>), dim3(2 * ((ncol + PIT_MC - 1) / PIT_MC)), dim3(pit_mfma_threads(ntot)), pit_mfma_lds(ntot), g_stream, Vb, src, (const Zf *)nullptr, dst, ntot, ncol, (const PitCtrl *)ctrl, f2);
                 };
                 if (p == 0 && model_event) QH_HIP(hipStreamWaitEvent(g_stream, model_event, 0));
+                if (resident) {
+                    PitAnalysisArgs<R> aa;
+                    aa.V = Vb; aa.VT = Vb + (size_t)ntot * ntot; aa.X = X; aa.Y = Y; aa.Xe = Xe; aa.Ye = Ye; aa.Yprev = Yprev; aa.D = Dz[1];
+                    aa.lam = lam; aa.dfc = dfc; aa.pw = pw; aa.gph = gph; aa.theta = theta; aa.ualpha = ualpha; aa.uq = uqv; aa.model = model;
+                    aa.sy0 = (const Cx<R> *)symbols + (size_t)modes[0] * nsy; aa.mu = (const R *)mu_dev; aa.devmax = devmax; aa.ticket = ticket;
+                    aa.c = ctrl; aa.sync = psync; aa.beta = beta; aa.T = sg.len;
+                    aa.n = ntot; aa.S = sg.S; aa.nsel = nsel; aa.sym = sym; aa.method = method; aa.ssb = ssb ? 1 : 0;
+                    aa.nt = res_nt; aa.groups = res_groups; aa.lds_group = (int)res_lds1;
+                    aa.carried = p > 0 ? 1 : 0; aa.back = p + 1 < npass ? 1 : 0;
+                    aa.gen0 = (unsigned)p * PIT_RES_BARRIERS; aa.polls = res_polls;
+                    aa.fz = fz; aa.fz.damp = 1.f;
+                    aa.da = decide_args(p, (const float *)devmax, (const float2 *)Ye, (float2 *)Yprev, ntot, ncol, 1);
+                    hipLaunchKernelGGL((pit_analysis_kernel<R>), dim3(res_grid), dim3(PIT_RES_THREADS), (size_t)res_groups * res_lds1, g_stream, aa);
+                    QH_HIP(hipGetLastError());
+                    return QH_OK;
+                }
                 forward2((const Cx<R> *)X, Xe, (const Cx<R> *)Y, Ye);
                 hipLaunchKernelGGL(pit_bound_kernel, dim3((nbnd + nsel + 3) / 4), dim3(256), 0, g_stream, (const Zf *)Xe, (const Zf *)Ye, (const Zf *)Yprev, lam, ntot, sg.S, nsel, sym,
                                    (const PitCtrl *)ctrl, dfc, pw, gph, ualpha);
@@ -2455,6 +2625,7 @@
         }
         bool ahead = false;
         bool certified = false;
+        bool abandoned = false;
         for (int p = 0; p < npass; p++) {
             double contr = PIT_CONTRACT;
             if (p >= 2 && ev.hview[2 * (p - 2) + 1] > 0) {
@@ -2485,7 +2656,7 @@
                 QH_HIP(hipEventElapsedTime(&ms, ev.t0[p], ev.t1[p]));
                 tm.pass_ms[tm.npass++] = ms;
             }
-            if (ev.hview[2 * p] != 0.f) { certified = ev.hview[2 * p] == 1.f; break; }
+            if (ev.hview[2 * p] != 0.f) { certified = ev.hview[2 * p] == 1.f; abandoned = ev.hview[2 * p] == 3.f; break; }
             if (p + 1 < npass && !ahead && (rc = enqueue_pass(p + 1))) return rc;
         }
         if (acq_timed) {
@@ -2494,7 +2665,7 @@
             QH_HIP(hipEventElapsedTime(&ms, ev.t0[PIT_NEV - 1], ev.t1[PIT_NEV - 1]));
             tm.acq_ms = ms; acq_timed = false;
         }
-        if (!adaptive && !certified && redo_ok && !split && depth < 3 && o.head_auto_off == 0) {
+        if (!adaptive && !certified && !abandoned && redo_ok && !split && depth < 3 && o.head_auto_off == 0) {
             double hp = 0;
             int hfront[2] = {-1, 0};
             bool finite = false;
```

After: 630.6. -47.8%, worse.
